# treangenlab/komb

Measured on AMD Instinct MI355X. Metric: peeled edges/sec (k-truss), higher is better.
Workload: dtype int32

## Files before the change

### komb_amd/csrc/api.cpp

```cpp
#include "common.h"

#include <cerrno>
#include <cmath>
#include <cstdlib>
#include <cstring>
#include <memory>
#include <new>
#include <vector>

using namespace komb;

namespace {

int require_device(komb_ctx *ctx)
{
    if (!ctx) return KOMB_ERR_ARG;
    if (!ctx->device_ok) {
        if (ctx->err.empty()) ctx->err = "no usable HIP device";
        return KOMB_ERR_DEVICE;
    }
    KOMB_HIP(ctx, hipSetDevice(ctx->device));
    ctx->err.clear();
    return KOMB_OK;
}

}

extern "C" {

int komb_abi_version(void) { return KOMB_ACCEL_ABI_VERSION; }

komb_ctx *komb_create(const komb_opts *opts)
{
    komb_ctx *ctx = new (std::nothrow) komb_ctx();
    if (!ctx) return nullptr;
    if (opts) ctx->opts = *opts;
    ctx->device = ctx->opts.device;
    int ndev = 0;
    hipError_t e = hipGetDeviceCount(&ndev);
    if (e != hipSuccess || ndev <= 0) {
        ctx->err = std::string("no usable HIP device: ") + (e != hipSuccess ? hipGetErrorString(e) : "device count is 0");
        (void)hipGetLastError();
        return ctx;
    }
    if (ctx->device < 0 || ctx->device >= ndev) {
        ctx->err = "device ordinal out of range";
        return ctx;
    }
    e = hipSetDevice(ctx->device);
    if (e == hipSuccess) e = hipHostMalloc((void **)&ctx->h_ctrl, 2 * sizeof(PeelCtrl), hipHostMallocDefault);
    if (e == hipSuccess) e = hipHostMalloc((void **)&ctx->h_local, 2 * sizeof(LocalCtrl), hipHostMallocDefault);
    if (e == hipSuccess) e = hipHostMalloc(&ctx->h_stage, kStageBytes, hipHostMallocDefault);
    ctx->stream = nullptr;
    if (e == hipSuccess && !(ctx->opts.reserved[0] & KOMB_CREATE_NULL_STREAM)) { e = hipStreamCreate(&ctx->stream); ctx->own_stream = e == hipSuccess; }
    if (e == hipSuccess && !ctx->timer.init()) e = hipErrorUnknown;
    if (e != hipSuccess) {
        ctx->err = std::string("device initialisation failed: ") + hipGetErrorString(e);
        return ctx;
    }
    ctx->device_ok = true;
    if (!(ctx->opts.reserved[0] & KOMB_CREATE_NO_WARMUP)) warm_up(ctx);
    return ctx;
}

void komb_destroy(komb_ctx *ctx)
{
    if (!ctx) return;
    if (ctx->device_ok) {
        (void)hipSetDevice(ctx->device);
        graph_free(ctx);
        stager_free(ctx);
        ctx->pool.clear();
        ctx->timer.destroy();
        if (ctx->own_stream && ctx->stream) (void)hipStreamDestroy(ctx->stream);
        if (ctx->h_ctrl) (void)hipHostFree(ctx->h_ctrl);
        if (ctx->h_local) (void)hipHostFree(ctx->h_local);
        if (ctx->h_stage) (void)hipHostFree(ctx->h_stage);
    }
    delete ctx;
}

const char *komb_last_error(const komb_ctx *ctx) { return ctx ? ctx->err.c_str() : "null context"; }

int komb_graph_from_edges(komb_ctx *ctx, int64_t nv, int64_t n_raw, const int64_t *uv_pairs)
{
    KOMB_TRY(require_device(ctx));
    return graph_from_edges(ctx, nv, n_raw, uv_pairs);
}
// ... 926 lines not shown
```

### komb_amd/csrc/clique_census.hip

```cpp
#include "clique_root_dev.h"

#include <algorithm>

namespace komb {

namespace {

constexpr int kCcGrid = 1024;
constexpr uint32_t kCcBatch = 256;
static_assert((long long)kCcGrid * kCcBatch == KOMB_MAXCLQ_OVERSHOOT, "the documented overshoot");
constexpr uint32_t kCcLdsCand = 512;
constexpr size_t kCcLdsBytes = 56u << 10;
constexpr size_t kCcScratchBytes = 512ull << 20;
constexpr long long kCcDefaultBudget = 1ll << 30;
constexpr long long kCcMaxBudget = 0x7FFFFFFFll - KOMB_MAXCLQ_OVERSHOOT;
constexpr unsigned long long kCcSat = ~0ull;
constexpr int32_t kCcPivotBit = (int32_t)0x80000000u;

struct CcCtl {
    unsigned long long nodes;
    unsigned long long n_roots;
    uint32_t cursor;
    uint32_t t_max;
    uint32_t max_p;
// ... 330 lines not shown
        uint32_t n_l = std::min(max_p, (uint32_t)cc_opt(ctx, "CENSUS_LDS", kCcLdsCand, 0, kCcLdsCand));
        while (n_l > 0 && (head_words + (size_t)n_l * ((n_l + 63u) >> 6)) * 8 > kCcLdsBytes) n_l -= 1;
        const uint32_t w_l = (n_l + 63u) >> 6;
        A.lds_cand = n_l;
        A.lds_off_tot = (uint32_t)(head_words - n_k);
        A.lds_off_mat = (uint32_t)head_words;
        A.lds_off_stk = A.lds_off_mat + n_l * w_l;
        A.lds_levels = std::min(n_l, depth) + 2;
        size_t lds_words = A.lds_off_stk;
        if (n_l > 0 && (lds_words + (size_t)A.lds_levels * w_l) * 8 <= kCcLdsBytes) lds_words += (size_t)A.lds_levels * w_l;
        else A.lds_levels = 0;
        if (lds_words * 8 > kCcLdsBytes)
            KOMB_FAIL(ctx, KOMB_ERR_LIMIT, "komb_clique_census_run: a window of %u sizes at t_max %d does not fit the LDS of a wavefront", n_k, (int)t_max);
        int grid = (int)std::min<uint32_t>(A.n_chunks, (uint32_t)kCcGrid);
        const size_t fit = kCcScratchBytes / A.slot_bytes;
        if ((size_t)grid > fit) grid = fit < 1 ? 1 : (int)fit;
        KOMB_HIP(ctx, bufs.alloc(&A.scratch, (size_t)grid * A.slot_bytes));
        A.count_only = false;
        KOMB_HIP(ctx, hipMemsetAsync(&A.ctl->cursor, 0, sizeof(uint32_t), s));
        k_cc_census<<<grid, kWave, lds_words * 8, s>>>(A);
        KOMB_HIP(ctx, hipGetLastError());
        const uint32_t n_scan = std::max<uint32_t>(n_k, k_local ? (uint32_t)nv : 0u);
        k_cc_saturated<<<(int)((n_scan + kBlock - 1) / kBlock), kBlock, 0, s>>>(A.total, n_k, A.local, (uint32_t)nv, A.ctl);
        KOMB_HIP(ctx, hipGetLastError());
        KOMB_HIP(ctx, d2h(ctx, &h, A.ctl, sizeof(CcCtl)));
        if (h.bad)
            KOMB_FAIL(ctx, KOMB_ERR_DEVICE, "komb_clique_census_run: the walk is inconsistent (k_lo %d, k_hi %d, largest candidate set %u)", (int)k_lo, (int)k_hi, max_p);
        KOMB_HIP(ctx, staged_copy(ctx, res.total.data(), A.total, (size_t)n_k * sizeof(unsigned long long), false));
        res.flags = (h.stopped ? 0 : KOMB_CENSUS_COMPLETE) | (h.saturated ? KOMB_CENSUS_SATURATED : 0);
        res.max_p = (int32_t)max_p;
        res.n_roots = (int64_t)h.n_roots;
        res.nodes = (int64_t)h.nodes;
    }
    res.ms = ctx->timer.stop(s);
    KOMB_HIP(ctx, hipGetLastError());
    for (uint32_t i = 0; i < n_k; ++i)
        if (res.total[i]) res.omega = k_lo + (int32_t)i;
    if (ctx_flag(ctx, "CENSUS_DEBUG"))
        fprintf(stderr, "komb clique census: %lld edges, t_max %d, window %d .. %d, k_local %d, omega %d, flags %d, largest candidate set %d, %lld roots, "
                "%lld nodes of %lld, run %.3f ms\n", (long long)m, res.t_max, res.k_lo, res.k_hi, res.k_local, res.omega, res.flags, res.max_p,
                (long long)res.n_roots, (long long)res.nodes, limit, res.ms);
    clique_census_drop(ctx);
    ctx->d_cc_local = fresh.local;
    fresh.local = nullptr;
    ctx->cc = std::move(res);
    ctx->cc_done = true;
    return KOMB_OK;
}

}
```

### komb_amd/csrc/clique_communities.hip

```cpp
#include "common.h"
#include "unionfind_dev.h"

#include <algorithm>

namespace komb {

namespace {

constexpr int kPcGrid = 1024;
constexpr long long kPcDefaultBudget = 1ll << 32;
constexpr long long kPcMaxWords = 1ll << 24;
constexpr uint32_t kPcMaxSize = 4098;
constexpr uint32_t kPcNone = 0xFFFFFFFFu;

struct PcCtl {
    unsigned long long pair_tests;
    unsigned long long links;
    uint32_t cursor;
    uint32_t bad;
    uint32_t pad[2];
};
static_assert(sizeof(PcCtl) == 32, "PcCtl layout");

struct PcArgs {
// ... 378 lines not shown
        k_pc_vfix<<<pc_grid(nv), kBlock, 0, s>>>(d_vc, d_vc + nv, unv);
        KOMB_HIP(ctx, hipGetLastError());
        KOMB_HIP(ctx, d2h(ctx, &h, A.ctl, sizeof(PcCtl)));
        if (h.bad)
            KOMB_FAIL(ctx, KOMB_ERR_DEVICE, "komb_clique_communities_run: the links are inconsistent (k %d, %lld member cliques, %lld communities)", (int)k,
                      (long long)res.n_member, (long long)n_comm);
        links_seen = (uint32_t)std::min<unsigned long long>(h.links, 0xFFFFFFFFull);
        res.n_comm = n_comm;
        res.rep.resize((size_t)n_comm);
        res.n_cliques.resize((size_t)n_comm);
        res.verts.resize((size_t)n_uniq);
        std::vector<uint32_t> coff((size_t)n_comm);
        KOMB_HIP(ctx, staged_copy(ctx, res.label.data(), d_label, (size_t)nc * sizeof(int32_t), false));
        KOMB_HIP(ctx, staged_copy(ctx, res.size.data(), d_size, (size_t)nc * sizeof(int32_t), false));
        KOMB_HIP(ctx, staged_copy(ctx, res.rep.data(), d_rep, (size_t)n_comm * sizeof(int32_t), false));
        KOMB_HIP(ctx, staged_copy(ctx, res.n_cliques.data(), d_ncl, (size_t)n_comm * sizeof(int32_t), false));
        KOMB_HIP(ctx, staged_copy(ctx, coff.data(), d_coff, (size_t)n_comm * sizeof(uint32_t), false));
        KOMB_HIP(ctx, staged_copy(ctx, res.verts.data(), d_cverts, (size_t)n_uniq * sizeof(int32_t), false));
        KOMB_HIP(ctx, staged_copy(ctx, res.v_comm.data(), d_vc, (size_t)nv * sizeof(int32_t), false));
        KOMB_HIP(ctx, staged_copy(ctx, res.v_first.data(), d_vc + nv, (size_t)nv * sizeof(int32_t), false));
        res.offset.assign((size_t)n_comm + 1, 0);
        for (int64_t c = 0; c < n_comm; ++c) res.offset[(size_t)c] = (int64_t)coff[(size_t)c];
        res.offset[(size_t)n_comm] = n_uniq;
        for (int64_t c = 0; c < n_comm; ++c) {
            const int64_t len = res.offset[(size_t)c + 1] - res.offset[(size_t)c];
            if (len < k) KOMB_FAIL(ctx, KOMB_ERR_DEVICE, "komb_clique_communities_run: community %lld has %lld vertices at k %d", (long long)c, (long long)len, (int)k);
            res.largest = std::max(res.largest, len);
        }
        for (int64_t v = 0; v < nv; ++v) {
            res.n_covered += res.v_comm[(size_t)v] >= 1;
            res.n_overlap += res.v_comm[(size_t)v] >= 2;
        }
    }
    res.ms = ctx->timer.stop(s);
    KOMB_HIP(ctx, hipGetLastError());
    if (ctx_flag(ctx, "PERC_DEBUG"))
        fprintf(stderr, "komb clique communities: k %d (list k_min %d), %lld cliques, %lld members of at most %u vertices, %lld entries, group %u, "
                "%lld pair tests of %llu, %u links, %lld communities, largest %lld, covered %lld, overlap %lld, run %.3f ms\n", (int)k, (int)res.k_min,
                (long long)nc, (long long)res.n_member, smax, (long long)entries, group, (long long)res.pair_tests, limit, links_seen, (long long)res.n_comm,
                (long long)res.largest, (long long)res.n_covered, (long long)res.n_overlap, res.ms);
    ctx->pc = std::move(res);
    ctx->pc_done = true;
    return KOMB_OK;
}

}
```

### komb_amd/csrc/common.h

```cpp
#pragma once

#include <hip/hip_runtime.h>

#include <chrono>
#include <cstddef>
#include <cstdint>
#include <cstdio>
#include <cstdlib>
#include <cstring>
#include <map>
#include <string>
#include <vector>

#include "komb_accel.h"

#include <roctracer/roctx.h>

namespace komb {

struct Range {
    explicit Range(const char *name) { (void)roctxRangePushA(name); }
    ~Range() { (void)roctxRangePop(); }
    void next(const char *name) { (void)roctxRangePop(); (void)roctxRangePushA(name); }
    Range(const Range &) = delete;
// ... 33 lines not shown
    int32_t  live_sel;
    int32_t  live_mode;
    int32_t  seq;
    uint32_t tail_l[2];
    uint32_t tail_h[2];
    int32_t  next_min;
    uint32_t live_tail;
    int32_t  last_retire;
    uint32_t tail_limit;
    uint32_t pad1[7];
    int32_t  max_retire_gap;
};
static_assert(offsetof(PeelCtrl, seq) == 60 && offsetof(PeelCtrl, tail_l) == 64, "PeelCtrl: the entry state is one 64-byte line");
static_assert(sizeof(PeelCtrl) == 128, "PeelCtrl layout");

struct LocalCtrl {
    int32_t  done;
    int32_t  iters;
    uint32_t spare[3];
    uint32_t bad;
    int32_t  max_val;
    uint32_t levels;
    uint32_t evals;
    uint32_t n_light, n_heavy;
    uint32_t n_giant;
    uint32_t n_chunk;
    uint32_t pad0;
    unsigned long long key_sum;
};
static_assert(sizeof(LocalCtrl) == 64, "LocalCtrl layout");

enum FinishMode : int { FIN_LOCAL = 0, FIN_LDS = 1, FIN_NONE = 2 };

struct Timer {
    hipEvent_t a = nullptr, b = nullptr;
    bool init() { return hipEventCreate(&a) == hipSuccess && hipEventCreate(&b) == hipSuccess; }
    void start(hipStream_t s) { (void)hipEventRecord(a, s); }
    double stop(hipStream_t s)
    {
        (void)hipEventRecord(b, s);
        (void)hipEventSynchronize(b);
        float ms = 0.f;
        (void)hipEventElapsedTime(&ms, a, b);
        return (double)ms;
    }
    void destroy() { if (a) (void)hipEventDestroy(a); if (b) (void)hipEventDestroy(b); a = b = nullptr; }
};

struct EventSet {
    std::vector<hipEvent_t> v;
    EventSet() = default;
    EventSet(const EventSet &) = delete;
    EventSet &operator=(const EventSet &) = delete;
    hipError_t make(hipEvent_t *out, unsigned flags = 0)
    {
        hipEvent_t e = nullptr;
        const hipError_t rc = flags ? hipEventCreateWithFlags(&e, flags) : hipEventCreate(&e);
        if (rc == hipSuccess) { v.push_back(e); *out = e; }
        return rc;
    }
    ~EventSet() { for (hipEvent_t e : v) if (e) (void)hipEventDestroy(e); }
};

}

struct Poison {
    bool on = false;
    uint32_t word = 0;
    hipStream_t stream = nullptr;
    hipError_t fill(void *p, size_t bytes) const
    {
        if (!on || !p || !bytes) return hipSuccess;
        const size_t words = bytes / 4, rest = bytes % 4;
        hipError_t e = hipSuccess;
        if (words) e = hipMemsetD32Async((hipDeviceptr_t)p, (int)word, words, stream);
        if (e == hipSuccess && rest) e = hipMemsetAsync((char *)p + 4 * words, (int)(word & 0xFFu), rest, stream);
        return e == hipSuccess ? hipStreamSynchronize(stream) : e;
    }
    hipError_t malloc(void **out, size_t bytes) const
// ... 58 lines not shown
        for (auto &b : blocks) { if (b.used) keep.push_back(b); else (void)hipFree(b.p); }
        blocks.swap(keep);
    }
    void clear()
    {
        for (auto &b : blocks) (void)hipFree(b.p);
        blocks.clear();
    }
};

struct TrussPrep {
    bool valid = false;
    int64_t nv = 0, ne = 0;
    int32_t  *o2i = nullptr, *i2o = nullptr;
    uint32_t *orow = nullptr;
    int32_t  *ocol = nullptr, *osrc = nullptr;
    uint32_t *e2k = nullptr;
    uint4    *vline = nullptr;
    void     *wtasks = nullptr;
    int64_t   n_wtasks = 0;
    int64_t   own_bound = 0;
    double    ms = 0.0;
    double    ms_part[4] = {0, 0, 0, 0};
};

struct komb_ctx {
    komb_opts opts{};
    DevPool pool;
    std::string err;
    bool device_ok = false;
    int device = 0;
    hipStream_t stream = nullptr;
    bool own_stream = false;
    komb::Timer timer;
    std::map<std::string, std::string> options;

    int64_t nv = -1, ne = 0;
    uint32_t *d_o_rowptr = nullptr;
    int32_t  *d_o_col = nullptr;
    TrussPrep prep;

    int32_t *d_deg = nullptr;
    int32_t *d_core = nullptr;
    bool core_done = false;

    int32_t *d_onion_layer = nullptr;
    int32_t *d_onion_core = nullptr;
    int64_t onion_layers = 0;
    int32_t onion_max_core = 0;
    double onion_ms = 0.0;
    bool onion_done = false;

    int32_t *d_comp_label = nullptr;
    int32_t *d_comp_size = nullptr;
    int32_t comp_kind = 0, comp_k = 0;
    int64_t comp_members = 0, comp_count = 0, comp_largest = 0;
    double comp_ms = 0.0;
    bool comp_done = false;

    int32_t *d_hier_nodes = nullptr;
    int32_t *d_hier_vnode = nullptr;
    int32_t hier_kind = 0, hier_kmax = 0, hier_depth = 0;
    int64_t hier_nodes = 0, hier_roots = 0;
    double hier_ms = 0.0;
    bool hier_done = false;

    int32_t *d_dens_member = nullptr;
// ... 178 lines not shown
    void release(void *q)
    {
        for (auto &p : owned) if (p == q && q) { ctx->pool.put(q); p = nullptr; }
    }
    ~DevBufs() { for (void *p : owned) if (p) ctx->pool.put(p); }
};

#define KOMB_FAIL(ctx, code, ...)                                   \
    do {                                                            \
        char _b[512];                                               \
        snprintf(_b, sizeof(_b), __VA_ARGS__);                      \
        (ctx)->err = _b;                                            \
        return (code);                                              \
    } while (0)

#define KOMB_HIP(ctx, call)                                                          \
    do {                                                                             \
        hipError_t _e = (call);                                                      \
        if (_e != hipSuccess) {                                                      \
            hipError_t _nomem = hipErrorOutOfMemory;                                 \
            KOMB_FAIL(ctx, _e == _nomem ? KOMB_ERR_NOMEM : KOMB_ERR_DEVICE,          \
                      "%s failed: %s (%s:%d)", #call, hipGetErrorString(_e),         \
                      __FILE__, __LINE__);                                           \
        }                                                                            \
    } while (0)

#define KOMB_TRY(expr)                         \
    do {                                       \
        int _s = (expr);                       \
        if (_s != KOMB_OK) return _s;          \
    } while (0)

constexpr size_t kStageBytes = 64 << 10;
inline hipError_t d2h(komb_ctx *ctx, void *dst, const void *src, size_t bytes)
{
    if (ctx->h_stage && bytes <= kStageBytes && dst != ctx->h_stage) {
        hipError_t e = hipMemcpyAsync(ctx->h_stage, src, bytes, hipMemcpyDeviceToHost, ctx->stream);
        if (e == hipSuccess) e = hipStreamSynchronize(ctx->stream);
        if (e == hipSuccess) memcpy(dst, ctx->h_stage, bytes);
        return e;
    }
    hipError_t e = hipMemcpyAsync(dst, src, bytes, hipMemcpyDeviceToHost, ctx->stream);
    return e == hipSuccess ? hipStreamSynchronize(ctx->stream) : e;
}

namespace komb {
int prim_sort_u64(komb_ctx *ctx, uint64_t *keys, uint64_t *tmp_keys, int64_t n, int end_bit, uint64_t **sorted);
int prim_unique_u64(komb_ctx *ctx, const uint64_t *in, uint64_t *out, int64_t n, int64_t *n_out);
int prim_exclusive_sum_u32(komb_ctx *ctx, const uint32_t *in, uint32_t *out, int64_t n);
int prim_exclusive_sum_u32_u64(komb_ctx *ctx, const uint32_t *in, unsigned long long *out, int64_t n);
int prim_sort_pairs_desc_i64(komb_ctx *ctx, int64_t *keys, int64_t *keys_tmp, uint32_t *vals, uint32_t *vals_tmp,
                             int64_t n, int end_bit, int64_t **sorted_keys, uint32_t **sorted_vals);

int prim_sort_pairs_u32_u64(komb_ctx *ctx, uint32_t *keys, uint32_t *keys_alt, unsigned long long *vals, unsigned long long *vals_alt,
                            int64_t n, int begin_bit, int end_bit, uint32_t **sorted_keys, unsigned long long **sorted_vals);
int prim_sort_pairs_u32_u32(komb_ctx *ctx, uint32_t *keys, uint32_t *keys_alt, uint32_t *vals, uint32_t *vals_alt,
                            int64_t n, int end_bit, uint32_t **sorted_keys, uint32_t **sorted_vals);
int prim_sort_pairs_u64_u32(komb_ctx *ctx, uint64_t *keys, uint64_t *keys_alt, uint32_t *vals, uint32_t *vals_alt,
                            int64_t n, int end_bit, uint64_t **sorted_keys, uint32_t **sorted_vals);

struct ForestNodes { int32_t *k, *rep, *par; uint32_t *size, *shell; };
struct ForestCtl {
    uint32_t log_n;
    uint32_t n_nodes;
    uint32_t n_roots;
    int32_t  depth;
// ... 41 lines not shown
void clique_census_drop(komb_ctx *ctx);
int maximal_cliques_run(komb_ctx *ctx, int32_t k_min, int64_t budget);
void maximal_cliques_drop(komb_ctx *ctx);
int clique_communities_run(komb_ctx *ctx, int32_t k, int64_t budget);
void clique_communities_drop(komb_ctx *ctx);
int densest_run(komb_ctx *ctx, int32_t iters);
int truss_run(komb_ctx *ctx, const uint8_t *vmask_host, int rank, int world, komb_allreduce_fn fn, void *user);
int merge_run(komb_ctx *ctx, const double *susp_host, int32_t *order, int32_t *side, int64_t *n_block, double *max_density);
int corea_ranks(komb_ctx *ctx, const int32_t *deg, const int32_t *core, int64_t n, double *rank_deg, double *rank_key);
int graph_from_edges(komb_ctx *ctx, int64_t nv, int64_t n_raw, const int64_t *uv);
int graph_from_csr(komb_ctx *ctx, int64_t nv, const int64_t *rowptr, const int32_t *col);
void graph_free(komb_ctx *ctx);
void stager_free(komb_ctx *ctx);
hipError_t staged_copy(komb_ctx *ctx, void *dst, const void *src, size_t bytes, bool to_device);
void warm_up(komb_ctx *ctx);
int prep_build(komb_ctx *ctx, const uint32_t *rowptr, const int32_t *col, int64_t nv, int64_t ns, TrussPrep *out);
void prep_free(komb_ctx *ctx, TrussPrep *p);
int prep_ensure(komb_ctx *ctx);
int prep_sources(komb_ctx *ctx, TrussPrep *p);
int graph_moments(komb_ctx *ctx, int64_t out[5]);
struct InducedCsr { int64_t nv = 0, ns = 0; uint32_t *rowptr = nullptr; int32_t *col = nullptr; int32_t *vold = nullptr; };
int induce_csr(komb_ctx *ctx, const uint8_t *vmask_host, InducedCsr *out);
void induced_free(komb_ctx *ctx, InducedCsr *g);
int edge_list(komb_ctx *ctx, const uint32_t *rowptr, const int32_t *col, int64_t nv, const int32_t *vold, int32_t *eu, int32_t *ev);
int truss_edges_canonical(komb_ctx *ctx);
void truss_free(komb_ctx *ctx);
int truss_support_canonical(komb_ctx *ctx);
void peel_ctrl_pre(hipStream_t s, uint32_t *d_grp_done);
void peel_collect_ctrl(hipStream_t s, PeelCtrl *d_collect, const PeelCtrl *d_from);
void peel_ctrl_init(hipStream_t s, PeelCtrl *d_ctrl, uint32_t *d_grp_done, uint32_t units, uint32_t tail_limit = 0);
int peel_grid(int64_t units);

template <typename F>
int drive_peel(komb_ctx *ctx, PeelCtrl *d_ctrl, int64_t units, F &&launch, int *launches_out)
{
#ifndef KOMB_PEEL_BATCH
#define KOMB_PEEL_BATCH 24
#endif
#ifndef KOMB_PEEL_BATCH_SHORT
#define KOMB_PEEL_BATCH_SHORT 6
#endif
    constexpr int kBatch = KOMB_PEEL_BATCH, kBatchShort = KOMB_PEEL_BATCH_SHORT, kShortBatches = 6;
    PeelCtrl first;
    KOMB_HIP(ctx, d2h(ctx, &first, d_ctrl, sizeof(PeelCtrl)));
    int32_t next = first.seq;
#ifdef KOMB_DEBUG_SWITCHES
    if (const char *tr = getenv("KOMB_PEEL_TRACE")) {
        FILE *f = fopen(tr, "a");
        hipEvent_t a = nullptr, b = nullptr;
        if (hipEventCreate(&a) != hipSuccess || hipEventCreate(&b) != hipSuccess) {
            if (f) fclose(f);
            if (a) (void)hipEventDestroy(a);
            KOMB_FAIL(ctx, KOMB_ERR_DEVICE, "peel trace: hipEventCreate failed");
        }
        int launches = 0;
        if (f) fprintf(f, "# peel units=%lld\n", (long long)units);
        for (int64_t i = 0; i < 4 * units + 4096; ++i) {
            PeelCtrl before;
            if (d2h(ctx, &before, d_ctrl, sizeof(PeelCtrl)) != hipSuccess) break;
            if (before.done) break;
            (void)hipEventRecord(a, ctx->stream);
            launch(before.seq); ++launches;
            (void)hipEventRecord(b, ctx->stream);
            (void)hipEventSynchronize(b);
            float ms = 0.f;
            (void)hipEventElapsedTime(&ms, a, b);
            if (f) fprintf(f, "%d %d %d %u %u %d %u %u %.1f\n", before.mode, before.level, before.round, before.cur_light,
                           before.cur_heavy, before.live_mode, before.live_count, before.remaining, ms * 1000.f);
        }
        if (f) fclose(f);
        (void)hipEventDestroy(a); (void)hipEventDestroy(b);
        if (launches_out) *launches_out = launches;
        KOMB_HIP(ctx, d2h(ctx, &ctx->h_ctrl[0], d_ctrl, sizeof(PeelCtrl)));
        return KOMB_OK;
    }
#endif
    EventSet evs;
    hipEvent_t ev[2] = {nullptr, nullptr};
    KOMB_HIP(ctx, evs.make(&ev[0], hipEventDisableTiming));
    KOMB_HIP(ctx, evs.make(&ev[1], hipEventDisableTiming));
    const int64_t max_batches = (4 * units + 4096) / kBatch + 16 + kShortBatches;
    int launches = 0, slot = 0, status = KOMB_OK;
    bool have_prev = false, finished = false, stuck = false;
    int32_t seen_seq = first.seq - 1;
    for (int64_t batch = 0; batch < max_batches && !finished; ++batch) {
        const int nb = (batch >= 1 && batch <= kShortBatches) ? kBatchShort : kBatch;
        for (int i = 0; i < nb; ++i) { launch(next); ++next; ++launches; }
        if (hipMemcpyAsync(&ctx->h_ctrl[slot], d_ctrl, sizeof(PeelCtrl), hipMemcpyDeviceToHost, ctx->stream) != hipSuccess ||
            hipEventRecord(ev[slot], ctx->stream) != hipSuccess) { status = KOMB_ERR_DEVICE; break; }
        if (have_prev) {
            if (hipEventSynchronize(ev[slot ^ 1]) != hipSuccess) { status = KOMB_ERR_DEVICE; break; }
            const PeelCtrl &h = ctx->h_ctrl[slot ^ 1];
            if (h.done) finished = true;
            else if (h.seq == seen_seq) { stuck = true; finished = true; }
            seen_seq = h.seq;
        }
        have_prev = true;
        slot ^= 1;
    }
    hipError_t e = hipStreamSynchronize(ctx->stream);
    if (launches_out) *launches_out = launches;
    if (status != KOMB_OK || e != hipSuccess)
        KOMB_FAIL(ctx, KOMB_ERR_DEVICE, "peel driver: HIP failure (%s)", hipGetErrorString(e));
    if (d2h(ctx, &ctx->h_ctrl[0], d_ctrl, sizeof(PeelCtrl)) != hipSuccess)
        KOMB_FAIL(ctx, KOMB_ERR_DEVICE, "peel driver: control block readback failed");
    if (!ctx->h_ctrl[0].done)
        KOMB_FAIL(ctx, KOMB_ERR_DEVICE, "peel driver: %s (level %d, remaining %u, launch %d of state %d)",
                  stuck ? "the launches make no progress" : "launch budget exhausted before completion",
                  ctx->h_ctrl[0].level, ctx->h_ctrl[0].remaining, (int)next, (int)ctx->h_ctrl[0].seq);
    return KOMB_OK;
}
}
```

### komb_amd/csrc/communities.hip

```cpp
#include "common.h"
#include "unionfind_dev.h"

namespace komb {

namespace {

constexpr uint32_t kCommShort = 16;
constexpr uint32_t kCommHeavy = 2048;
constexpr int kCommHeavyGrid = 256, kCommHeavyChunks = 8;
constexpr int kCommTailGrid = 2048;

struct CommCtl {
    uint32_t n_heavy;
    uint32_t n_members, n_communities, largest;
    uint32_t n_multi;
    uint32_t pad[11];
};
static_assert(sizeof(CommCtl) == 64, "CommCtl layout");

inline int comm_grid(int64_t n) { return (int)((n + kBlock - 1) / kBlock); }

__global__ void k_comm_flag(const int32_t *__restrict__ truss, uint32_t m, int32_t k, uint32_t *__restrict__ flag)
{
    const uint32_t i = blockIdx.x * kBlock + threadIdx.x;
// ... 247 lines not shown
    KOMB_HIP(ctx, bufs.alloc(&d_ctl, 1));
    KOMB_HIP(ctx, bufs.alloc(&d_flag, (size_t)m + 1));
    KOMB_HIP(ctx, bufs.alloc(&d_pos, (size_t)m + 1));
    KOMB_HIP(ctx, bufs.alloc(&d_kept, (size_t)m));
    KOMB_HIP(ctx, bufs.alloc(&d_mu, (size_t)m));
    KOMB_HIP(ctx, bufs.alloc(&d_mv, (size_t)m));
    KOMB_HIP(ctx, bufs.alloc(&d_parent, (size_t)m));
    KOMB_HIP(ctx, bufs.alloc(&d_heavy, (size_t)heavy_cap));
    KOMB_HIP(ctx, bufs.alloc(&d_rs, (size_t)nv));
    KOMB_HIP(ctx, bufs.alloc(&d_re, (size_t)nv));
    const uint32_t n_short = comm_opt_u32(ctx, "COMM_SHORT", kCommShort);
    uint32_t n_heavy = comm_opt_u32(ctx, "COMM_HEAVY", kCommHeavy);
    if (n_heavy <= n_short) n_heavy = n_short + 1;

    const int32_t *eu = ctx->d_t_eu, *ev = ctx->d_t_ev, *truss = ctx->d_t_truss;
    const uint32_t *d_nm = d_pos + m;
    uint32_t *d_cnt = d_flag;
    const int grid = comm_grid(m), grid1 = comm_grid(m + 1);
    ctx->timer.start(s);
    KOMB_HIP(ctx, hipMemsetAsync(d_ctl, 0, sizeof(CommCtl), s));
    KOMB_HIP(ctx, hipMemsetAsync(d_rs, 0, (size_t)nv * sizeof(uint32_t), s));
    KOMB_HIP(ctx, hipMemsetAsync(d_re, 0, (size_t)nv * sizeof(uint32_t), s));
    k_comm_flag<<<grid1, kBlock, 0, s>>>(truss, (uint32_t)m, k, d_flag);
    KOMB_TRY(prim_exclusive_sum_u32(ctx, d_flag, d_pos, m + 1));
    k_comm_compact<<<grid, kBlock, 0, s>>>(eu, ev, truss, (uint32_t)m, k, d_pos, d_kept, d_mu, d_mv, d_parent, d_cnt);
    k_comm_rows<<<grid, kBlock, 0, s>>>(d_mu, d_nm, d_rs, d_re);
    k_comm_tri<<<grid, kBlock, 0, s>>>(d_mu, d_mv, d_rs, d_re, d_nm, d_parent, d_ctl, d_heavy, heavy_cap, n_short, n_heavy);
    k_comm_heavy<<<dim3(kCommHeavyGrid, kCommHeavyChunks), kBlock, 0, s>>>(d_mu, d_mv, d_rs, d_re, d_parent, d_ctl, d_heavy, heavy_cap);
    k_comm_flatten<false><<<grid, kBlock, 0, s>>>(d_nm, d_parent);
    k_comm_flatten<true><<<grid, kBlock, 0, s>>>(d_nm, d_parent);
    const int tail_grid = grid < kCommTailGrid ? grid : kCommTailGrid;
    k_comm_count<<<tail_grid, kBlock, 0, s>>>(d_nm, d_parent, d_cnt);
    k_comm_finish<<<tail_grid, kBlock, 0, s>>>((uint32_t)m, truss, k, d_pos, d_parent, d_kept, d_cnt, ctx->d_comm_label, ctx->d_comm_size, d_ctl);
    const double ms = ctx->timer.stop(s);
    KOMB_HIP(ctx, hipGetLastError());
    CommCtl h;
    KOMB_HIP(ctx, d2h(ctx, &h, d_ctl, sizeof(CommCtl)));
    ctx->comm_members = (int64_t)h.n_members; ctx->comm_count = (int64_t)h.n_communities; ctx->comm_largest = (int64_t)h.largest;
    ctx->comm_ms = ms;
    ctx->comm_done = true;
    fail.armed = false;
    return KOMB_OK;
}

int communities_vertices(komb_ctx *ctx)
{
    if (ctx->comm_v_ready) return KOMB_OK;
    hipStream_t s = ctx->stream;
    const int64_t m = ctx->t_ne, nv = ctx->nv, nm = ctx->comm_members;
    if (!ctx->d_comm_ncomm) KOMB_HIP(ctx, ctx->pool.get((void **)&ctx->d_comm_ncomm, (size_t)(nv > 0 ? nv : 1) * sizeof(int32_t)));
    ctx->comm_multi = 0;
    ctx->timer.start(s);
    KOMB_HIP(ctx, hipMemsetAsync(ctx->d_comm_ncomm, 0, (size_t)(nv > 0 ? nv : 1) * sizeof(int32_t), s));
    if (nm > 0) {
        Range r_all("komb_truss_communities: vertices");
        DevBufs bufs(ctx);
        CommCtl *d_ctl = nullptr;
        uint32_t *d_flag = nullptr, *d_pos = nullptr;
        uint64_t *d_keys = nullptr, *d_tmp = nullptr, *sorted = nullptr;
        KOMB_HIP(ctx, bufs.alloc(&d_ctl, 1));
        KOMB_HIP(ctx, bufs.alloc(&d_flag, (size_t)m + 1));
        KOMB_HIP(ctx, bufs.alloc(&d_pos, (size_t)m + 1));
        KOMB_HIP(ctx, bufs.alloc(&d_keys, 2 * (size_t)nm));
        KOMB_HIP(ctx, bufs.alloc(&d_tmp, 2 * (size_t)nm));
        KOMB_HIP(ctx, hipMemsetAsync(d_ctl, 0, sizeof(CommCtl), s));
        k_comm_vflag<<<comm_grid(m + 1), kBlock, 0, s>>>(ctx->d_comm_label, (uint32_t)m, d_flag);
        KOMB_TRY(prim_exclusive_sum_u32(ctx, d_flag, d_pos, m + 1));
        k_comm_keys<<<comm_grid(m), kBlock, 0, s>>>(ctx->d_t_eu, ctx->d_t_ev, ctx->d_comm_label, (uint32_t)m, d_pos, d_keys);
        int vb = 1;
        while (vb < 31 && (1ll << vb) < nv) ++vb;
        KOMB_TRY(prim_sort_u64(ctx, d_keys, d_tmp, 2 * nm, 32 + vb, &sorted));
        uint64_t *uniq = sorted == d_keys ? d_tmp : d_keys;
        int64_t n_u = 0;
        KOMB_TRY(prim_unique_u64(ctx, sorted, uniq, 2 * nm, &n_u));
        k_comm_runs<<<comm_grid(n_u), kBlock, 0, s>>>(uniq, (uint32_t)n_u, ctx->d_comm_ncomm, d_ctl);
        KOMB_HIP(ctx, hipGetLastError());
        CommCtl h;
        KOMB_HIP(ctx, d2h(ctx, &h, d_ctl, sizeof(CommCtl)));
        ctx->comm_multi = (int64_t)h.n_multi;
    }
    ctx->comm_ms_vertices = ctx->timer.stop(s);
    ctx->comm_v_ready = true;
    return KOMB_OK;
}

}
```

### komb_amd/csrc/community_hierarchy.hip

```cpp
#include "forest_dev.h"

namespace komb {

namespace {

constexpr uint32_t kChShort = 16;
constexpr uint32_t kChHeavy = 2048;
constexpr int kChHeavyGrid = 256, kChHeavyChunks = 8;
constexpr uint64_t kChMaxRecords = 0x7FFFFFFFull;

struct ChCtl {
    ForestCtl f;
    uint32_t n_heavy;
    uint32_t n_members;
    uint32_t rec_n;
    uint32_t pad0;
    unsigned long long n_tri;
    uint32_t pad[6];
};
static_assert(sizeof(ChCtl) == 64 && offsetof(ChCtl, f) == 0, "ChCtl layout");


__global__ void k_ch_flag(const int32_t *__restrict__ truss, uint32_t m, uint32_t *__restrict__ flag)
{
// ... 325 lines not shown
            uint32_t n_levels = 0;
            for (int32_t k = (int32_t)levels - 1; k >= 3; --k) n_levels += moff[k + 1] - moff[k] ? 1u : 0u;
            KOMB_HIP(ctx, bufs.alloc(&seg, (size_t)n_levels + 1));
            KOMB_HIP(ctx, hipMemsetAsync(seg, 0, ((size_t)n_levels + 1) * sizeof(uint32_t), s));

            const ForestState f{parent, log, claimk, cur, cnt, seg, mnode, t, &d_ctl->f, nm};
            uint32_t li = 0;
            for (int32_t k = (int32_t)levels - 1; k >= 3; --k) {
                const uint32_t sh_b = moff[k], sh_n = moff[k + 1] - moff[k];
                const uint32_t r_b = roff[k], r_n = roff[k + 1] - roff[k];
                if (!sh_n) continue;
                if (li == 0) k_max = k;
                if (r_n) k_ch_link<<<forest_grid(r_n), kBlock, 0, s>>>(recs, r_b, r_n, nm, parent, d_ctl, log, nm);
                forest_level(ctx, f, k, li, false, mord, sh_b, sh_n, r_n < nm ? r_n : nm);
                ++li;
            }
            KOMB_HIP(ctx, hipGetLastError());
            KOMB_HIP(ctx, d2h(ctx, &h, d_ctl, sizeof(ChCtl)));
            if (h.f.n_nodes > nm || h.f.log_n > nm || h.rec_n != n_rec)
                KOMB_FAIL(ctx, KOMB_ERR_DEVICE, "komb_community_hierarchy_run: inconsistent state (%u nodes, %u hooks, %u members, %u of %u records)",
                          h.f.n_nodes, h.f.log_n, nm, h.rec_n, n_rec);
            n = h.f.n_nodes;
            if (n > 0) {
                cap_nodes = n;
                KOMB_HIP(ctx, ctx->pool.get((void **)&fresh.nodes, 5 * cap_nodes * sizeof(int32_t)));
                ForestNodes out{fresh.nodes, fresh.nodes + cap_nodes, fresh.nodes + 2 * cap_nodes,
                                (uint32_t *)fresh.nodes + 3 * cap_nodes, (uint32_t *)fresh.nodes + 4 * cap_nodes};
                KOMB_TRY(forest_tail(ctx, bufs, f, n, bits, out, rank, kept, mvals, mvals2));
            }
            k_ch_edges_out<<<grid, kBlock, 0, s>>>((uint32_t)m, truss, d_pos, mnode, rank, n, fresh.enode);
        } else {
            k_ch_edges_out<<<grid, kBlock, 0, s>>>((uint32_t)m, truss, d_pos, nullptr, nullptr, 0u, fresh.enode);
        }
        ms = ctx->timer.stop(s);
        KOMB_HIP(ctx, hipGetLastError());
        KOMB_HIP(ctx, d2h(ctx, &h, d_ctl, sizeof(ChCtl)));
        n_nodes = (int64_t)n; n_roots = (int64_t)h.f.n_roots; depth = h.f.depth; n_members = (int64_t)nm;
        if (n == 0) k_max = 2;
    }
    if (!fresh.nodes) KOMB_HIP(ctx, ctx->pool.get((void **)&fresh.nodes, 5 * cap_nodes * sizeof(int32_t)));

    community_hierarchy_drop(ctx);
    ctx->d_ch_nodes = fresh.nodes; ctx->d_ch_enode = fresh.enode;
    fresh.nodes = fresh.enode = nullptr;
    ctx->ch_cap = (int64_t)cap_nodes;
    ctx->ch_nodes = n_nodes; ctx->ch_roots = n_roots; ctx->ch_members = n_members;
    ctx->ch_kmax = k_max; ctx->ch_depth = depth; ctx->ch_ms = ms;
    ctx->ch_done = true;
    return KOMB_OK;
}

int community_hierarchy_labels(komb_ctx *ctx, int32_t k, int32_t *label, int32_t *size)
{
    const int64_t m = ctx->t_ne > 0 ? ctx->t_ne : 0;
    if (m == 0 || (!label && !size)) return KOMB_OK;
    hipStream_t s = ctx->stream;
    DevBufs bufs(ctx);
    int32_t *d_label = nullptr, *d_size = nullptr;
    KOMB_HIP(ctx, bufs.alloc(&d_label, (size_t)m));
    KOMB_HIP(ctx, bufs.alloc(&d_size, (size_t)m));
    const int32_t *nodes = ctx->d_ch_nodes;
    const size_t c = (size_t)ctx->ch_cap;
    k_ch_labels<<<forest_grid(m), kBlock, 0, s>>>((uint32_t)m, k, ctx->d_ch_enode, (uint32_t)ctx->ch_nodes, nodes, nodes + c, nodes + 2 * c,
                                              nodes + 3 * c, d_label, d_size);
    KOMB_HIP(ctx, hipGetLastError());
    KOMB_HIP(ctx, hipStreamSynchronize(s));
    if (label) KOMB_HIP(ctx, staged_copy(ctx, label, d_label, (size_t)m * sizeof(int32_t), false));
// ... 6 lines not shown
```

### komb_amd/csrc/components.hip

```cpp
#include "common.h"
#include "unionfind_dev.h"

namespace komb {

namespace {

constexpr uint32_t kCompShort = 16;
constexpr uint32_t kCompHeavy = 2048;
constexpr uint32_t kCompWindow = 16;
constexpr int kCompSamples = 1024;
constexpr int kCompHeavyGrid = 256, kCompHeavyChunks = 8;
constexpr int kCompTailGrid = 2048;

struct CompCtl {
    int32_t  giant;
    uint32_t n_heavy;
    uint32_t n_members, n_components, largest;
    uint32_t pad[11];
};
static_assert(sizeof(CompCtl) == 64, "CompCtl layout");

__global__ void k_comp_init(uint32_t nv, const int32_t *__restrict__ core, int32_t k, bool all, bool none,
                            int32_t *__restrict__ parent, int32_t *__restrict__ flag, uint32_t *__restrict__ cnt)
{
// ... 211 lines not shown

    const bool truss = kind == KOMB_COMP_TRUSS;
    const int64_t m = truss ? ctx->t_ne : 0;
    if (truss && m > 0) KOMB_TRY(truss_edges_canonical(ctx));

    Range r_all("komb_components_run");
    DevBufs bufs(ctx);
    const uint32_t heavy_cap = (uint32_t)((2 * ctx->ne) / kCompHeavy + 64);
    CompCtl *d_ctl = nullptr; uint32_t *d_cnt = nullptr; int32_t *d_heavy = nullptr;
    KOMB_HIP(ctx, bufs.alloc(&d_ctl, 1));
    KOMB_HIP(ctx, bufs.alloc(&d_cnt, (size_t)nv));
    if (!truss) KOMB_HIP(ctx, bufs.alloc(&d_heavy, (size_t)heavy_cap));
    const char *so = ctx_opt(ctx, "COMP_SAMPLE");
    const bool sample = so ? strcmp(so, "0") != 0 : true;

    int32_t *parent = ctx->d_comp_label, *flag = ctx->d_comp_size;
    const int grid = comp_grid(nv);
    const bool all = !truss && k == 0;
    const bool none = truss || (k > 0 && k > ctx->stats.max_coreness);
    ctx->timer.start(s);
    KOMB_HIP(ctx, hipMemsetAsync(d_ctl, 0, sizeof(CompCtl), s));
    k_comp_init<<<grid, kBlock, 0, s>>>((uint32_t)nv, ctx->d_core, k, all, none, parent, flag, d_cnt);
    if (truss) {
        if (m > 0) k_comp_truss<<<comp_grid(m), kBlock, 0, s>>>(ctx->d_t_eu, ctx->d_t_ev, ctx->d_t_truss, (uint32_t)m, k, parent, flag);
    } else if (!none && ctx->ne > 0) {
        if (all) comp_link_rows<true>(ctx, sample, k, parent, flag, d_ctl, d_heavy, heavy_cap);
        else comp_link_rows<false>(ctx, sample, k, parent, flag, d_ctl, d_heavy, heavy_cap);
    }
    k_comp_flatten<false><<<grid, kBlock, 0, s>>>((uint32_t)nv, parent, flag);
    k_comp_flatten<true><<<grid, kBlock, 0, s>>>((uint32_t)nv, parent, flag);
    const int tail_grid = grid < kCompTailGrid ? grid : kCompTailGrid;
    k_comp_count<<<tail_grid, kBlock, 0, s>>>((uint32_t)nv, parent, d_cnt);
    k_comp_finish<<<tail_grid, kBlock, 0, s>>>((uint32_t)nv, parent, d_cnt, ctx->d_comp_size, d_ctl);
    const double ms = ctx->timer.stop(s);
    KOMB_HIP(ctx, hipGetLastError());
    CompCtl h;
    KOMB_HIP(ctx, d2h(ctx, &h, d_ctl, sizeof(CompCtl)));
    ctx->comp_members = (int64_t)h.n_members; ctx->comp_count = (int64_t)h.n_components; ctx->comp_largest = (int64_t)h.largest;
    ctx->comp_ms = ms;
    ctx->comp_done = true;
    return KOMB_OK;
}

}
```

### komb_amd/csrc/corea.hip

```cpp
#include "common.h"

namespace komb {

namespace {

__global__ __launch_bounds__(kBlock) void k_corea_keys(const int32_t *__restrict__ deg, const int32_t *__restrict__ core,
                                                       int64_t n, int64_t *__restrict__ kdeg, int64_t *__restrict__ kcore,
                                                       uint32_t *__restrict__ idx0, uint32_t *__restrict__ idx1)
{
    for (int64_t i = (int64_t)blockIdx.x * kBlock + threadIdx.x; i < n; i += (int64_t)gridDim.x * kBlock) {
        const int64_t d = deg[i];
        kdeg[i] = d;
        kcore[i] = (int64_t)core[i] * n + d;
        idx0[i] = (uint32_t)i; idx1[i] = (uint32_t)i;
    }
}

__global__ __launch_bounds__(kBlock) void k_run_ranks(const int64_t *__restrict__ sk, const uint32_t *__restrict__ sidx,
                                                      int64_t n, double *__restrict__ rank)
{
    for (int64_t p = (int64_t)blockIdx.x * kBlock + threadIdx.x; p < n; p += (int64_t)gridDim.x * kBlock) {
        const int64_t key = sk[p];
        int64_t lo = 0, hi = p;
        while (lo < hi) {
// ... 25 lines not shown
    if (n < 0 || (n > 0 && (!deg || !core || !rank_deg || !rank_key)))
        KOMB_FAIL(ctx, KOMB_ERR_ARG, "komb_corea: bad arguments");
    ctx->stats.ms_corea = 0.0;
    if (n == 0) return KOMB_OK;
    if (n > INT32_MAX - 1) KOMB_FAIL(ctx, KOMB_ERR_LIMIT, "komb_corea: n exceeds 2^31-2");
    int32_t maxd = 0, maxc = 0;
    for (int64_t i = 0; i < n; ++i) {
        if (deg[i] < 0 || core[i] < 0) KOMB_FAIL(ctx, KOMB_ERR_ARG, "komb_corea: negative degree/coreness at %lld", (long long)i);
        if (deg[i] > maxd) maxd = deg[i];
        if (core[i] > maxc) maxc = core[i];
    }
    hipStream_t s = ctx->stream;
    DevBufs bufs(ctx);
    int32_t *d_deg = nullptr, *d_core = nullptr; int64_t *d_k[4] = {nullptr, nullptr, nullptr, nullptr};
    uint32_t *d_i[4] = {nullptr, nullptr, nullptr, nullptr}; double *d_r[2] = {nullptr, nullptr};
    KOMB_HIP(ctx, bufs.alloc(&d_deg, (size_t)n));
    KOMB_HIP(ctx, bufs.alloc(&d_core, (size_t)n));
    for (int t = 0; t < 4; ++t) KOMB_HIP(ctx, bufs.alloc(&d_k[t], (size_t)n));
    for (int t = 0; t < 4; ++t) KOMB_HIP(ctx, bufs.alloc(&d_i[t], (size_t)n));
    for (int t = 0; t < 2; ++t) KOMB_HIP(ctx, bufs.alloc(&d_r[t], (size_t)n));
    KOMB_HIP(ctx, staged_copy(ctx, d_deg, deg, (size_t)n * 4, true));
    KOMB_HIP(ctx, staged_copy(ctx, d_core, core, (size_t)n * 4, true));
    int64_t g64 = (n + kBlock - 1) / kBlock;
    const int grid = (int)(g64 > 4096 ? 4096 : g64);
    ctx->timer.start(s);
    k_corea_keys<<<grid, kBlock, 0, s>>>(d_deg, d_core, n, d_k[0], d_k[2], d_i[0], d_i[2]);
    int64_t *sk = nullptr; uint32_t *si = nullptr;
    int st = prim_sort_pairs_desc_i64(ctx, d_k[0], d_k[1], d_i[0], d_i[1], n, bits_for(maxd), &sk, &si);
    if (st == KOMB_OK) {
        k_run_ranks<<<grid, kBlock, 0, s>>>(sk, si, n, d_r[0]);
        st = prim_sort_pairs_desc_i64(ctx, d_k[2], d_k[3], d_i[2], d_i[3], n, bits_for((int64_t)maxc * n + maxd), &sk, &si);
    }
    if (st == KOMB_OK) k_run_ranks<<<grid, kBlock, 0, s>>>(sk, si, n, d_r[1]);
    ctx->stats.ms_corea = ctx->timer.stop(s);
    KOMB_TRY(st);
    KOMB_HIP(ctx, staged_copy(ctx, rank_deg, d_r[0], (size_t)n * 8, false));
    KOMB_HIP(ctx, staged_copy(ctx, rank_key, d_r[1], (size_t)n * 8, false));
    return KOMB_OK;
}

}
```

### komb_amd/csrc/densest.hip

```cpp
#include "common.h"

namespace komb {

namespace {

constexpr uint32_t kDenShort = 16;
constexpr uint32_t kDenHeavy = 2048;
constexpr int kDenHeavyGrid = 64, kDenHeavyChunks = 8;
constexpr int kDenGrid = 2048;
constexpr uint32_t kDenLdsBins = 4096;
constexpr int kDenLocalBlock = 1024;
constexpr int kDenPairs = 4;
constexpr uint64_t kDenLocalAutoPairs = 20000;

struct DenCtl {
    uint32_t n_heavy;
    int32_t  k_best, k_prune;
    uint32_t n_p;
    uint32_t max_deg_p;
    uint32_t load_max;
    int32_t  source;
    uint32_t best_i;
    unsigned long long m_best, n_best;
    unsigned long long m_p;
// ... 437 lines not shown
    DevBufs bufs(ctx);
    const int32_t k_max = ctx->stats.max_coreness > 0 ? ctx->stats.max_coreness : 0;
    const uint32_t K = (uint32_t)k_max + 1u;
    const uint32_t heavy_cap = (uint32_t)((2 * ctx->ne) / kDenHeavy + 64);
    const int grid = den_grid((uint64_t)nv);

    DenCtl *d_ctl = nullptr; int32_t *d_heavy = nullptr;
    uint32_t *d_hist = nullptr, *d_flag = nullptr, *d_pid = nullptr, *d_cnt = nullptr, *d_off = nullptr, *d_hdeg = nullptr, *d_hcur = nullptr;
    long long *d_prof = nullptr;
    KOMB_HIP(ctx, bufs.alloc(&d_ctl, 1));
    KOMB_HIP(ctx, bufs.alloc(&d_heavy, (size_t)heavy_cap));
    KOMB_HIP(ctx, bufs.alloc(&d_hdeg, (size_t)heavy_cap));
    KOMB_HIP(ctx, bufs.alloc(&d_hcur, (size_t)heavy_cap));
    KOMB_HIP(ctx, bufs.alloc(&d_hist, (size_t)2 * K));
    KOMB_HIP(ctx, bufs.alloc(&d_prof, (size_t)2 * K));
    KOMB_HIP(ctx, bufs.alloc(&d_flag, (size_t)nv));
    KOMB_HIP(ctx, bufs.alloc(&d_pid, (size_t)nv));
    KOMB_HIP(ctx, bufs.alloc(&d_cnt, (size_t)nv));
    KOMB_HIP(ctx, bufs.alloc(&d_off, (size_t)nv));

    ctx->timer.start(s);
    KOMB_HIP(ctx, hipMemsetAsync(d_ctl, 0, sizeof(DenCtl), s));
    KOMB_HIP(ctx, hipMemsetAsync(d_hist, 0, (size_t)2 * K * sizeof(uint32_t), s));
    KOMB_HIP(ctx, hipMemsetAsync(d_hdeg, 0, (size_t)heavy_cap * sizeof(uint32_t), s));
    KOMB_HIP(ctx, hipMemsetAsync(d_hcur, 0, (size_t)heavy_cap * sizeof(uint32_t), s));
    if (K <= kDenLdsBins) den_row_pass(ctx, DenHist<true>{ctx->d_core, K, d_hist}, (size_t)2 * K * sizeof(uint32_t), d_ctl, d_heavy, heavy_cap);
    else den_row_pass(ctx, DenHist<false>{ctx->d_core, K, d_hist}, 0, d_ctl, d_heavy, heavy_cap);
    k_den_profile<<<1, kBlock, 0, s>>>(K, d_hist, d_prof, d_prof + K, d_ctl);
    k_den_mark<<<grid, kBlock, 0, s>>>((uint32_t)nv, ctx->d_core, d_ctl, d_flag);
    KOMB_TRY(prim_exclusive_sum_u32(ctx, d_flag, d_pid, nv));
    den_row_pass(ctx, DenCount{ctx->d_core, d_cnt, d_hdeg, 0u, 0u, 0u}, 0, d_ctl, d_heavy, heavy_cap);
    KOMB_TRY(prim_exclusive_sum_u32(ctx, d_cnt, d_off, nv));
    k_den_total<<<1, kBlock, 0, s>>>((uint32_t)nv, d_flag, d_pid, d_cnt, d_off, d_hdeg, heavy_cap, d_ctl);
    double ms = ctx->timer.stop(s);
    KOMB_HIP(ctx, hipGetLastError());
    DenCtl h;
    KOMB_HIP(ctx, d2h(ctx, &h, d_ctl, sizeof(DenCtl)));
    std::vector<int64_t> profile((size_t)2 * K);
    KOMB_HIP(ctx, d2h(ctx, profile.data(), d_prof, profile.size() * sizeof(int64_t)));
    const uint64_t n_p = h.n_p, m_p = h.m_p;
    if (n_p > (uint64_t)nv || m_p > (uint64_t)ctx->ne)
        KOMB_FAIL(ctx, KOMB_ERR_DEVICE, "komb_densest_subgraph_run: inconsistent state (%llu of %lld vertices, %llu of %lld edges)",
                  (unsigned long long)n_p, (long long)nv, (unsigned long long)m_p, (long long)ctx->ne);
    if ((uint64_t)iters * h.max_deg_p > (uint64_t)INT32_MAX)
        KOMB_FAIL(ctx, KOMB_ERR_LIMIT, "komb_densest_subgraph_run: %d rounds on a vertex of degree %u inside the pruned set overflow the 32-bit load word",
                  iters, h.max_deg_p);

    const bool rounds = iters >= 1 && m_p > 0;
    uint2 *d_pairs = nullptr; uint32_t *d_load = nullptr, *d_delta = nullptr, *d_rank = nullptr, *d_rhist = nullptr;
    uint64_t *d_keys = nullptr, *d_keys2 = nullptr;
    unsigned long long *d_excl = nullptr, *d_part = nullptr;
    const int part_grid = den_grid_capped(n_p);
    bool local = false;
    if (rounds) {
        KOMB_HIP(ctx, bufs.alloc(&d_pairs, (size_t)m_p + kDenPairs));
        KOMB_HIP(ctx, bufs.alloc(&d_load, (size_t)n_p));
        KOMB_HIP(ctx, bufs.alloc(&d_delta, (size_t)n_p));
        KOMB_HIP(ctx, bufs.alloc(&d_rank, (size_t)n_p));
        KOMB_HIP(ctx, bufs.alloc(&d_rhist, (size_t)n_p));
        KOMB_HIP(ctx, bufs.alloc(&d_keys, (size_t)n_p));
        KOMB_HIP(ctx, bufs.alloc(&d_keys2, (size_t)n_p));
        KOMB_HIP(ctx, bufs.alloc(&d_excl, (size_t)n_p));
        KOMB_HIP(ctx, bufs.alloc(&d_part, (size_t)2 * part_grid));
        int lds_cap = 0;
        KOMB_HIP(ctx, hipDeviceGetAttribute(&lds_cap, hipDeviceAttributeMaxSharedMemoryPerBlock, ctx->device));
        const bool fits = n_p * 2 * sizeof(uint32_t) <= (uint64_t)(lds_cap > 0 ? lds_cap : 0) && m_p <= 0xFFFFFFFFull;
        const char *lo = ctx_opt(ctx, "DENSEST_LOCAL");
        local = fits && (lo ? strcmp(lo, "0") != 0 : m_p <= kDenLocalAutoPairs);
        if (local)
            KOMB_HIP(ctx, hipFuncSetAttribute((const void *)k_den_local, hipFuncAttributeMaxDynamicSharedMemorySize, (int)(n_p * 2 * sizeof(uint32_t))));
    }
    ctx->timer.start(s);
    if (rounds) {
        den_row_pass(ctx, DenFill{ctx->d_core, d_pid, d_off, d_pairs, d_hcur, m_p, 0u}, 0, d_ctl, d_heavy, heavy_cap);
        if (local) {
            k_den_local<<<1, kDenLocalBlock, (size_t)n_p * 2 * sizeof(uint32_t), s>>>(d_pairs, (uint32_t)m_p, (uint32_t)n_p, iters, d_load);
        } else {
            const int rgrid = den_grid((m_p + kDenPairs - 1) / kDenPairs), ngrid = den_grid(n_p);
            k_den_zero2<<<ngrid, kBlock, 0, s>>>((uint32_t)n_p, d_load, d_delta);
            for (int32_t t = 0; t < iters; ++t) {
                k_den_round<<<rgrid, kBlock, 0, s>>>(d_pairs, m_p, (uint32_t)n_p, d_load, d_delta, t & 1);
                k_den_fold<<<ngrid, kBlock, 0, s>>>((uint32_t)n_p, d_load, d_delta);
            }
        }
        KOMB_HIP(ctx, hipGetLastError());
        k_den_keys<<<part_grid, kBlock, 0, s>>>((uint32_t)n_p, d_load, d_keys, d_ctl);
        uint64_t *sorted = nullptr;
        KOMB_TRY(prim_sort_u64(ctx, d_keys, d_keys2, (int64_t)n_p, 64, &sorted));
        k_den_ranks<<<den_grid(n_p), kBlock, 0, s>>>((uint32_t)n_p, sorted, d_rank, d_rhist);
        k_den_rank_hist<<<den_grid(m_p), kBlock, 0, s>>>(d_pairs, m_p, (uint32_t)n_p, d_rank, d_rhist);
        KOMB_TRY(prim_exclusive_sum_u32_u64(ctx, d_rhist, d_excl, (int64_t)n_p));
        k_den_prefix_part<<<part_grid, kBlock, 0, s>>>((uint32_t)n_p, d_rhist, d_excl, d_part);
    }
    k_den_decide<<<1, kWave, 0, s>>>(rounds ? (uint32_t)part_grid : 0u, d_part, d_ctl);
    KOMB_HIP(ctx, hipGetLastError());
    k_den_out<<<grid, kBlock, 0, s>>>((uint32_t)nv, ctx->d_core, d_pid, d_load, d_rank, d_ctl, ctx->d_dens_member, ctx->d_dens_load);
    ms += ctx->timer.stop(s);
    hipError_t e = hipGetLastError();
    if (e == hipSuccess) e = d2h(ctx, &h, d_ctl, sizeof(DenCtl));
    if (e != hipSuccess) { ctx->dens_done = false; KOMB_HIP(ctx, e); }
    komb_ctx::Densest &r = ctx->dens;
    r.source = h.source; r.k_best = h.k_best; r.k_prune = h.k_prune; r.iters = iters; r.k_max = k_max;
    r.n_pruned = (int64_t)n_p; r.m_pruned = (int64_t)m_p; r.n_sub = (int64_t)h.n_sub; r.m_sub = (int64_t)h.m_sub;
    r.load_max = (int64_t)h.load_max; r.ms = ms; r.local = local;
    ctx->dens_profile.swap(profile);
    ctx->dens_done = true;
    return KOMB_OK;
}

}
```

### komb_amd/csrc/hierarchy.hip

```cpp
#include "forest_dev.h"

namespace komb {

namespace {

constexpr uint32_t kHierShort = 16;
constexpr uint32_t kHierHeavy = 2048;
constexpr int kHierHeavyGrid = 64, kHierHeavyChunks = 8;

struct HierCtl {
    ForestCtl f;
    uint32_t n_heavy;
    uint32_t pad[11];
};
static_assert(sizeof(HierCtl) == 64 && offsetof(HierCtl, f) == 0, "HierCtl layout");

__global__ void k_hier_init(uint32_t nv, int32_t *__restrict__ parent, int32_t *__restrict__ cur, int32_t *__restrict__ claimk,
                            uint32_t *__restrict__ cnt, int32_t *__restrict__ vnode, int32_t *__restrict__ lvl)
{
    const uint32_t v = blockIdx.x * kBlock + threadIdx.x;
    if (v >= nv) return;
    parent[v] = (int32_t)v;
    cur[v] = -1;
    claimk[v] = 0x7FFFFFFF;
// ... 213 lines not shown
        if (li == 0) k_top = k;
        uint64_t hooks;
        if (truss) {
            k_hier_edges<<<forest_grid(e_n), kBlock, 0, s>>>(ctx->d_t_eu, ctx->d_t_ev, eord, second[k], e_n, parent, d_ctl, log, (uint32_t)nv);
            hooks = e_n < (uint64_t)nv ? e_n : (uint64_t)nv;
        } else {
            if (k > 0) {
                k_hier_rows<<<forest_grid(sh_n), kBlock, 0, s>>>(ctx->d_o_rowptr, ctx->d_o_col, ctx->d_core, k, vord, sh_b, sh_n, parent, d_ctl,
                                                               d_heavy, heavy_cap, log, (uint32_t)nv);
                if (second[k])
                    k_hier_heavy<<<dim3(second[k] < (uint32_t)kHierHeavyGrid ? second[k] : kHierHeavyGrid, kHierHeavyChunks), kBlock, 0, s>>>(
                        ctx->d_o_rowptr, ctx->d_o_col, ctx->d_core, k, parent, d_ctl, d_heavy, heavy_done, second[k], heavy_cap, log, (uint32_t)nv);
                heavy_done += second[k];
            }
            hooks = (uint64_t)nv - voff[k];
        }
        forest_level(ctx, f, k, li, !truss && k == 0, vord, sh_b, sh_n, hooks);
        ++li;
    }
    KOMB_HIP(ctx, hipGetLastError());
    HierCtl h;
    KOMB_HIP(ctx, d2h(ctx, &h, d_ctl, sizeof(HierCtl)));
    if (h.f.n_nodes > (uint64_t)nv || h.f.log_n > (uint64_t)nv)
        KOMB_FAIL(ctx, KOMB_ERR_DEVICE, "komb_hierarchy_run: inconsistent state (%u nodes, %u hooks, %lld vertices)", h.f.n_nodes, h.f.log_n, (long long)nv);
    if (h.n_heavy != heavy_done)
        KOMB_FAIL(ctx, KOMB_ERR_DEVICE, "komb_hierarchy_run: inconsistent state (%u long rows queued, %u counted)", h.n_heavy, heavy_done);
    const uint32_t n = h.f.n_nodes;

    ForestNodes out{ctx->d_hier_nodes, ctx->d_hier_nodes + cap, ctx->d_hier_nodes + 2 * cap,
                    (uint32_t *)ctx->d_hier_nodes + 3 * cap, (uint32_t *)ctx->d_hier_nodes + 4 * cap};
    int32_t *rank = cur;
    if (n > 0) KOMB_TRY(forest_tail(ctx, bufs, f, n, bits, out, rank, nullptr, vvals, vvals2));
    k_hier_vertices_out<<<grid, kBlock, 0, s>>>((uint32_t)nv, vnode, rank, ctx->d_hier_vnode);
    const double ms = ctx->timer.stop(s);
    KOMB_HIP(ctx, hipGetLastError());
    KOMB_HIP(ctx, d2h(ctx, &h, d_ctl, sizeof(HierCtl)));
    ctx->hier_nodes = (int64_t)n; ctx->hier_roots = (int64_t)h.f.n_roots; ctx->hier_depth = h.f.depth;
    ctx->hier_kmax = n > 0 ? k_top : k_min;
    ctx->hier_ms = ms;
    ctx->hier_done = true;
    return KOMB_OK;
}

}
```

### komb_amd/csrc/kcore.hip

```cpp
#include "peel_dev.h"
#include "core_tail.h"
#include "local_dev.h"
#include "shard_dev.h"

#include <cstdlib>

namespace komb {

namespace {

__global__ __launch_bounds__(kBlock) void k_core_init(const uint32_t *__restrict__ rowptr, int64_t nv,
                                                      int32_t *__restrict__ deg, int32_t *__restrict__ degw,
                                                      int32_t *__restrict__ core, uint32_t *__restrict__ init)
{
    uint32_t zeros = 0;
    int32_t lmin = 0x7FFFFFFF;
    for (int64_t v = (int64_t)blockIdx.x * kBlock + threadIdx.x; v < nv; v += (int64_t)gridDim.x * kBlock) {
        const int32_t d = (int32_t)(rowptr[v + 1] - rowptr[v]);
        deg[v] = d; degw[v] = d;
        if (d == 0) { core[v] = 0; ++zeros; }
        else { core[v] = alive_marker((uint32_t)d); lmin = min(lmin, d); }
    }
    block_add_min(zeros, lmin, &init[0], (int32_t *)&init[1]);
}
// ... 171 lines not shown
{
    k_ctrl_init<<<1, 64, 0, s>>>(d_ctrl, d_grp_done, units, tail_limit);
}

int peel_grid(int64_t units)
{
    int64_t g = (units + kPeelBlock - 1) / kPeelBlock;
    if (g < 1) g = 1;
    if (g > 256 * kPeelPerCu) g = 256 * kPeelPerCu;
    return (int)g;
}

int core_run(komb_ctx *ctx, int rank, int world, komb_allreduce_fn fn, void *user, bool sharded)
{
    if (ctx->nv < 0) KOMB_FAIL(ctx, KOMB_ERR_STATE, "komb_core_run: no graph loaded");
    const int64_t nv = ctx->nv;
    hipStream_t s = ctx->stream;
    ctx->core_done = false;
    if (!ctx->d_deg) {
        KOMB_HIP(ctx, dev_malloc(ctx, (void **)&ctx->d_deg, (size_t)(nv > 0 ? nv : 1) * sizeof(int32_t)));
        KOMB_HIP(ctx, dev_malloc(ctx, (void **)&ctx->d_core, (size_t)(nv > 0 ? nv : 1) * sizeof(int32_t)));
    }
    komb_stats &stt = ctx->stats;
    stt.core_levels = stt.core_subrounds = stt.core_launches = 0;
    stt.max_coreness = 0; stt.ms_core = 0.0;
    stt.core_local_units = 0; stt.core_local_sweeps = 0; stt.core_local_items = 0; stt.ms_core_local = 0.0;
    if (ctx_flag(ctx, "SHARD_ENGINE")) sharded = true;
    stt.shard_exchanges = 0; stt.ms_exchange = 0.0; stt.exchange_words = 0;
    stt.engine_flags = sharded ? KOMB_ENGINE_SHARD_PEEL : 0;
    if (nv == 0) { ctx->core_done = true; return KOMB_OK; }

    Range r_all("komb_core_run");
    DevBufs bufs(ctx);
    const size_t heavy_cap = (size_t)(2 * ctx->ne) / 32 + 64;
    int32_t *d_degw = nullptr; PeelCtrl *d_ctrl = nullptr; uint32_t *d_grp = nullptr;
    CoreTailBufs T{};
    PeelQueues Q{nullptr, {nullptr, nullptr}, {nullptr, nullptr}, {nullptr, nullptr}, 0};
    KOMB_HIP(ctx, bufs.alloc(&d_degw, (size_t)nv));
    for (int i = 0; i < 2; ++i) {
        KOMB_HIP(ctx, bufs.alloc(&Q.light[i], (size_t)nv));
        KOMB_HIP(ctx, bufs.alloc(&Q.heavy[i], heavy_cap));
        KOMB_HIP(ctx, bufs.alloc(&Q.live[i], (size_t)nv / 2 + 64));
    }
    KOMB_HIP(ctx, bufs.alloc(&Q.code, (size_t)nv));
    KOMB_HIP(ctx, bufs.alloc(&d_ctrl, 1));
    KOMB_HIP(ctx, bufs.alloc(&d_grp, (size_t)kInitOff + 4));
    const FinishMode fin = finish_mode(ctx, FIN_LOCAL);
    uint32_t tail_limit = 0;
    const size_t live_words = ((size_t)nv + 63) / 64;
    unsigned long long *d_livebits = nullptr;
    if (fin == FIN_LDS) {
        tail_limit = kCoreTailV;
        if (const char *tl = ctx_opt(ctx, "CORE_TAIL")) tail_limit = (uint32_t)strtoul(tl, nullptr, 10);
        if (tail_limit > kCoreTailV) tail_limit = kCoreTailV;
        if (tail_limit) {
            KOMB_HIP(ctx, bufs.alloc(&T.livebits, live_words));
            KOMB_HIP(ctx, bufs.alloc(&T.vnum, (size_t)nv));
            KOMB_HIP(ctx, bufs.alloc(&T.cnt, 4));
            KOMB_HIP(ctx, bufs.alloc(&T.vlist, (size_t)kCoreTailV));
            KOMB_HIP(ctx, bufs.alloc(&T.rows, (size_t)kCoreTailV * kCoreTailWords));
        }
    } else if (fin == FIN_LOCAL) {
        tail_limit = local_limit(ctx, (uint64_t)nv, 16);
        if (tail_limit) KOMB_HIP(ctx, bufs.alloc(&d_livebits, live_words));
    }

    int64_t g = (nv + kBlock - 1) / kBlock;
    const int grid_init = (int)(g > 1024 ? 1024 : g);
    const int grid = peel_grid(nv);
    CoreProblem P{(uint32_t)nv, ctx->d_o_rowptr, ctx->d_o_col, d_degw, ctx->d_core};
    ctx->timer.start(s);
    peel_ctrl_pre(s, d_grp);
    k_core_init<<<grid_init, kBlock, 0, s>>>(ctx->d_o_rowptr, nv, ctx->d_deg, d_degw, ctx->d_core, d_grp + kInitOff);
    peel_ctrl_init(s, d_ctrl, d_grp, (uint32_t)nv, tail_limit);
    auto run_tail = [&](const int32_t *list, uint32_t n_in) -> int {
        KOMB_HIP(ctx, hipMemsetAsync(T.livebits, 0, live_words * sizeof(unsigned long long), s));
        KOMB_HIP(ctx, hipMemsetAsync(T.cnt, 0, 4 * sizeof(uint32_t), s));
        KOMB_HIP(ctx, hipMemsetAsync(T.rows, 0, (size_t)kCoreTailV * kCoreTailWords * sizeof(unsigned long long), s));
        int64_t gm = ((int64_t)n_in + kBlock - 1) / kBlock;
        k_ctail_mark<<<(int)(gm < 1 ? 1 : (gm > 1024 ? 1024 : gm)), kBlock, 0, s>>>(list, n_in, ctx->d_core, T);
        k_ctail_rows<<<dim3(kCoreTailV, 8), kBlock, 0, s>>>(ctx->d_o_rowptr, ctx->d_o_col, T);
        k_core_tail<false><<<1, 1024, 0, s>>>(d_ctrl, T, d_degw, ctx->d_core, nullptr);
        KOMB_HIP(ctx, d2h(ctx, &ctx->h_ctrl[0], d_ctrl, sizeof(PeelCtrl)));
        return KOMB_OK;
    };
    auto run_local = [&]() -> int {
        const PeelCtrl hc = ctx->h_ctrl[0];
        Range r_local("core: local finish");
        EventSet evs;
        hipEvent_t ev[2] = {nullptr, nullptr};
        for (auto &e : ev) KOMB_HIP(ctx, evs.make(&e));
        (void)hipEventRecord(ev[0], s);
        KOMB_HIP(ctx, hipMemsetAsync(d_livebits, 0, live_words * sizeof(unsigned long long), s));
        LocalStats ls;
        const int rc = local_finish(ctx, bufs, hc, d_ctrl, (uint32_t)nv, ctx->d_core, d_degw, Q.live[hc.live_sel],
            (uint32_t)kWave * CoreLocal::kU, sizeof(uint32_t), local_item_limit(ctx, std::max<uint64_t>(kCoreLocalItems, (uint64_t)ctx->ne / 3)), 0u, false, 0, ctx->d_core,
            [&](const LocalGraph &lg, const int32_t *num, void *items, PeelCtrl *d_cctrl, int32_t launch) {
                CoreCollect C{(uint32_t)nv, ctx->d_o_rowptr, ctx->d_o_col, ctx->d_core, d_livebits, num, lg.off, lg.cur, (uint32_t *)items};
                k_peel_step<CoreCollect><<<grid, kPeelBlock, 0, s>>>(d_cctrl, d_grp, Q, C, launch);
            },
            [&](const LocalGraph &lg, void *items, uint64_t total, LocalCtrl *d_lctrl, uint32_t *d_cnt, int *launches) -> int {
                return local_fixpoint(ctx, d_lctrl, d_cnt, lg, CoreLocal{(const uint32_t *)items}, total, launches);
            },
            &ls,
            [&](const LocalGraph &lg) { k_live_bits<<<(int)((lg.n + 255) / 256 > 1024 ? 1024 : (lg.n + 255) / 256), 256, 0, s>>>(lg.gid, lg.n, d_livebits); });
        (void)hipEventRecord(ev[1], s);
        (void)hipEventSynchronize(ev[1]);
        float ms = 0.f;
        (void)hipEventElapsedTime(&ms, ev[0], ev[1]);
        KOMB_TRY(rc);
        if (ls.refused) { ctx->h_ctrl[0].done = 0; ctx->h_ctrl[0].tail_limit = ls.new_limit; return KOMB_OK; }
        stt.core_local_units = (int32_t)ls.units; stt.core_local_sweeps = ls.sweeps; stt.core_local_items = (int64_t)ls.items;
        stt.ms_core_local = (double)ms;
        PeelCtrl done = hc;
        done.done = 1; done.remaining = 0;
        done.n_levels += (int32_t)ls.levels;
        done.max_level = ls.max_val > done.max_level ? ls.max_val : done.max_level;
        ctx->h_ctrl[0] = done;
        return KOMB_OK;
    };
    int launches = 0, st = KOMB_OK;
    if (sharded) {
        uint32_t iw[2] = {0u, 0u};
        KOMB_HIP(ctx, d2h(ctx, iw, d_grp + kInitOff, sizeof(iw)));
        ShardCore SP{(uint32_t)nv, ctx->d_o_rowptr, ctx->d_o_col, d_degw, ctx->d_core, 0u, 0u};
        shard_bounds((uint64_t)nv, rank, world, &SP.lo, &SP.hi);
        ShardStats ss;
        st = shard_peel(ctx, bufs, SP, d_degw, (uint32_t)nv, iw[0], (int32_t)iw[1], rank, world, fn, user, Q, d_ctrl,
                        [&](int32_t launch) { k_peel_step<ShardCore><<<grid, kPeelBlock, 0, s>>>(d_ctrl, d_grp, Q, SP, launch); },
                        fin == FIN_LOCAL ? tail_limit : 0u, [&]() -> int { return run_local(); }, &ss);
        stt.shard_exchanges = (int32_t)ss.exchanges; stt.ms_exchange = ss.ms_exchange; stt.exchange_words = ss.words;
        launches = ss.launches;
        PeelCtrl fc{};
        fc.done = st == KOMB_OK ? 1 : 2; fc.n_levels = ss.levels; fc.n_rounds = ss.rounds; fc.n_scans = ss.scans; fc.max_level = ss.max_level;
        ctx->h_ctrl[0] = fc;
    } else if (tail_limit && (uint64_t)nv <= tail_limit) {
        st = d2h(ctx, &ctx->h_ctrl[0], d_ctrl, sizeof(PeelCtrl)) == hipSuccess ? KOMB_OK : KOMB_ERR_DEVICE;
        if (st == KOMB_OK && !ctx->h_ctrl[0].done) st = (fin == FIN_LOCAL) ? run_local() : run_tail(nullptr, (uint32_t)nv);
    } else {
        ctx->h_ctrl[0].done = 0;
    }
    for (int guard = 0; st == KOMB_OK && ctx->h_ctrl[0].done != 1 && ctx->h_ctrl[0].done != 2 && guard < 64; ++guard) {
        if (ctx->h_ctrl[0].done == 3) {
            const PeelCtrl &c = ctx->h_ctrl[0];
            if (fin == FIN_LOCAL) st = run_local();
            else st = c.live_mode ? run_tail(Q.live[c.live_sel], c.live_count) : run_tail(nullptr, (uint32_t)nv);
            continue;
        }
        int batch = 0;
        st = drive_peel(ctx, d_ctrl, nv, [&](int32_t launch) {
            k_peel_step<CoreProblem><<<grid, kPeelBlock, 0, s>>>(d_ctrl, d_grp, Q, P, launch);
        }, &batch);
        launches += batch;
    }
    stt.ms_core = ctx->timer.stop(s);
#ifdef KOMB_STEP_TIMERS
    {
        const PeelCtrl &c = ctx->h_ctrl[0];
        const double n = c.pad1[6] ? (double)c.pad1[6] : 1.0;
        fprintf(stderr, "komb core step timers (block 0, %u small multi-workgroup PROCESS steps), us per step: ctrl %.2f queue+slice %.2f items %.2f flush %.2f barrier %.2f ticket %.2f\n",
                c.pad1[6], c.pad1[0] / n / 100.0, c.pad1[1] / n / 100.0, c.pad1[2] / n / 100.0, c.pad1[3] / n / 100.0, c.pad1[4] / n / 100.0, c.pad1[5] / n / 100.0);
    }
#endif
    KOMB_TRY(st);
    if (ctx->h_ctrl[0].done != 1) KOMB_FAIL(ctx, KOMB_ERR_DEVICE, "k-core peel ended in an inconsistent state");
    if (stt.core_local_units) stt.engine_flags |= KOMB_ENGINE_LOCAL_FINISH;
    else if (fin == FIN_LDS && tail_limit) stt.engine_flags |= KOMB_ENGINE_LDS_TAIL;
    stt.core_levels = ctx->h_ctrl[0].n_levels;
    stt.core_subrounds = ctx->h_ctrl[0].n_rounds;
    stt.core_launches = launches;
    stt.max_coreness = ctx->h_ctrl[0].max_level;
    ctx->core_done = true;
    return KOMB_OK;
}

}
```

### komb_amd/csrc/ktruss.hip

```cpp
#include "peel_dev.h"
#include "truss_tail.h"
#include "local_dev.h"
#include "shard_dev.h"

#include <algorithm>
#include <cstdlib>
#include <cstring>

#include "truss_line.h"
#include "truss_tri.h"
#include "truss_wedge.h"
#include "truss_index.h"
#include "truss_gather.h"

namespace komb {

namespace {

struct TrussProblem {
    static constexpr bool kChain = false;
    static constexpr bool kSingleStep = false;
    uint32_t units;
    const uint2 *off2;
    const int2 *inc;
// ... 226 lines not shown
    hipStream_t s = ctx->stream;
    const int64_t m = ctx->t_ne;
    KOMB_HIP(ctx, ctx->pool.get((void **)&ctx->d_t_sup, (size_t)m * sizeof(int32_t)));
#ifndef KOMB_TEST_SKIP_SLICE_ZERO
    if (ctx->t_k_lo) KOMB_HIP(ctx, hipMemsetAsync(ctx->d_t_sup, 0, (size_t)ctx->t_k_lo * sizeof(int32_t), s));
    if (ctx->t_k_hi < (uint32_t)m) KOMB_HIP(ctx, hipMemsetAsync(ctx->d_t_sup + ctx->t_k_hi, 0, ((size_t)m - ctx->t_k_hi) * sizeof(int32_t), s));
#endif
    k_scatter_len<<<grid_for(m), kBlock, 0, s>>>(ctx->d_t_slice, ctx->prep.e2k, m, ctx->t_k_lo, ctx->t_k_hi, ctx->d_t_sup);
    KOMB_HIP(ctx, hipStreamSynchronize(s));
    ctx->t_sup_ready = true;
    return KOMB_OK;
}

int truss_run(komb_ctx *ctx, const uint8_t *vmask_host, int rank, int world, komb_allreduce_fn fn, void *user)
{
    if (world < 1 || rank < 0 || rank >= world || (world > 1 && !fn))
        KOMB_FAIL(ctx, KOMB_ERR_ARG, "komb_truss_run_sharded: bad rank %d / world %d / callback", rank, world);
    if (ctx->nv < 0) KOMB_FAIL(ctx, KOMB_ERR_STATE, "komb_truss_run: no graph loaded");
    truss_free(ctx);
    hipStream_t s = ctx->stream;
    komb_stats &st = ctx->stats;
    st.triangles = 0; st.truss_levels = st.truss_subrounds = st.truss_launches = 0;
    st.max_trussness = 0; st.ms_support = st.ms_peel = st.ms_orient = st.ms_tri_count = st.ms_tri_fill = st.ms_gather = st.ms_allreduce = st.ms_compact = 0.0;
    st.truss_scans = 0; st.ms_prepare = 0.0; st.truss_prepared = 0; st.ms_prep_vertex = st.ms_prep_edges = st.ms_prep_rows = 0.0;
    auto empty_result = [&]() -> int {
        KOMB_HIP(ctx, ctx->pool.get((void **)&ctx->d_t_eu, 4)); KOMB_HIP(ctx, ctx->pool.get((void **)&ctx->d_t_ev, 4));
        KOMB_HIP(ctx, ctx->pool.get((void **)&ctx->d_t_truss, 4)); KOMB_HIP(ctx, ctx->pool.get((void **)&ctx->d_t_sup, 4));
        ctx->t_own_edges = true; ctx->t_ne = 0; ctx->truss_done = true; ctx->t_sup_ready = true;
        return KOMB_OK;
    };
    if (ctx->nv == 0 || ctx->ne == 0) return empty_result();
    Range r_all("komb_truss_run");
    DevBufs bufs(ctx);

    Range phase("truss: preparation");
    InducedCsr sub;
    TrussPrep sub_prep;
    struct SubGuard { komb_ctx *c; InducedCsr *g; TrussPrep *p; ~SubGuard() { prep_free(c, p); induced_free(c, g); } } sub_guard{ctx, &sub, &sub_prep};
    TrussPrep *tp = &ctx->prep;
    if (vmask_host) {
        ctx->timer.start(s);
        KOMB_TRY(induce_csr(ctx, vmask_host, &sub));
        st.ms_orient = ctx->timer.stop(s);
        if (sub.ns == 0) return empty_result();
        KOMB_TRY(prep_build(ctx, sub.rowptr, sub.col, sub.nv, sub.ns, &sub_prep));
        st.ms_prepare = sub_prep.ms; st.truss_prepared = 1;
        st.ms_prep_vertex = sub_prep.ms_part[0]; st.ms_prep_edges = sub_prep.ms_part[1]; st.ms_prep_rows = sub_prep.ms_part[2];
        tp = &sub_prep;
    } else if (!ctx->prep.valid) {
        KOMB_TRY(prep_ensure(ctx));
        st.ms_prepare = ctx->prep.ms; st.truss_prepared = 1;
        st.ms_prep_vertex = ctx->prep.ms_part[0]; st.ms_prep_edges = ctx->prep.ms_part[1]; st.ms_prep_rows = ctx->prep.ms_part[2];
    }
    const int64_t nv = tp->nv;
    const int64_t m = tp->ne;
    const uint32_t *d_orow = tp->orow;
    const int32_t *d_ocol = tp->ocol;
    const uint4 *d_line = tp->vline;
    const uint2 *d_wtasks = (const uint2 *)tp->wtasks;
    const int64_t n_wtasks = tp->n_wtasks;
    const int gw = grid_for(n_wtasks, kTriWaves);
    phase.next("truss: triangles + incidence index");

    const int ge = grid_for(m);
    const int tri_tv = (int)std::max<int64_t>(1, std::min<int64_t>(kTriV, nv / (256 * KOMB_TRI_EU * kTriWaves * 4)));
    const int64_t ntasks = (nv + tri_tv - 1) / tri_tv;
    const int gt = grid_for(ntasks, kTriWaves);
    uint32_t *d_own = nullptr, *d_other = nullptr, *d_cnt = nullptr, *d_off = nullptr;
    uint2 *d_off2 = nullptr;
    KOMB_HIP(ctx, bufs.alloc(&d_own, 2 * ((size_t)m + 1)));
    d_other = d_own + ((size_t)m + 1);
    KOMB_HIP(ctx, bufs.alloc(&d_cnt, (size_t)m + 1));
    KOMB_HIP(ctx, bufs.alloc(&d_off2, (size_t)m + 4));
    unsigned long long *d_mom = nullptr;
    KOMB_HIP(ctx, bufs.alloc(&d_mom, 12));
    KOMB_HIP(ctx, hipMemsetAsync(d_mom, 0, 12 * sizeof(unsigned long long), s));
// ... 8 lines not shown
        if (const char *tl = ctx_opt(ctx, "TAIL")) tail_limit = (uint32_t)strtoul(tl, nullptr, 10);
        if (tail_limit > kTailMaxEdges) tail_limit = kTailMaxEdges;
    } else if (fin == FIN_LOCAL) tail_limit = local_limit(ctx, (uint64_t)m, 32);
    const bool whole_peel_finish = tail_limit && (uint64_t)m <= tail_limit;
    const bool shard_peel_on = (ctx->shard_peel && world > 1) || ctx_flag(ctx, "SHARD_ENGINE");
    enum { IDX_STREAM = 0, IDX_TWO_PASS = 2 };
    int layout = IDX_STREAM;
    if (const char *ix = ctx_opt(ctx, "INDEX")) {
        if (!strcmp(ix, "two_pass")) layout = IDX_TWO_PASS;
        else if (strcmp(ix, "stream")) KOMB_FAIL(ctx, KOMB_ERR_ARG, "option INDEX=%s: expected stream or two_pass", ix);
    }
    int2 *d_owndense = nullptr;
    unsigned long long *d_ownoff = nullptr, *d_dcur = nullptr;
    uint32_t *d_cnt_ref = nullptr;
    uint32_t *d_toff = nullptr;
    uint32_t *d_grp = nullptr;
    int32_t *d_light0 = nullptr;
    uint32_t *d_bintot = nullptr;
    uint32_t *d_reckey = nullptr;
    int2 *d_recval = nullptr;
    const BinGeom geom = bin_geom(m);
    const int64_t n_bins = (int64_t)geom.nb;
    const TriStream no_stream{nullptr, nullptr, nullptr, 0ull, 0u, 0u, 0};
#ifdef KOMB_DEBUG_SWITCHES
    const int ablate = getenv("KOMB_TRI_ABLATE") ? atoi(getenv("KOMB_TRI_ABLATE")) : 0;
#else
    const int ablate = 0;
#endif
    st.ms_sort = 0.0; st.tri_records = 0; st.ms_compact = 0.0; st.ms_tri_count = 0.0; st.ms_tri_fill = 0.0; st.stream_retries = 0;
    st.index_layout = layout;
    auto zero_counts = [&]() -> hipError_t { return hipMemsetAsync(d_own, 0, 2 * ((size_t)m + 1) * sizeof(uint32_t), s); };
    if (!(world == 1 && layout == IDX_STREAM)) KOMB_HIP(ctx, zero_counts());
    bool have_counts = false;
    if (world > 1) {
        const int64_t task_lo = n_wtasks * rank / world, task_hi = n_wtasks * (rank + 1) / world;
        ctx->timer.start(s);
        k_wedges<TRI_COUNT><<<gw, kBlock, 0, s>>>(d_orow, d_ocol, d_line, d_wtasks, task_lo, task_hi, d_own, d_other, nullptr, nullptr, 0ull, nullptr, no_stream, nullptr, ablate);
        st.ms_tri_count = ctx->timer.stop(s);
        k_sum_counts<<<ge, kBlock, 0, s>>>(d_own, d_other, nullptr, m + 1, d_cnt, d_mom + 5);
        ctx->timer.start(s);
        KOMB_HIP(ctx, hipStreamSynchronize(s));
        if (fn(user, d_cnt, (int64_t)m + 1) != 0)
            KOMB_FAIL(ctx, KOMB_ERR_DEVICE, "komb_truss_run_sharded: all-reduce callback failed");
        st.ms_allreduce = ctx->timer.stop(s);
        KOMB_HIP(ctx, hipMemsetAsync(d_mom + 5, 0, sizeof(unsigned long long), s));
        k_total_u32<<<ge, kBlock, 0, s>>>(d_cnt, m + 1, d_mom + 5);
        have_counts = true;
        if (layout != IDX_TWO_PASS) {
            KOMB_HIP(ctx, bufs.alloc(&d_cnt_ref, (size_t)m + 1));
            KOMB_HIP(ctx, hipMemcpyAsync(d_cnt_ref, d_cnt, ((size_t)m + 1) * sizeof(uint32_t), hipMemcpyDeviceToDevice, s));
            KOMB_HIP(ctx, zero_counts());
        }
    }

    if (layout == IDX_STREAM) {
        const unsigned long long bound = (unsigned long long)tp->own_bound;
        const int gws = std::min(gw, 256 * KOMB_WEDGE_EU);
        const unsigned long long slack = (unsigned long long)gws * kTriWaves * kRecChunk + kRecChunk;
        const unsigned long long own_slack = (unsigned long long)gws * kTriWaves * kOwnChunk + kOwnChunk;
        const unsigned long long t_bound = bound / 2;
        const unsigned long long own_full = bound + bound / 8 + own_slack, rec_full = 3 * t_bound + (3 * t_bound) / 14 + slack;
        unsigned long long own_cap = std::min(own_full, 4ull * (unsigned long long)m + own_slack);
        unsigned long long rec_cap = std::min(rec_full, 2ull * (unsigned long long)m + slack);
        bool fixed_caps = false;
        if (const char *oc = ctx_opt(ctx, "OWN_DENSE_CAP")) { own_cap = strtoull(oc, nullptr, 10) + 1; rec_cap = rec_full; fixed_caps = true; }
        if (ctx_flag(ctx, "NO_OWN_DENSE")) { own_cap = 1; rec_cap = rec_full; fixed_caps = true; }
        if (const char *rc = ctx_opt(ctx, "REC_CAP")) { rec_cap = strtoull(rc, nullptr, 10) + 1; fixed_caps = true; }
        if (ctx_flag(ctx, "FULL_CAPS")) { own_cap = own_full; rec_cap = rec_full; }
        if (!fixed_caps && ctx->cap_hint.nv == nv && ctx->cap_hint.m == m) {
            own_cap = std::min(own_full, std::max(own_cap, ctx->cap_hint.own_cap));
            rec_cap = std::min(rec_full, std::max(rec_cap, ctx->cap_hint.rec_cap));
        }
        const uint32_t sentinel = geom.sentinel_base();
        uint32_t *d_key = nullptr; int2 *d_val = nullptr;
        unsigned long long n_claimed = 0;
        bool ok = false;
        st.ms_tri_fill = 0.0;
        for (int attempt = 0; attempt < 2; ++attempt) {
            size_t free_b = 0, total_b = 0;
            (void)hipMemGetInfo(&free_b, &total_b);
            const unsigned long long budget = (unsigned long long)((free_b + ctx->pool.unused_bytes()) * 0.7);
            if (own_cap * sizeof(int2) > budget / 2) own_cap = budget / 2 / sizeof(int2);
            if (rec_cap * 12ull > budget / 2) rec_cap = budget / 2 / 12ull;
            if (rec_cap > 0xFFFFFFF0ull) rec_cap = 0xFFFFFFF0ull;
            ok = bufs.alloc(&d_key, (size_t)rec_cap) == hipSuccess && bufs.alloc(&d_val, (size_t)rec_cap) == hipSuccess &&
                 bufs.alloc(&d_owndense, (size_t)own_cap) == hipSuccess &&
                 (d_ownoff || bufs.alloc(&d_ownoff, (size_t)m + 1) == hipSuccess) && (d_dcur || bufs.alloc(&d_dcur, 4) == hipSuccess);
            uint2 *d_scratch = nullptr;
            if (ok && !ctx_flag(ctx, "NO_REC_SCRATCH") && bufs.alloc(&d_scratch, (size_t)gws * kTriWaves * kScratchRec) != hipSuccess) { (void)hipGetLastError(); d_scratch = nullptr; }
            if (!ok) { (void)hipGetLastError(); break; }
            KOMB_HIP(ctx, hipMemsetAsync(d_dcur, 0, 4 * sizeof(unsigned long long), s));
            const TriStream ts{d_key, d_val, d_dcur + 2, rec_cap, sentinel, geom.nb - 1u, kChunkBits};
            ctx->timer.start(s);
            k_wedges<TRI_SINGLE><<<gws, kBlock, 0, s>>>(d_orow, d_ocol, d_line, d_wtasks, 0, n_wtasks, d_own, d_other, d_owndense, d_dcur, own_cap, d_ownoff, ts, d_scratch, ablate);
            st.ms_tri_fill += ctx->timer.stop(s);
            unsigned long long dc[4] = {0, 0, 0, 0};
            KOMB_HIP(ctx, d2h(ctx, dc, d_dcur, sizeof(dc)));
            n_claimed = dc[2];
            bufs.release(d_scratch);
            if (ctx_flag(ctx, "TRI_DEBUG"))
                fprintf(stderr, "komb triangles: stream build (attempt %d): %llu record positions claimed of %llu, dense own-role region %llu entries claimed of %llu, %llu task ranges overflowed their record buffer\n",
                        attempt, dc[2], rec_cap, dc[0], own_cap, dc[1]);
            if (n_claimed <= rec_cap) {
                if (!fixed_caps) { ctx->cap_hint.nv = nv; ctx->cap_hint.m = m; ctx->cap_hint.own_cap = own_cap; ctx->cap_hint.rec_cap = rec_cap; }
                break;
            }
            ok = false;
            if (attempt == 1 || fixed_caps) break;
            bufs.release(d_key); bufs.release(d_val); bufs.release(d_owndense);
            d_key = nullptr; d_val = nullptr; d_owndense = nullptr;
            own_cap = std::min(own_full, std::max(own_cap, dc[0] + own_slack));
            rec_cap = std::min(rec_full, n_claimed + slack);
            st.stream_retries += 1;
        }
        uint32_t *d_skey = nullptr;
        if (ok) {
            uint32_t *d_key2 = nullptr; unsigned long long *d_val2 = nullptr;
            ok = bufs.alloc(&d_key2, (size_t)n_claimed + 1) == hipSuccess && bufs.alloc(&d_val2, (size_t)n_claimed + 1) == hipSuccess;
            if (ok) {
                ctx->timer.start(s);
                unsigned long long *sv = nullptr;
                if (geom.nb_bits > 0) KOMB_TRY(prim_sort_pairs_u32_u64(ctx, d_key, d_key2, (unsigned long long *)d_val, d_val2, (int64_t)n_claimed, kChunkBits, kChunkBits + geom.nb_bits, &d_skey, &sv));
                else { d_skey = d_key; sv = (unsigned long long *)d_val; }
                st.ms_sort = ctx->timer.stop(s);
                d_recval = (int2 *)sv;
                if (d_skey == d_key) { bufs.release(d_key2); bufs.release(d_val2); } else { bufs.release(d_key); bufs.release(d_val); }
                d_reckey = d_skey;
                KOMB_HIP(ctx, bufs.alloc(&d_toff, (size_t)n_bins + 2));
                KOMB_HIP(ctx, bufs.alloc(&d_bintot, (size_t)n_bins + 2));
                KOMB_HIP(ctx, bufs.alloc(&d_grp, (size_t)kInitOff + 4));
                if (!whole_peel_finish && !shard_peel_on && !ctx_flag(ctx, "NO_FIRST_QUEUE")) KOMB_HIP(ctx, bufs.alloc(&d_light0, (size_t)m));
                ctx->timer.start(s);
                peel_ctrl_pre(s, d_grp);
                KOMB_HIP(ctx, hipMemsetAsync(d_mom + 5, 0, sizeof(unsigned long long), s));
                k_bin_offsets<<<grid_for(n_bins + 1), kBlock, 0, s>>>(d_skey, (int64_t)n_claimed, geom, d_toff);
                k_bin_count<<<grid_for(n_bins, 1, 256 * 8), kBlock, 0, s>>>(d_skey, d_toff, geom, d_own, m, d_cnt, d_bintot, d_mom + 5, (int32_t *)(d_grp + kInitOff + 1));
                st.ms_compact = ctx->timer.stop(s);
                st.tri_records = (int64_t)n_claimed;
            } else (void)hipGetLastError();
        }
        if (!ok) {
            bufs.release(d_key); bufs.release(d_val); bufs.release(d_owndense); bufs.release(d_ownoff); bufs.release(d_dcur);
            bufs.release(d_grp); bufs.release(d_light0); d_grp = nullptr; d_light0 = nullptr;
            d_owndense = nullptr; d_ownoff = nullptr; d_dcur = nullptr;
            KOMB_HIP(ctx, zero_counts());
            KOMB_HIP(ctx, hipMemsetAsync(d_mom + 5, 0, sizeof(unsigned long long), s));
            st.ms_tri_fill = 0.0;
            layout = IDX_TWO_PASS;
        }
    }
    if (layout != IDX_TWO_PASS && d_cnt_ref) {
        k_count_mismatch<<<ge, kBlock, 0, s>>>(d_cnt, d_cnt_ref, m + 1, d_mom + 8);
    }
    if (layout == IDX_TWO_PASS) {
        if (d_cnt_ref) {
            KOMB_HIP(ctx, hipMemcpyAsync(d_cnt, d_cnt_ref, ((size_t)m + 1) * sizeof(uint32_t), hipMemcpyDeviceToDevice, s));
            KOMB_HIP(ctx, hipMemsetAsync(d_mom + 5, 0, sizeof(unsigned long long), s));
            k_total_u32<<<ge, kBlock, 0, s>>>(d_cnt, m + 1, d_mom + 5);
        } else if (!have_counts) {
            ctx->timer.start(s);
            k_triangles<TRI_COUNT><<<gt, kBlock, 0, s>>>(d_orow, d_ocol, nv, 0, ntasks, d_own, d_other, nullptr, nullptr, ablate, tri_tv);
            st.ms_tri_count = ctx->timer.stop(s);
            k_sum_counts<<<ge, kBlock, 0, s>>>(d_own, d_other, nullptr, m + 1, d_cnt, d_mom + 5);
        }
    }
    st.index_layout = layout;
    {
        unsigned long long mom[9];
        KOMB_HIP(ctx, d2h(ctx, mom, d_mom, sizeof(mom)));
        st.triangles = (int64_t)(mom[5] / 3);
        bufs.release(d_mom);
        if (mom[8] != 0)
            KOMB_FAIL(ctx, KOMB_ERR_DEVICE, "komb_truss_run_sharded: %llu edges whose all-reduced support differs from the support of the index build", mom[8]);
        if (mom[5] > 0xFFFFFFF0ull)
            KOMB_FAIL(ctx, KOMB_ERR_LIMIT, "graph has %llu triangles; the incidence index is limited to 2^32-16 entries (3 per triangle)",
                      mom[5] / 3);
    }
    bufs.release(d_cnt_ref);
    uint32_t total = 0;
    const uint32_t sum_supports = (uint32_t)st.triangles * 3u;
    int2 *d_inc = nullptr;
    int32_t *d_sup = nullptr, *d_stamp = nullptr, *d_truss = nullptr;
    uint8_t *d_st8 = nullptr;
    bool peel_inited = false;
    if (layout == IDX_STREAM) {
        KOMB_TRY(prim_exclusive_sum_u32(ctx, d_bintot, d_bintot, n_bins + 1));
        total = sum_supports;
        KOMB_HIP(ctx, bufs.alloc(&d_inc, (size_t)total));
        KOMB_HIP(ctx, bufs.alloc(&d_sup, (size_t)m));
        KOMB_HIP(ctx, bufs.alloc(&d_stamp, (size_t)m));
        KOMB_HIP(ctx, bufs.alloc(&d_st8, (size_t)m + 16));
        KOMB_HIP(ctx, bufs.alloc(&d_truss, (size_t)m));
        ctx->timer.start(s);
        k_bin_finish<<<grid_for(n_bins, 1, 256 * kFinPerCu), kFinBlock, 0, s>>>(d_reckey, d_recval, d_toff, geom, d_own, d_cnt, d_bintot, d_owndense, d_ownoff, d_inc, m,
                                                                      d_off2, d_sup, d_stamp, d_st8, d_grp + kInitOff, d_light0);
        st.ms_compact += ctx->timer.stop(s);
        peel_inited = true;
        bufs.release(d_toff); bufs.release(d_bintot); bufs.release((void *)d_recval); bufs.release(d_reckey);
        bufs.release(d_owndense); bufs.release(d_ownoff); bufs.release(d_dcur);
    } else {
        KOMB_HIP(ctx, bufs.alloc(&d_off, (size_t)m + 1));
        KOMB_TRY(prim_exclusive_sum_u32(ctx, d_cnt, d_off, m + 1));
        KOMB_HIP(ctx, d2h(ctx, &total, d_off + m, sizeof(uint32_t)));
        KOMB_HIP(ctx, bufs.alloc(&d_inc, (size_t)total));
        ctx->timer.start(s);
        KOMB_HIP(ctx, zero_counts());
        k_back_cursors<<<ge, kBlock, 0, s>>>(d_off, m, d_other);
        k_triangles<TRI_SINGLE><<<gt, kBlock, 0, s>>>(d_orow, d_ocol, nv, 0, ntasks, d_own, d_other, d_off, d_inc, ablate, tri_tv);
        st.ms_tri_fill = ctx->timer.stop(s);
    }
    st.ms_support = st.ms_tri_count + st.ms_tri_fill + st.ms_sort + st.ms_compact;
    bufs.release(d_cnt); bufs.release(d_own);

    phase.next("truss: peel");
    PeelCtrl *d_ctrl = nullptr;
    PeelQueues Q{nullptr, {nullptr, nullptr}, {nullptr, nullptr}, {nullptr, nullptr}, 0};
    const size_t heavy_cap = (size_t)total / 32 + 64;
    if (!peel_inited) {
        KOMB_HIP(ctx, bufs.alloc(&d_sup, (size_t)m));
        KOMB_HIP(ctx, bufs.alloc(&d_stamp, (size_t)m));
        KOMB_HIP(ctx, bufs.alloc(&d_st8, (size_t)m + 16));
        KOMB_HIP(ctx, bufs.alloc(&d_truss, (size_t)m));
        KOMB_HIP(ctx, bufs.alloc(&d_grp, (size_t)kInitOff + 4));
    }
    for (int i = 0; i < 2; ++i) {
        if (i == 0 && d_light0) Q.light[0] = d_light0;
        else KOMB_HIP(ctx, bufs.alloc(&Q.light[i], (size_t)m));
        KOMB_HIP(ctx, bufs.alloc(&Q.heavy[i], heavy_cap));
        KOMB_HIP(ctx, bufs.alloc(&Q.live[i], (size_t)m / 2 + 64));
    }
    KOMB_HIP(ctx, bufs.alloc(&d_ctrl, 1));
    KOMB_HIP(ctx, bufs.alloc(&Q.code, (size_t)m));
    KOMB_HIP(ctx, bufs.alloc(&Q.rlevel, (size_t)m + 2));
    KOMB_HIP(ctx, hipMemsetAsync(Q.rlevel, 0, 2 * sizeof(int32_t), s));
    int32_t retire_every = kRetireEvery;
    if (const char *e = ctx_opt(ctx, "RETIRE_EVERY")) retire_every = std::max(1, std::min((int)kRetireEvery, atoi(e)));
#ifdef KOMB_DEBUG_SWITCHES
    TrussProblem P{(uint32_t)m, d_off2, d_inc, d_sup, d_stamp, d_st8, retire_every, getenv("KOMB_PEEL_ABLATE") ? atoi(getenv("KOMB_PEEL_ABLATE")) : 0};
#else
    TrussProblem P{(uint32_t)m, d_off2, d_inc, d_sup, d_stamp, d_st8, retire_every};
#endif
    TailBufs T{};
    if (fin == FIN_LDS && tail_limit) {
        KOMB_HIP(ctx, bufs.alloc(&T.vmap, (size_t)nv));
        KOMB_HIP(ctx, bufs.alloc(&T.cnt, 64));
        KOMB_HIP(ctx, bufs.alloc(&T.vlist, (size_t)kTailMaxV));
        KOMB_HIP(ctx, bufs.alloc(&T.rows, (size_t)kTailMaxV * kTailRowWords));
        KOMB_HIP(ctx, bufs.alloc(&T.pair, (size_t)tail_limit));
        KOMB_HIP(ctx, bufs.alloc(&T.sup, (size_t)tail_limit));
        KOMB_HIP(ctx, bufs.alloc(&T.gid, (size_t)tail_limit));
        KOMB_HIP(ctx, bufs.alloc(&T.gid_by_rank, (size_t)tail_limit));
        KOMB_HIP(ctx, bufs.alloc(&T.pair_by_rank, (size_t)tail_limit));
        KOMB_HIP(ctx, bufs.alloc(&T.truss_by_rank, (size_t)tail_limit));
        KOMB_HIP(ctx, bufs.alloc(&T.spill[0], (size_t)tail_limit));
        KOMB_HIP(ctx, bufs.alloc(&T.spill[1], (size_t)tail_limit));
        T.max_edges = tail_limit;
    }
    auto run_tail = [&](const int32_t *list, uint32_t n_in) -> int {
        KOMB_HIP(ctx, hipMemsetAsync(T.vmap, 0, (size_t)nv * sizeof(int32_t), s));
        KOMB_HIP(ctx, hipMemsetAsync(T.cnt, 0, 64 * sizeof(uint32_t), s));
        KOMB_HIP(ctx, hipMemsetAsync(T.rows, 0, (size_t)kTailMaxV * kTailRowWords * sizeof(unsigned long long), s));
        const int g = grid_for(n_in, kBlock, 256);
        const bool dbg = ctx_flag(ctx, "TAIL_DEBUG");
        hipEvent_t ev[3] = {nullptr, nullptr, nullptr};
        for (auto &e : ev) (void)hipEventCreate(&e);
        (void)hipEventRecord(ev[0], s);
        k_tail_mark<<<g, kBlock, 0, s>>>(list, n_in, d_sup, d_stamp, d_osrc, d_ocol, T);
        k_tail_number<<<1, kTailMaxV, 0, s>>>(T);
        k_tail_rows<<<g, kBlock, 0, s>>>(list, n_in, d_sup, d_stamp, d_osrc, d_ocol, T);
        (void)hipEventRecord(ev[1], s);
        k_truss_tail<<<1, 1024, 0, s>>>(d_ctrl, T, d_truss);
        (void)hipEventRecord(ev[2], s);
        KOMB_HIP(ctx, d2h(ctx, &ctx->h_ctrl[0], d_ctrl, sizeof(PeelCtrl)));
        ++st.truss_tail_runs;
        float m0 = 0, m1 = 0, m2 = 0;
        (void)hipEventElapsedTime(&m0, ctx->timer.a, ev[0]); (void)hipEventElapsedTime(&m1, ev[0], ev[1]); (void)hipEventElapsedTime(&m2, ev[1], ev[2]);
        for (auto &e : ev) (void)hipEventDestroy(e);
        st.ms_tail += (double)m1 + (double)m2;
        if (dbg) {
            uint32_t h[16];
            KOMB_HIP(ctx, d2h(ctx, h, T.cnt, sizeof(h)));
            fprintf(stderr, "komb tail: %u vertices, %u edges, %s; general engine before it %.1f us, setup %.1f us, tail kernel %.1f us\n",
                    h[0], h[1], ctx->h_ctrl[0].done == 1 ? "done" : "refused", m0 * 1000.f, m1 * 1000.f, m2 * 1000.f);
#ifdef KOMB_TAIL_TIMERS
            fprintf(stderr, "komb tail: us in kernel: load %.1f ranks %.1f supports %.1f scan %.1f mark %.1f triangles %.1f retire %.1f results %.1f\n",
                    h[14] / 100.0, h[15] / 100.0, h[8] / 100.0, h[9] / 100.0, h[10] / 100.0, h[11] / 100.0, h[12] / 100.0, h[13] / 100.0);
#endif
        }
        return KOMB_OK;
    };
    const int gp = peel_grid(m);
    auto run_local = [&]() -> int {
        const PeelCtrl hc = ctx->h_ctrl[0];
        EventSet evs;
        hipEvent_t ev[2] = {nullptr, nullptr};
        for (auto &e : ev) KOMB_HIP(ctx, evs.make(&e));
        (void)hipEventRecord(ev[0], s);
        LocalStats ls;
        const int lrc = local_finish(ctx, bufs, hc, d_ctrl, (uint32_t)m, d_stamp, d_sup, Q.live[hc.live_sel],
            (uint32_t)kWave * TrussLocal::kU, sizeof(uint2), local_item_limit(ctx, kTrussLocalItems), local_density_limit(ctx, kTrussLocalDensity), true, 2, d_truss,
            [&](const LocalGraph &lg, const int32_t *num, void *items, PeelCtrl *d_cctrl, int32_t launch) {
                TrussCollect C{(uint32_t)m, d_off2, d_inc, d_stamp, num, lg.off, lg.cur, (uint2 *)items};
                PeelQueues Qc = Q;
                Qc.rlevel = nullptr;
                k_peel_step<TrussCollect><<<gp, kPeelBlock, 0, s>>>(d_cctrl, d_grp, Qc, C, launch);
            },
            [&](const LocalGraph &lg, void *items, uint64_t total_items, LocalCtrl *d_lctrl, uint32_t *d_cnt, int *nl) -> int {
                return local_fixpoint(ctx, d_lctrl, d_cnt, lg, TrussLocal{(const uint2 *)items}, total_items, nl);
            },
            &ls, [](const LocalGraph &) {});
        (void)hipEventRecord(ev[1], s);
        (void)hipEventSynchronize(ev[1]);
        float ms = 0.f;
        (void)hipEventElapsedTime(&ms, ev[0], ev[1]);
        KOMB_TRY(lrc);
        if (ls.refused) { ctx->h_ctrl[0].done = 0; ctx->h_ctrl[0].tail_limit = ls.new_limit; return KOMB_OK; }
        st.truss_local_units = (int32_t)ls.units; st.truss_local_sweeps = ls.sweeps; st.truss_local_items = (int64_t)ls.items;
        st.ms_truss_local = (double)ms;
        PeelCtrl fin_c = hc;
        fin_c.done = 1; fin_c.remaining = 0;
        fin_c.n_levels += (int32_t)ls.levels;
        fin_c.max_level = ls.max_val > fin_c.max_level ? ls.max_val : fin_c.max_level;
        ctx->h_ctrl[0] = fin_c;
        return KOMB_OK;
    };
    ctx->timer.start(s);
    if (!peel_inited) {
        peel_ctrl_pre(s, d_grp);
        k_peel_init<<<grid_for(m, kBlock, 1024), kBlock, 0, s>>>(m, d_off, d_off2, d_sup, d_stamp, d_st8, d_grp + kInitOff);
    }
    peel_ctrl_init(s, d_ctrl, d_grp, (uint32_t)m, tail_limit);
    int launches = 0, rc = KOMB_OK;
    st.truss_tail_runs = 0; st.ms_tail = 0.0;
    st.truss_local_units = 0; st.truss_local_sweeps = 0; st.truss_local_items = 0; st.ms_truss_local = 0.0;
    st.shard_exchanges = 0; st.ms_exchange = 0.0; st.exchange_words = 0;
    if (shard_peel_on) {
        uint32_t iw[2] = {0u, 0u};
        KOMB_HIP(ctx, d2h(ctx, iw, d_grp + kInitOff, sizeof(iw)));
        ShardTruss SP{(uint32_t)m, d_off2, d_inc, d_sup, d_stamp, 0u, 0u};
        shard_bounds((uint64_t)m, rank, world, &SP.lo, &SP.hi);
        ShardStats ss;
        rc = shard_peel(ctx, bufs, SP, d_sup, (uint32_t)m, iw[0], (int32_t)iw[1], rank, world, fn, user, Q, d_ctrl,
                        [&](int32_t launch) { k_peel_step<ShardTruss><<<gp, kPeelBlock, 0, s>>>(d_ctrl, d_grp, Q, SP, launch); },
                        fin == FIN_LOCAL ? tail_limit : 0u, [&]() -> int { return run_local(); }, &ss);
        st.shard_exchanges = (int32_t)ss.exchanges; st.ms_exchange = ss.ms_exchange; st.exchange_words = ss.words;
        launches = ss.launches;
        PeelCtrl fc{};
        fc.done = rc == KOMB_OK ? 1 : 2; fc.n_levels = ss.levels; fc.n_rounds = ss.rounds; fc.n_scans = ss.scans; fc.max_level = ss.max_level;
        ctx->h_ctrl[0] = fc;
    } else if (whole_peel_finish) {
        rc = d2h(ctx, &ctx->h_ctrl[0], d_ctrl, sizeof(PeelCtrl)) == hipSuccess ? KOMB_OK : KOMB_ERR_DEVICE;
        if (rc == KOMB_OK && !ctx->h_ctrl[0].done) rc = (fin == FIN_LOCAL) ? run_local() : run_tail(nullptr, (uint32_t)m);
    } else {
        ctx->h_ctrl[0].done = 0;
    }
    for (int guard = 0; rc == KOMB_OK && ctx->h_ctrl[0].done != 1 && ctx->h_ctrl[0].done != 2 && guard < 64; ++guard) {
        if (ctx->h_ctrl[0].done == 3) {
            const PeelCtrl &c = ctx->h_ctrl[0];
            if (fin == FIN_LOCAL) rc = run_local();
            else rc = c.live_mode ? run_tail(Q.live[c.live_sel], c.live_count) : run_tail(nullptr, (uint32_t)m);
            continue;
        }
        int batch = 0;
        rc = drive_peel(ctx, d_ctrl, m, [&](int32_t launch) {
            k_peel_step<TrussProblem><<<gp, kPeelBlock, 0, s>>>(d_ctrl, d_grp, Q, P, launch);
        }, &batch);
        launches += batch;
    }
    st.ms_peel = ctx->timer.stop(s);
    KOMB_TRY(rc);
#ifdef KOMB_STEP_TIMERS
    {
        const PeelCtrl &c = ctx->h_ctrl[0];
        const double n = c.pad1[6] ? (double)c.pad1[6] : 1.0;
        fprintf(stderr, "komb step timers (block 0, %u small multi-workgroup PROCESS steps), us per step: ctrl %.2f queue+slice %.2f items %.2f flush %.2f barrier %.2f ticket %.2f\n",
                c.pad1[6], c.pad1[0] / n / 100.0, c.pad1[1] / n / 100.0, c.pad1[2] / n / 100.0, c.pad1[3] / n / 100.0, c.pad1[4] / n / 100.0, c.pad1[5] / n / 100.0);
    }
#endif
    if (ctx->h_ctrl[0].done != 1) KOMB_FAIL(ctx, KOMB_ERR_DEVICE, "k-truss peel ended in an inconsistent state");
    if (ctx->h_ctrl[0].max_retire_gap > retire_every)
        KOMB_FAIL(ctx, KOMB_ERR_DEVICE, "k-truss peel: %d sub-rounds passed without a RETIRE step (period %d): edge state codes may have wrapped",
                  ctx->h_ctrl[0].max_retire_gap, retire_every);
    st.engine_flags = (layout == IDX_TWO_PASS ? KOMB_ENGINE_TWO_PASS : 0) | (shard_peel_on ? KOMB_ENGINE_SHARD_PEEL : 0) |
                      (st.truss_local_units ? KOMB_ENGINE_LOCAL_FINISH : 0) | (st.truss_tail_runs ? KOMB_ENGINE_LDS_TAIL : 0);
    st.truss_levels = ctx->h_ctrl[0].n_levels;
    st.truss_subrounds = ctx->h_ctrl[0].n_rounds;
    st.truss_launches = launches;
    st.truss_scans = ctx->h_ctrl[0].n_scans;
    st.max_trussness = ctx->h_ctrl[0].max_level + 2;
    for (int i = 0; i < 2; ++i) { bufs.release(Q.light[i]); bufs.release(Q.heavy[i]); bufs.release(Q.live[i]); }
    bufs.release(Q.code);
    bufs.release(d_sup); bufs.release(d_inc);

    phase.next("truss: canonical gather");
    ctx->timer.start(s);
    KOMB_HIP(ctx, ctx->pool.get((void **)&ctx->d_t_truss, (size_t)m * sizeof(int32_t)));
    uint32_t k_lo = 0, k_hi = (uint32_t)m;
    if (!vmask_host) {
        ctx->d_t_eu = ctx->d_ceu; ctx->d_t_ev = ctx->d_cev;
        ctx->t_own_edges = false;
        if (ctx->slice_world > 1) {
            shard_bounds((uint64_t)m, ctx->slice_rank, ctx->slice_world, &k_lo, &k_hi);
#ifndef KOMB_TEST_SKIP_SLICE_ZERO
            if (k_lo) KOMB_HIP(ctx, hipMemsetAsync(ctx->d_t_truss, 0, (size_t)k_lo * sizeof(int32_t), s));
            if (k_hi < (uint32_t)m) KOMB_HIP(ctx, hipMemsetAsync(ctx->d_t_truss + k_hi, 0, ((size_t)m - k_hi) * sizeof(int32_t), s));
#endif
        }
    } else {
        ctx->t_own_edges = true;
        KOMB_HIP(ctx, ctx->pool.get((void **)&ctx->d_t_eu, (size_t)m * sizeof(int32_t)));
        KOMB_HIP(ctx, ctx->pool.get((void **)&ctx->d_t_ev, (size_t)m * sizeof(int32_t)));
        KOMB_TRY(edge_list(ctx, sub.rowptr, sub.col, sub.nv, sub.vold, ctx->d_t_eu, ctx->d_t_ev));
    }
    ctx->t_k_lo = k_lo; ctx->t_k_hi = k_hi;
    k_truss_results<<<grid_for(m), kBlock, 0, s>>>(d_stamp, Q.rlevel, d_truss, tp->e2k, m, k_lo, k_hi, ctx->d_t_truss);
    ctx->d_t_slice = d_off2;
    bufs.detach(d_off2);
    ctx->t_sup_ready = false;
    if (vmask_host) {
        ctx->t_ne = m;
        KOMB_HIP(ctx, ctx->pool.get((void **)&ctx->d_t_sup, (size_t)m * sizeof(int32_t)));
        k_scatter_len<<<grid_for(m), kBlock, 0, s>>>(ctx->d_t_slice, tp->e2k, m, 0u, (uint32_t)m, ctx->d_t_sup);
        ctx->t_sup_ready = true;
    }
    st.ms_gather = ctx->timer.stop(s);
    if (ctx_flag(ctx, "POOL_DEBUG")) {
        size_t held = 0;
        for (const auto &b : ctx->pool.blocks) held += b.bytes;
        fprintf(stderr, "komb pool: %zu blocks, %.2f GB held, %zu hipMalloc calls so far (%.1f ms inside them), %zu trims\n", ctx->pool.blocks.size(), held / 1e9, ctx->pool.n_malloc, ctx->pool.ms_malloc, ctx->pool.n_trim);
    }
    if (vmask_host) KOMB_HIP(ctx, hipStreamSynchronize(s));
    ctx->t_ne = m;
    ctx->truss_done = true;
    return KOMB_OK;
}

}
```

### komb_amd/csrc/local_dev.h

```cpp
#pragma once

#include "peel_dev.h"

namespace komb {

constexpr int kLocBlock = 512;
constexpr int kLocWaves = kLocBlock / kWave;
constexpr int kLocHB = 4096;
constexpr int kLocBins = kLocHB / kLocBlock;
constexpr int kCntWays = 8;
constexpr int kCntWords = (5 * kCntWays + 5) * 32;
constexpr int kCntTimerWords = 6 * 12 * 2;
constexpr int kHvU = 8;
constexpr uint32_t kKeyBins = 4096;
constexpr uint32_t kMedMax = 2048;
constexpr int kGiantWin = 8;
constexpr uint32_t kGiantChunk = 8192;
constexpr int kLocBatch = 6;


struct LocalGraph {
    uint32_t n, nh;
    uint32_t *off;
    int32_t *val;
// ... 637 lines not shown
    }
    __shared__ int32_t sh_mx;
    if (threadIdx.x == 0) sh_mx = 0;
    __syncthreads();
    for (uint32_t i = threadIdx.x; i < kFinWords; i += kBlock) if (sh_bits[i]) atomicOr(&present[i], sh_bits[i]);
    for (int o = 32; o > 0; o >>= 1) mx = max(mx, __shfl_xor(mx, o));
    if (lane_id() == 0 && mx) atomicMax(&sh_mx, mx);
    __syncthreads();
    if (threadIdx.x == 0 && sh_mx) atomicMax(&ctrl->max_val, sh_mx);
}
static __global__ __launch_bounds__(kBlock) void k_local_levels(const uint32_t *__restrict__ present, uint32_t words, const uint32_t *__restrict__ cnt, LocalCtrl *ctrl)
{
    if (blockIdx.x == 0 && threadIdx.x == 0) { uint32_t e = 0; for (int i = 0; i < kCntWays; ++i) e += cnt[(4 * kCntWays + i) * 32]; ctrl->evals = e; }
    uint32_t c = 0;
    for (uint32_t i = blockIdx.x * kBlock + threadIdx.x; i < words; i += gridDim.x * kBlock) c += (uint32_t)__popc(present[i]);
    c = wave_sum(c);
    if (lane_id() == 0 && c) atomicAdd(&ctrl->levels, c);
}

template <class P>
int local_fixpoint(komb_ctx *ctx, LocalCtrl *d_ctrl, uint32_t *d_cnt, const LocalGraph &g, const P &p, uint64_t total_items, int *launches_out)
{
    hipStream_t s = ctx->stream;
    const int grid = 512;
    const uint32_t nlight_all = g.n - g.nh;
    const int list_grid = (int)std::min<uint32_t>(256u, (nlight_all + kListBlock - 1) / kListBlock ? (nlight_all + kListBlock - 1) / kListBlock : 1u);
    EventSet evs;
    hipEvent_t ev[2] = {nullptr, nullptr};
    KOMB_HIP(ctx, evs.make(&ev[0], hipEventDisableTiming));
    KOMB_HIP(ctx, evs.make(&ev[1], hipEventDisableTiming));
    LocalCtrl *h = ctx->h_local;
    const uint64_t max_launches = total_items + (uint64_t)g.n + 64u;
    int launches = 0, slot = 0, status = KOMB_OK;
    bool have_prev = false, finished = false, stuck = false;
    int32_t k = 0, seen_iters = -1;
    uint32_t full_thr = g.n / 8u + 1u;
#ifdef KOMB_DEBUG_SWITCHES
    if (const char *e = getenv("KOMB_LOCAL_FULL")) { const long d = atol(e); full_thr = d > 0 ? g.n / (uint32_t)d + 1u : 0xFFFFFFFFu; }
#endif
    const char *dbg_env = ctx_opt(ctx, "LOCAL_DEBUG");
    const bool per_sweep = dbg_env && atoi(dbg_env) >= 2;
    std::vector<hipEvent_t> sw;
    if (per_sweep) { sw.resize(1); if (evs.make(&sw[0]) == hipSuccess) (void)hipEventRecord(sw[0], s); }
    while (!finished && (uint64_t)launches < max_launches && k < 0x3FFFFFF0) {
        for (int i = 0; i < kLocBatch; ++i) {
            ++k;
            if (g.flags & kLocUseList) k_local_list<<<list_grid, kListBlock, 0, s>>>(d_ctrl, d_cnt, g, k);
            k_local_step<P><<<grid, kLocBlock, 0, s>>>(d_ctrl, d_cnt, g, p, k, full_thr); ++launches;
            if (g.nchunk && (g.flags & kLocDeferNotify)) k_local_giant_notify<P><<<(int)std::min<uint32_t>(g.nchunk, 1024u), kLocBlock, 0, s>>>(d_ctrl, g, p, k);
            if (per_sweep && sw.size() < 600) { hipEvent_t e2 = nullptr; if (evs.make(&e2) == hipSuccess) { (void)hipEventRecord(e2, s); sw.push_back(e2); } }
        }
        if (hipMemcpyAsync(&h[slot], d_ctrl, sizeof(LocalCtrl), hipMemcpyDeviceToHost, s) != hipSuccess ||
            hipEventRecord(ev[slot], s) != hipSuccess) { status = KOMB_ERR_DEVICE; break; }
        if (have_prev) {
            if (hipEventSynchronize(ev[slot ^ 1]) != hipSuccess) { status = KOMB_ERR_DEVICE; break; }
            if (h[slot ^ 1].done) finished = true;
            else if ((int32_t)h[slot ^ 1].spare[0] == seen_iters) { stuck = true; finished = true; }
            seen_iters = (int32_t)h[slot ^ 1].spare[0];
        }
        have_prev = true;
        slot ^= 1;
    }
    hipError_t e = hipStreamSynchronize(s);
    if (per_sweep) {
        fprintf(stderr, "komb local sweeps (us):");
        for (size_t i = 1; i < sw.size(); ++i) { float ms = 0.f; (void)hipEventElapsedTime(&ms, sw[i - 1], sw[i]); fprintf(stderr, " %.0f", ms * 1e3f); }
        fprintf(stderr, "\n");
    }
    if (launches_out) *launches_out = launches;
    if (status != KOMB_OK || e != hipSuccess)
        KOMB_FAIL(ctx, KOMB_ERR_DEVICE, "local fixed point: HIP failure (%s)", hipGetErrorString(e));
    if (stuck) KOMB_FAIL(ctx, KOMB_ERR_DEVICE, "local fixed point: the sweeps make no progress (sweep %d)", (int)seen_iters);
    return KOMB_OK;
}

static __global__ __launch_bounds__(kBlock) void k_local_zero(uint32_t *a, uint32_t na, uint32_t *b, uint32_t nb, uint32_t *c, uint32_t nc,
                                                       uint32_t *d, uint32_t nd, uint32_t *e, uint32_t ne)
{
    const uint32_t t = blockIdx.x * kBlock + threadIdx.x, step = gridDim.x * kBlock;
    for (uint32_t i = t; i < na; i += step) a[i] = 0u;
    for (uint32_t i = t; i < nb; i += step) b[i] = 0u;
    for (uint32_t i = t; i < nc; i += step) c[i] = 0u;
    for (uint32_t i = t; i < nd; i += step) d[i] = 0u;
    for (uint32_t i = t; i < ne; i += step) e[i] = 0u;
}

struct LocalStats {
    uint32_t units = 0, heavy = 0, levels = 0;
    int32_t max_val = 0;
    int sweeps = 0, launches = 0;
    uint64_t items = 0, evals = 0;
    bool refused = false;
    uint32_t new_limit = 0;
};

template <class LaunchCollect, class RunFix, class AfterNumber>
int local_finish(komb_ctx *ctx, DevBufs &bufs, const PeelCtrl &hc, PeelCtrl *d_ctrl, uint32_t units, const int32_t *marker,
                 const int32_t *key, const int32_t *live_list, uint32_t light_max, size_t item_bytes, uint64_t item_limit, uint32_t max_density, bool use_list, int32_t add, int32_t *out,
                 LaunchCollect &&launch_collect, RunFix &&run_fix, LocalStats *ls, AfterNumber &&after_number)
{
    hipStream_t s = ctx->stream;
    const uint32_t n = hc.remaining;
    if (n == 0) KOMB_FAIL(ctx, KOMB_ERR_STATE, "local finish: nothing left to hand over");
    const bool dbg = ctx_opt(ctx, "LOCAL_DEBUG") != nullptr;
    EventSet evs;
    hipEvent_t ev[5] = {nullptr, nullptr, nullptr, nullptr, nullptr};
    if (dbg) for (auto &e : ev) (void)evs.make(&e);
    auto stamp = [&](int i) { if (dbg) (void)hipEventRecord(ev[i], s); };
    stamp(0);
    const int32_t *list = hc.live_mode ? live_list : nullptr;
    const uint32_t n_in = hc.live_mode ? hc.live_count : units;
    LocalGraph g{};
    int32_t *d_num = nullptr;
    LocalCtrl *d_lctrl = nullptr;
    PeelCtrl *d_cctrl = nullptr;
    uint32_t *d_present = nullptr;
    const size_t present_words = ((size_t)units >> 5) + 2 > kFinWords ? ((size_t)units >> 5) + 2 : (size_t)kFinWords;
    KOMB_HIP(ctx, bufs.alloc(&d_num, (size_t)units));
    KOMB_HIP(ctx, bufs.alloc(&g.off, (size_t)n + 1));
    KOMB_HIP(ctx, bufs.alloc(&g.len, (size_t)n + 1));
    KOMB_HIP(ctx, bufs.alloc(&g.val, (size_t)n));
    KOMB_HIP(ctx, bufs.alloc(&g.mark[0], (size_t)n));
    KOMB_HIP(ctx, bufs.alloc(&g.mark[1], (size_t)n));
    KOMB_HIP(ctx, bufs.alloc(&g.gid, (size_t)n));
    KOMB_HIP(ctx, bufs.alloc(&g.cur, (size_t)n));
    KOMB_HIP(ctx, bufs.alloc(&g.list, (size_t)n));
    KOMB_HIP(ctx, bufs.alloc(&g.giant, (size_t)n));
    KOMB_HIP(ctx, bufs.alloc(&g.khist, (size_t)kKeyBins));
    KOMB_HIP(ctx, bufs.alloc(&d_lctrl, 1));
    uint32_t *d_cnt = nullptr;
    KOMB_HIP(ctx, bufs.alloc(&d_cnt, (size_t)kCntWords + kCntTimerWords));
    KOMB_HIP(ctx, bufs.alloc(&d_cctrl, 1));
// ... 61 lines not shown
    int32_t K = 0x7FFFFFFF;
    {
        uint64_t ge = 0;
        for (int32_t k = (int32_t)kKeyBins - 1; k >= 0; --k) {
            ge += kh[(size_t)k];
            if (ge >= (uint64_t)k) { if (k < (int32_t)kKeyBins - 1) K = k; break; }
        }
    }
    stamp(1);
    after_number(g);
    KOMB_HIP(ctx, bufs.alloc((unsigned char **)&d_items, (size_t)total * item_bytes));

    peel_collect_ctrl(s, d_cctrl, d_ctrl);
    PeelCtrl hcc{};
    int32_t cl = 1;
    for (int guard = 0; guard < 16 && hcc.done == 0; ++guard) {
        for (int i = 0; i < 3; ++i) launch_collect(g, d_num, d_items, d_cctrl, cl++);
        KOMB_HIP(ctx, d2h(ctx, &hcc, d_cctrl, sizeof(PeelCtrl)));
        cl = hcc.seq;
    }
    if (hcc.done != 1) KOMB_FAIL(ctx, KOMB_ERR_DEVICE, "local finish: collect pass did not complete (state %d)", hcc.done);
    int64_t gn = ((int64_t)n + kBlock - 1) / kBlock;
    const int grid_n = (int)(gn > 1024 ? 1024 : gn);
    k_local_check<<<grid_n, kBlock, 0, s>>>(g, d_lctrl);
    if (K != 0x7FFFFFFF) k_local_clamp<<<grid_n, kBlock, 0, s>>>(g, K);
    stamp(2);

    int launches = 0;
    KOMB_TRY(run_fix(g, d_items, (uint64_t)total, d_lctrl, d_cnt, &launches));
    stamp(3);
    k_local_finish<<<grid_n, kBlock, 0, s>>>(g, add, out, d_present, d_lctrl);
    k_local_levels<<<(int)(present_words / kBlock + 1 > 256 ? 256 : present_words / kBlock + 1), kBlock, 0, s>>>(d_present, (uint32_t)present_words, d_cnt, d_lctrl);
    stamp(4);
    KOMB_HIP(ctx, d2h(ctx, &hl, d_lctrl, sizeof(LocalCtrl)));
    if (dbg) {
        float t[4] = {0, 0, 0, 0};
        for (int i = 0; i < 4; ++i) (void)hipEventElapsedTime(&t[i], ev[i], ev[i + 1]);
        fprintf(stderr, "komb local finish: %u units (%u heavy, %u of them long; bound %d), %u items; number+scan %.1f us, collect %.1f us, %d sweeps (%d launches, %u evaluations) %.1f us, scatter %.1f us\n",
                n, g.nh, g.ng, K == 0x7FFFFFFF ? -1 : K, total, t[0] * 1e3f, t[1] * 1e3f, hl.iters, launches, hl.evals, t[2] * 1e3f, t[3] * 1e3f);
    }
#ifdef KOMB_LOCAL_TIMERS
    {
        unsigned long long tm[72];
        KOMB_HIP(ctx, d2h(ctx, tm, d_cnt + kCntWords, sizeof(tm)));
        for (int sw = 0; sw < 6; ++sw) {
            const unsigned long long *t = tm + sw * 12;
            const double nwv = t[10] ? (double)t[10] : 1.0;
            fprintf(stderr, "komb local timers, sweep %d (%llu waves), us per wave: hscan %.1f medium %.1f workgroup %.1f setup %.1f load+count %.1f search %.1f notify %.1f; "
                            "batches/wave %.2f groups/wave %.2f; slowest wave %.1f us\n",
                    sw == 0 ? 1 : sw * 4, t[10], t[0] / nwv / 100.0, t[1] / nwv / 100.0, t[2] / nwv / 100.0, t[3] / nwv / 100.0, t[4] / nwv / 100.0, t[5] / nwv / 100.0,
                    t[6] / nwv / 100.0, t[7] / nwv, t[8] / nwv, t[9] / 100.0);
        }
    }
#endif
    if (hl.bad) KOMB_FAIL(ctx, KOMB_ERR_DEVICE, "local finish: %u consistency failures in the compact index", hl.bad);
    if (!hl.done) KOMB_FAIL(ctx, KOMB_ERR_DEVICE, "local finish: launch budget exhausted before the fixed point");
    if (ls) {
        ls->units = n; ls->heavy = g.nh; ls->levels = hl.levels; ls->max_val = hl.max_val;
        ls->sweeps = hl.iters; ls->launches = launches; ls->items = total; ls->evals = hl.evals;
    }
    release_all();
    return KOMB_OK;
}

}
```

### komb_amd/csrc/max_clique.hip

```cpp
#include "clique_root_dev.h"

#include <algorithm>

namespace komb {

namespace {

constexpr int kMcGrid = 1024;
constexpr uint32_t kMcBatch = 256;
static_assert((long long)kMcGrid * kMcBatch == KOMB_MAXCLQ_OVERSHOOT, "the documented overshoot");
constexpr uint32_t kMcLdsCand = 512;
constexpr size_t kMcLdsBytes = 56u << 10;
constexpr size_t kMcScratchBytes = 512ull << 20;
constexpr int kMcSeedWaves = 64;
constexpr long long kMcDefaultBudget = 1ll << 30;
constexpr long long kMcMaxBudget = 0x7FFFFFFFll - KOMB_MAXCLQ_OVERSHOOT;
constexpr long long kMcListDefault = 65536;

enum McMode : int { MC_COUNT = 0, MC_SEED = 1, MC_SEARCH = 2, MC_ENUM = 3 };

struct McCtl {
    unsigned long long nodes;
    unsigned long long n_cliques;
    unsigned long long n_roots;
// ... 373 lines not shown
            KOMB_TRY(run.launch(MC_ENUM, omega, kMcGrid));
            enumerated = !run.h.stopped;
            if (enumerated && run.h.n_cliques < 1)
                KOMB_FAIL(ctx, KOMB_ERR_DEVICE, "komb_max_clique_run: the enumeration found no clique of %u vertices", omega);
        }
        if (enumerated) {
            res.flags |= KOMB_MAXCLQ_ENUMERATED;
            res.n_max = (int64_t)run.h.n_cliques;
            if (run.h.n_cliques <= (unsigned long long)list_cap) {
                res.flags |= KOMB_MAXCLQ_LISTED;
                const size_t n = (size_t)run.h.n_cliques;
                std::vector<int32_t> raw(n * omega);
                KOMB_HIP(ctx, staged_copy(ctx, raw.data(), A.list, raw.size() * sizeof(int32_t), false));
                std::vector<size_t> order(n);
                for (size_t i = 0; i < n; ++i) { order[i] = i; std::sort(raw.begin() + i * omega, raw.begin() + (i + 1) * omega); }
                std::sort(order.begin(), order.end(), [&](size_t x, size_t y) {
                    return std::lexicographical_compare(raw.begin() + x * omega, raw.begin() + (x + 1) * omega, raw.begin() + y * omega, raw.begin() + (y + 1) * omega);
                });
                res.list.resize(n * omega);
                for (size_t i = 0; i < n; ++i) std::copy(raw.begin() + order[i] * omega, raw.begin() + (order[i] + 1) * omega, res.list.begin() + i * omega);
                wit.assign(res.list.begin(), res.list.begin() + omega);
            }
        } else {
            res.n_max = -1;
            KOMB_HIP(ctx, hipMemsetAsync(fresh.count, 0, (size_t)nv * sizeof(int32_t), s));
            k_mc_mark<<<(int)((omega + kBlock - 1) / kBlock), kBlock, 0, s>>>(d_wit, omega, fresh.count);
            KOMB_HIP(ctx, hipGetLastError());
        }
        (void)hipEventRecord(e3, s);
        timed = true;
        res.n_roots = (int64_t)run.h.n_roots;
        res.nodes = (int64_t)run.h.nodes;
    }
    res.ms = ctx->timer.stop(s);
    KOMB_HIP(ctx, hipGetLastError());
    if (ctx_flag(ctx, "MAXCLQ_DEBUG")) {
        float f[3] = {0.f, 0.f, 0.f};
        if (timed) { (void)hipEventElapsedTime(&f[0], e0, e1); (void)hipEventElapsedTime(&f[1], e1, e2); (void)hipEventElapsedTime(&f[2], e2, e3); }
        fprintf(stderr, "komb max clique: %lld edges, t_max %d, omega %d, upper %d, flags %d, %lld maximum cliques, %lld roots, nodes %llu seed + %llu search + "
                "%llu enumeration of %lld, run %.3f ms, seed %.3f ms, search %.3f ms, verify + enumeration %.3f ms\n", (long long)m, res.t_max, res.omega,
                res.upper, res.flags, (long long)res.n_max, (long long)res.n_roots, (unsigned long long)nodes_seed, (unsigned long long)nodes_search,
                (unsigned long long)((uint64_t)res.nodes - nodes_seed - nodes_search), limit, res.ms, f[0], f[1], f[2]);
    }
    max_clique_drop(ctx);
    ctx->d_mc_count = fresh.count;
    fresh.count = nullptr;
    ctx->mc = std::move(res);
    ctx->mc_done = true;
    return KOMB_OK;
}

}
```

### komb_amd/csrc/maximal_cliques.hip

```cpp
#include "clique_root_dev.h"

#include <algorithm>
#include <numeric>

namespace komb {

namespace {

constexpr int kMxGrid = 1024;
constexpr uint32_t kMxBatch = 256;
static_assert((long long)kMxGrid * kMxBatch == KOMB_MAXCLQ_OVERSHOOT, "the documented overshoot");
constexpr uint32_t kMxLdsCand = 512;
constexpr size_t kMxLdsBytes = 56u << 10;
constexpr size_t kMxScratchBytes = 512ull << 20;
constexpr long long kMxDefaultBudget = 1ll << 30;
constexpr long long kMxMaxBudget = 0x7FFFFFFFll - KOMB_MAXCLQ_OVERSHOOT;
constexpr long long kMxListDefault = 65536;
constexpr long long kMxListMax = 1ll << 24;

struct MxCtl {
    unsigned long long nodes;
    unsigned long long n_roots;
    unsigned long long list_words;
    uint32_t cursor;
// ... 396 lines not shown
        else A.lds_levels = 0;
        if (lds_words * 8 > kMxLdsBytes)
            KOMB_FAIL(ctx, KOMB_ERR_LIMIT, "komb_maximal_cliques_run: %u sizes at t_max %d do not fit the LDS of a wavefront", n_k, (int)t_max);
        int grid = (int)std::min<uint32_t>(A.n_chunks, (uint32_t)kMxGrid);
        const size_t fit = kMxScratchBytes / A.slot_bytes;
        if ((size_t)grid > fit) grid = fit < 1 ? 1 : (int)fit;
        KOMB_HIP(ctx, bufs.alloc(&A.scratch, (size_t)grid * A.slot_bytes));
        A.list_cap = (unsigned long long)std::min<long long>(list_cap * ((long long)t_max + 1), kMxListMax);
        KOMB_HIP(ctx, bufs.alloc(&A.list, (size_t)A.list_cap));
        A.count_only = false;
        KOMB_HIP(ctx, hipMemsetAsync(&A.ctl->cursor, 0, sizeof(uint32_t), s));
        k_mx_walk<<<grid, kWave, lds_words * 8, s>>>(A);
        KOMB_HIP(ctx, hipGetLastError());
        KOMB_HIP(ctx, d2h(ctx, &h, A.ctl, sizeof(MxCtl)));
        if (h.bad)
            KOMB_FAIL(ctx, KOMB_ERR_DEVICE, "komb_maximal_cliques_run: the walk is inconsistent (k_min %d, t_max %d, largest candidate list %u)", (int)k_min,
                      (int)t_max, max_q);
        std::vector<unsigned long long> hist(n_k);
        KOMB_HIP(ctx, staged_copy(ctx, hist.data(), A.hist, (size_t)n_k * sizeof(unsigned long long), false));
        for (uint32_t i = 0; i < n_k; ++i) res.hist[i] = (int64_t)hist[i];
        res.n_cliques = std::accumulate(res.hist.begin(), res.hist.end(), (int64_t)0);
        res.flags = h.stopped ? 0 : KOMB_MAXIMAL_COMPLETE;
        if (!h.stopped && !h.overflow && h.list_words <= A.list_cap && res.n_cliques <= list_cap) {
            std::vector<int32_t> raw((size_t)h.list_words);
            if (!raw.empty()) KOMB_HIP(ctx, staged_copy(ctx, raw.data(), A.list, raw.size() * sizeof(int32_t), false));
            if (!mx_sort_list(raw, (size_t)res.n_cliques, res.offset, res.verts))
                KOMB_FAIL(ctx, KOMB_ERR_DEVICE, "komb_maximal_cliques_run: the stream of %llu words does not hold %lld cliques", h.list_words, (long long)res.n_cliques);
            res.flags |= KOMB_MAXIMAL_LISTED;
        }
        res.max_q = (int32_t)max_q;
        res.n_roots = (int64_t)h.n_roots;
        res.nodes = (int64_t)h.nodes;
    }
    res.ms = ctx->timer.stop(s);
    KOMB_HIP(ctx, hipGetLastError());
    for (uint32_t i = 0; i < n_k; ++i)
        if (res.hist[i]) res.omega = k_min + (int32_t)i;
    if (ctx_flag(ctx, "MAXIMAL_DEBUG"))
        fprintf(stderr, "komb maximal cliques: %lld edges, t_max %d, k_min %d, omega %d, flags %d, %lld cliques, largest candidate list %d, %lld roots, "
                "%lld nodes of %lld, run %.3f ms\n", (long long)m, res.t_max, res.k_min, res.omega, res.flags, (long long)res.n_cliques, res.max_q,
                (long long)res.n_roots, (long long)res.nodes, limit, res.ms);
    maximal_cliques_drop(ctx);
    ctx->d_mx_count = fresh.count;
    fresh.count = nullptr;
    ctx->mx = std::move(res);
    ctx->mx_done = true;
    return KOMB_OK;
}

}
```

### komb_amd/csrc/nucleus.hip

```cpp
#include "common.h"
#include "nucleus_search_dev.h"

namespace komb {

namespace {

constexpr uint32_t kNucShort = 16;
constexpr uint32_t kNucHeavy = 2048;
constexpr int kNucHeavyGrid = 256, kNucHeavyChunks = 8;
constexpr int kNucSweepGrid = 2048;
constexpr int64_t kNucMaxTri = 0x7FFFFFFFll, kNucMaxClq = 0x3FFFFFFFll;

struct NucCtl {
    unsigned long long n_tri, n_clq;
    uint32_t n_heavy;
    uint32_t n_queued;
    uint32_t bad;
    int32_t kmin;
    uint32_t n_q[2];
    uint32_t pad[6];
};
static_assert(sizeof(NucCtl) == 64, "NucCtl layout");

inline int nuc_grid(int64_t n) { return (int)((n + kBlock - 1) / kBlock); }
// ... 465 lines not shown
            KOMB_HIP(ctx, hipMemcpyAsync(d_key, key0, (size_t)T * sizeof(int32_t), hipMemcpyDeviceToDevice, s));
            KOMB_HIP(ctx, hipMemsetAsync(fresh.b.theta, 0xFF, (size_t)T * sizeof(int32_t), s));
            uint32_t *queue[2] = {d_queue, d_queue + T};
            const int sweep = nuc_sweep(T);
            int64_t remaining = T;
            while (remaining > 0) {
                k_nuc_level_begin<<<1, 1, 0, s>>>(d_ctl);
                k_nuc_min<<<sweep, kBlock, 0, s>>>(uT, fresh.b.theta, d_key, d_ctl);
                k_nuc_collect<<<sweep, kBlock, 0, s>>>(uT, fresh.b.theta, d_key, d_ctl, queue[0]);
                int sel = 0, grid = sweep;
                bool first = true;
                for (;;) {
                    k_nuc_stamp<<<grid, kBlock, 0, s>>>(d_ctl, sel, queue[sel], uT, fresh.b.theta);
                    k_nuc_walk<<<grid, kBlock, 0, s>>>(d_ctl, sel, queue[sel], queue[sel ^ 1], uT, d_inc_ptr, d_inc, d_clq, d_dead, fresh.b.theta, d_key, n_short);
                    KOMB_HIP(ctx, hipGetLastError());
                    KOMB_HIP(ctx, d2h(ctx, &h, d_ctl, sizeof(NucCtl)));
                    const int64_t done = h.n_q[sel], next = h.n_q[sel ^ 1];
                    if (h.bad || done < 1 || done + next > remaining)
                        KOMB_FAIL(ctx, KOMB_ERR_DEVICE, "komb_nucleus_run: the peel is inconsistent at level %d (frontier %lld, next %lld, left %lld, bad %u)",
                                  h.kmin, (long long)done, (long long)next, (long long)remaining, h.bad);
                    remaining -= done;
                    ++res.n_subrounds;
                    if (first) { ++res.n_levels; res.theta_max = h.kmin; first = false; }
                    if (next == 0) break;
                    sel ^= 1;
                    grid = nuc_sweep(next);
                }
            }
            (void)hipEventRecord(e_p1, s);
            k_nuc_out<<<nuc_grid(T), kBlock, 0, s>>>(uT, o, fresh.b.theta, fresh.b.edge, fresh.b.vertex);
            KOMB_HIP(ctx, hipGetLastError());
        }
    }
    res.ms = ctx->timer.stop(s);
    KOMB_HIP(ctx, hipGetLastError());
    res.n_tri = T; res.n_clq = Q;
    if (T == 0) res.theta_max = -1;
    if (timed_clq) {
        float f = 0.f;
        if (hipEventElapsedTime(&f, e_t0, e_t1) == hipSuccess) res.ms_tri = (double)f;
        if (hipEventElapsedTime(&f, e_q0, e_q1) == hipSuccess) res.ms_clq = (double)f;
        if (hipEventElapsedTime(&f, e_q1, e_p1) == hipSuccess) res.ms_peel = (double)f;
    }
    if (ctx_flag(ctx, "NUC_DEBUG"))
        fprintf(stderr, "komb nucleus: %lld edges, %lld triangles, %lld cliques, theta_max %d, %d levels, %lld sub-rounds, run %.3f ms, "
                "triangle pass %.3f ms, clique pass %.3f ms, peel %.3f ms\n", (long long)m, (long long)T, (long long)Q, res.theta_max,
                res.n_levels, (long long)res.n_subrounds, res.ms, res.ms_tri, res.ms_clq, res.ms_peel);
    nucleus_drop(ctx);
    ctx->d_nuc_a = fresh.b.a; ctx->d_nuc_b = fresh.b.b; ctx->d_nuc_c = fresh.b.c; ctx->d_nuc_key0 = fresh.b.key0;
    ctx->d_nuc_theta = fresh.b.theta; ctx->d_nuc_edge = fresh.b.edge; ctx->d_nuc_vertex = fresh.b.vertex;
    fresh.b = NucBlocks{};
    ctx->nuc = res;
    ctx->nuc_done = true;
    return KOMB_OK;
}

}
```

### komb_amd/csrc/nucleus_hierarchy.hip

```cpp
#include "forest_dev.h"
#include "nucleus_search_dev.h"

namespace komb {

namespace {

constexpr uint32_t kNhShort = 16;

struct NhCtl {
    ForestCtl f;
    uint32_t rec_n;
    uint32_t n_members;
    uint32_t bad;
    uint32_t pad[9];
};
static_assert(sizeof(NhCtl) == 64 && offsetof(NhCtl, f) == 0, "NhCtl layout");

struct NhStream { uint32_t *keys, *idx; uint4 *recs; uint32_t cap; };


__global__ void k_nh_rows(const int32_t *__restrict__ eu, uint32_t m, uint32_t *__restrict__ rs, uint32_t *__restrict__ re)
{
    const uint32_t j = blockIdx.x * kBlock + threadIdx.x;
    if (j >= m) return;
// ... 365 lines not shown
        if (!ascending || moff[levels] != nm || roff[levels] != uQ || moff[1] != 0u || roff[1] != 0u)
            KOMB_FAIL(ctx, KOMB_ERR_DEVICE, "komb_nucleus_hierarchy_run: inconsistent level table (%u of %u members, %u of %u records, %u / %u below level 1)",
                      moff[levels], nm, roff[levels], uQ, moff[1], roff[1]);

        uint32_t n_levels = 0;
        for (int32_t k = (int32_t)levels - 1; k >= 1; --k) n_levels += moff[k + 1] - moff[k] ? 1u : 0u;
        KOMB_HIP(ctx, bufs.alloc(&seg, (size_t)n_levels + 1));
        KOMB_HIP(ctx, hipMemsetAsync(seg, 0, ((size_t)n_levels + 1) * sizeof(uint32_t), s));

        const ForestState f{parent, log, claimk, cur, cnt, seg, mnode, t, &d_ctl->f, nm};
        uint32_t li = 0;
        for (int32_t k = (int32_t)levels - 1; k >= 1; --k) {
            const uint32_t sh_b = moff[k], sh_n = moff[k + 1] - moff[k];
            const uint32_t r_b = roff[k], r_n = roff[k + 1] - roff[k];
            if (!sh_n) continue;
            if (r_n) k_nh_link<<<forest_grid(r_n), kBlock, 0, s>>>(st.recs, order, r_b, r_n, uQ, uT, parent, d_ctl, log, nm);
            forest_level(ctx, f, k, li, false, mord, sh_b, sh_n, 3ull * r_n < nm ? 3ull * r_n : nm);
            ++li;
        }
        KOMB_HIP(ctx, hipGetLastError());
        KOMB_HIP(ctx, d2h(ctx, &h, d_ctl, sizeof(NhCtl)));
        if (h.f.n_nodes < 1 || h.f.n_nodes > nm || h.f.log_n > nm || h.bad)
            KOMB_FAIL(ctx, KOMB_ERR_DEVICE, "komb_nucleus_hierarchy_run: inconsistent state (%u nodes, %u hooks, %u members, bad %u)",
                      h.f.n_nodes, h.f.log_n, nm, h.bad);

        const uint32_t n = h.f.n_nodes;
        int32_t *rank = cur;
        cap_nodes = n;
        KOMB_HIP(ctx, ctx->pool.get((void **)&fresh.nodes, 5 * cap_nodes * sizeof(int32_t)));
        ForestNodes out{fresh.nodes, fresh.nodes + cap_nodes, fresh.nodes + 2 * cap_nodes,
                        (uint32_t *)fresh.nodes + 3 * cap_nodes, (uint32_t *)fresh.nodes + 4 * cap_nodes};
        KOMB_TRY(forest_tail(ctx, bufs, f, n, bits, out, rank, nullptr, mvals, mvals2));
        k_nh_tri_out<<<forest_grid(T), kBlock, 0, s>>>(uT, theta, mnode, rank, n, fresh.tnode);
        res.ms = ctx->timer.stop(s);
        KOMB_HIP(ctx, hipGetLastError());
        KOMB_HIP(ctx, d2h(ctx, &h, d_ctl, sizeof(NhCtl)));
        res.n_nodes = (int64_t)n; res.n_roots = (int64_t)h.f.n_roots; res.depth = h.f.depth; res.n_members = (int64_t)nm;
    } else {
        if (T > 0) KOMB_HIP(ctx, hipMemsetAsync(fresh.tnode, 0xFF, (size_t)T * sizeof(int32_t), s));
        res.ms = ctx->timer.stop(s);
        KOMB_HIP(ctx, hipGetLastError());
    }
    if (!fresh.nodes) KOMB_HIP(ctx, ctx->pool.get((void **)&fresh.nodes, 5 * cap_nodes * sizeof(int32_t)));
    res.cap = (int64_t)cap_nodes;

    nucleus_hierarchy_drop(ctx);
    ctx->d_nh_nodes = fresh.nodes; ctx->d_nh_tnode = fresh.tnode;
    fresh.nodes = fresh.tnode = nullptr;
    ctx->nh = res;
    ctx->nh_done = true;
    return KOMB_OK;
}

int nucleus_hierarchy_labels(komb_ctx *ctx, int32_t k, int32_t *label, int32_t *size)
{
    const int64_t T = ctx->nuc.n_tri;
    if (T == 0 || (!label && !size)) return KOMB_OK;
    DevBufs bufs(ctx);
    int32_t *d_label = nullptr, *d_size = nullptr;
    KOMB_HIP(ctx, bufs.alloc(&d_label, (size_t)T));
    KOMB_HIP(ctx, bufs.alloc(&d_size, (size_t)T));
    KOMB_TRY(nh_labels_dev(ctx, k, d_label, d_size));
    KOMB_HIP(ctx, hipStreamSynchronize(ctx->stream));
    if (label) KOMB_HIP(ctx, staged_copy(ctx, label, d_label, (size_t)T * sizeof(int32_t), false));
    if (size) KOMB_HIP(ctx, staged_copy(ctx, size, d_size, (size_t)T * sizeof(int32_t), false));
    return KOMB_OK;
}

int nucleus_hierarchy_nuclei(komb_ctx *ctx, int32_t k, int64_t cap, int64_t *n_nuclei, int32_t *rep, int32_t *n_triangles,
                             int32_t *n_edges, int32_t *n_vertices)
{
    hipStream_t s = ctx->stream;
    const int64_t T = ctx->nuc.n_tri, m = ctx->t_ne > 0 ? ctx->t_ne : 0;
// ... 60 lines not shown
```

### komb_amd/csrc/onion.hip

```cpp
#include "peel_dev.h"
#include "core_tail.h"

namespace komb {

namespace {

__global__ __launch_bounds__(kBlock) void k_onion_init(const uint32_t *__restrict__ rowptr, int64_t nv, int32_t *__restrict__ degw,
                                                       int32_t *__restrict__ core, int32_t *__restrict__ layer, uint32_t *__restrict__ init)
{
    uint32_t zeros = 0;
    int32_t lmin = 0x7FFFFFFF;
    for (int64_t v = (int64_t)blockIdx.x * kBlock + threadIdx.x; v < nv; v += (int64_t)gridDim.x * kBlock) {
        const int32_t d = (int32_t)(rowptr[v + 1] - rowptr[v]);
        degw[v] = d;
        if (d == 0) { core[v] = 0; layer[v] = 1; ++zeros; }
        else { core[v] = alive_marker((uint32_t)d); lmin = min(lmin, d); }
    }
    block_add_min(zeros, lmin, &init[0], (int32_t *)&init[1]);
}

__global__ void k_onion_round_base(PeelCtrl *ctrl, const uint32_t *grp_done)
{
    if (threadIdx.x == 0 && grp_done[kInitOff] != 0u) ctrl->round = 2;
}
// ... 90 lines not shown
    peel_ctrl_pre(s, d_grp);
    k_onion_init<<<grid_init, kBlock, 0, s>>>(ctx->d_o_rowptr, nv, d_degw, ctx->d_onion_core, ctx->d_onion_layer, d_grp + kInitOff);
    peel_ctrl_init(s, d_ctrl, d_grp, (uint32_t)nv, tail_limit);
    k_onion_round_base<<<1, 64, 0, s>>>(d_ctrl, d_grp);
    auto run_tail = [&](const int32_t *list, uint32_t n_in) -> int {
        KOMB_HIP(ctx, hipMemsetAsync(T.livebits, 0, live_words * sizeof(unsigned long long), s));
        KOMB_HIP(ctx, hipMemsetAsync(T.cnt, 0, 4 * sizeof(uint32_t), s));
        KOMB_HIP(ctx, hipMemsetAsync(T.rows, 0, (size_t)kCoreTailV * kCoreTailWords * sizeof(unsigned long long), s));
        const int64_t gm = ((int64_t)n_in + kBlock - 1) / kBlock;
        k_ctail_mark<<<(int)(gm < 1 ? 1 : (gm > 1024 ? 1024 : gm)), kBlock, 0, s>>>(list, n_in, ctx->d_onion_core, T);
        k_ctail_rows<<<dim3(kCoreTailV, 8), kBlock, 0, s>>>(ctx->d_o_rowptr, ctx->d_o_col, T);
        k_core_tail<true><<<1, 1024, 0, s>>>(d_ctrl, T, d_degw, ctx->d_onion_core, ctx->d_onion_layer);
        KOMB_HIP(ctx, d2h(ctx, &ctx->h_ctrl[0], d_ctrl, sizeof(PeelCtrl)));
        return KOMB_OK;
    };
    int st = KOMB_OK;
    if (tail_limit && (uint64_t)nv <= tail_limit) {
        st = d2h(ctx, &ctx->h_ctrl[0], d_ctrl, sizeof(PeelCtrl)) == hipSuccess ? KOMB_OK : KOMB_ERR_DEVICE;
        if (st == KOMB_OK && !ctx->h_ctrl[0].done) st = run_tail(nullptr, (uint32_t)nv);
    } else {
        ctx->h_ctrl[0].done = 0;
    }
    for (int guard = 0; st == KOMB_OK && ctx->h_ctrl[0].done != 1 && ctx->h_ctrl[0].done != 2 && guard < 64; ++guard) {
        if (ctx->h_ctrl[0].done == 3) {
            const PeelCtrl &c = ctx->h_ctrl[0];
            st = c.live_mode ? run_tail(Q.live[c.live_sel], c.live_count) : run_tail(nullptr, (uint32_t)nv);
            continue;
        }
        int batch = 0;
        st = drive_peel(ctx, d_ctrl, nv, [&](int32_t launch) {
            k_peel_step<OnionProblem><<<grid, kPeelBlock, 0, s>>>(d_ctrl, d_grp, Q, P, launch);
        }, &batch);
    }
    const double ms = ctx->timer.stop(s);
    KOMB_TRY(st);
    if (ctx->h_ctrl[0].done != 1) KOMB_FAIL(ctx, KOMB_ERR_DEVICE, "onion peel ended in an inconsistent state");
    ctx->onion_layers = (int64_t)ctx->h_ctrl[0].round - 1;
    ctx->onion_max_core = ctx->h_ctrl[0].max_level;
    ctx->onion_ms = ms;
    ctx->onion_done = true;
    return KOMB_OK;
}

}
```

### komb_amd/csrc/structural.hip

```cpp
#include "common.h"
#include "unionfind_dev.h"

namespace komb {

namespace {

typedef unsigned __int128 u128;

constexpr int32_t kScNone = 0x7FFFFFFF;
constexpr int kScTailGrid = 2048;

struct ScCtl {
    uint32_t n_similar, n_cores, n_borders, n_hubs, n_outliers, n_clusters, largest;
    uint32_t pad[9];
};
static_assert(sizeof(ScCtl) == 64, "ScCtl layout");

inline int sc_grid(int64_t n) { return (int)((n + kBlock - 1) / kBlock); }

__global__ void k_sc_init(uint32_t nv, const uint32_t *__restrict__ rowptr, uint32_t *__restrict__ deg, uint32_t *__restrict__ simdeg,
                          int32_t *__restrict__ parent, int32_t *__restrict__ lo, int32_t *__restrict__ hi, uint32_t *__restrict__ cnt)
{
    const uint32_t v = blockIdx.x * kBlock + threadIdx.x;
    if (v >= nv) return;
// ... 242 lines not shown
        KOMB_HIP(ctx, bufs.alloc(&d_parent, (size_t)nv));
        KOMB_HIP(ctx, bufs.alloc(&d_lo, (size_t)nv));
        KOMB_HIP(ctx, bufs.alloc(&d_hi, (size_t)nv));
        EventSet evs;
        hipEvent_t e0 = nullptr, e1 = nullptr;
        KOMB_HIP(ctx, evs.make(&e0));
        KOMB_HIP(ctx, evs.make(&e1));

        const int32_t *eu = ctx->d_t_eu, *ev = ctx->d_t_ev, *sup = ctx->d_t_sup;
        const bool whole = !ctx->t_own_edges;
        uint32_t *simdeg = (uint32_t *)fresh.b.simdeg;
        const uint32_t un = (uint32_t)nv, um = (uint32_t)m, umu = (uint32_t)mu;
        const uint64_t num2 = (uint64_t)eps_num * (uint64_t)eps_num, den2 = (uint64_t)eps_den * (uint64_t)eps_den;
        const int gv = sc_grid(nv), ge = sc_grid(m);
        ctx->timer.start(s);
        KOMB_HIP(ctx, hipMemsetAsync(d_ctl, 0, sizeof(ScCtl), s));
        k_sc_init<<<gv, kBlock, 0, s>>>(un, whole ? ctx->d_o_rowptr : nullptr, d_deg, simdeg, d_parent, d_lo, d_hi, d_cnt);
        if (m > 0) {
            if (!whole) k_sc_degree<<<ge, kBlock, 0, s>>>(eu, ev, um, d_deg);
            (void)hipEventRecord(e0, s);
            k_sc_similar<<<ge, kBlock, 0, s>>>(eu, ev, sup, um, d_deg, num2, den2, fresh.b.similar, simdeg, d_ctl);
            (void)hipEventRecord(e1, s);
            k_sc_link<<<ge, kBlock, 0, s>>>(eu, ev, fresh.b.similar, um, simdeg, umu, d_parent);
            k_sc_flatten<false><<<gv, kBlock, 0, s>>>(un, simdeg, umu, d_parent, fresh.b.label);
        }
        k_sc_flatten<true><<<gv, kBlock, 0, s>>>(un, simdeg, umu, d_parent, fresh.b.label);
        if (m > 0) {
            k_sc_border<<<ge, kBlock, 0, s>>>(eu, ev, fresh.b.similar, um, simdeg, umu, fresh.b.label);
            k_sc_hub<<<ge, kBlock, 0, s>>>(eu, ev, um, fresh.b.label, d_lo, d_hi);
        }
        const int tail_grid = gv < kScTailGrid ? gv : kScTailGrid;
        k_sc_count<<<tail_grid, kBlock, 0, s>>>(un, fresh.b.label, d_cnt);
        k_sc_finish<<<tail_grid, kBlock, 0, s>>>(un, simdeg, umu, d_lo, d_hi, d_cnt, fresh.b.label, fresh.b.size, fresh.b.role, d_ctl);
        res.ms = ctx->timer.stop(s);
        KOMB_HIP(ctx, hipGetLastError());
        ScCtl h;
        KOMB_HIP(ctx, d2h(ctx, &h, d_ctl, sizeof(ScCtl)));
        if (m > 0) {
            float f = 0.f;
            if (hipEventElapsedTime(&f, e0, e1) == hipSuccess) res.ms_similar = (double)f;
        }
        res.n_similar = (int64_t)h.n_similar; res.n_cores = (int64_t)h.n_cores; res.n_borders = (int64_t)h.n_borders;
        res.n_hubs = (int64_t)h.n_hubs; res.n_outliers = (int64_t)h.n_outliers; res.n_clusters = (int64_t)h.n_clusters;
        res.largest = (int64_t)h.largest;
        if (ctx_flag(ctx, "STRUCT_DEBUG"))
            fprintf(stderr, "komb structural: %lld vertices, %lld edges, run %.3f ms, similarity pass %.3f ms\n",
                    (long long)nv, (long long)m, res.ms, res.ms_similar);
    }
    structural_drop(ctx);
    ctx->d_sc_label = fresh.b.label; ctx->d_sc_size = fresh.b.size; ctx->d_sc_role = fresh.b.role; ctx->d_sc_simdeg = fresh.b.simdeg;
    ctx->d_sc_similar = fresh.b.similar;
    fresh.b = ScBlocks{};
    ctx->sc = res;
    ctx->sc_done = true;
    return KOMB_OK;
}

int structural_fetch_edges(komb_ctx *ctx, int32_t *similar)
{
    const int64_t m = ctx->t_ne > 0 ? ctx->t_ne : 0;
    if (m == 0 || ctx->nv <= 0 || !similar) return KOMB_OK;
    DevBufs bufs(ctx);
    int32_t *d_out = nullptr;
    KOMB_HIP(ctx, bufs.alloc(&d_out, (size_t)m));
    k_sc_widen<<<sc_grid(m), kBlock, 0, ctx->stream>>>(ctx->d_sc_similar, (uint32_t)m, d_out);
    KOMB_HIP(ctx, hipGetLastError());
    KOMB_HIP(ctx, hipStreamSynchronize(ctx->stream));
// ... 6 lines not shown
```

Before: 4.098 billion.

## Defer timer event synchronization and trim host round-trips in peel drivers

Replaces the blocking Timer with a Stopwatch that records event marks and resolves all spans at one final synchronization, so intermediate phase timings no longer stall the host. The peel driver can take a known starting sequence instead of reading it back from the device, returns as soon as a done control block is observed, and polls into separate pinned slots. Local finish can skip its final stream synchronize and defer the control readback. The k-truss path also gains a staging keep area and an index capacity check. The cost is more bookkeeping and a larger risk that deferred checks or timings are resolved at the wrong point.

Result: no change. 4.128 billion (median of 6 runs) (+0.7%).

```diff
diff --git a/komb_amd/csrc/api.cpp b/komb_amd/csrc/api.cpp
--- a/komb_amd/csrc/api.cpp
+++ b/komb_amd/csrc/api.cpp
@@ -48,12 +48,11 @@
         return ctx;
     }
     e = hipSetDevice(ctx->device);
-    if (e == hipSuccess) e = hipHostMalloc((void **)&ctx->h_ctrl, 2 * sizeof(PeelCtrl), hipHostMallocDefault);
+    if (e == hipSuccess) e = hipHostMalloc((void **)&ctx->h_ctrl, 3 * sizeof(PeelCtrl), hipHostMallocDefault);
     if (e == hipSuccess) e = hipHostMalloc((void **)&ctx->h_local, 2 * sizeof(LocalCtrl), hipHostMallocDefault);
-    if (e == hipSuccess) e = hipHostMalloc(&ctx->h_stage, kStageBytes, hipHostMallocDefault);
+    if (e == hipSuccess) e = hipHostMalloc(&ctx->h_stage, kStageBytes + kStageKeep, hipHostMallocDefault);
     ctx->stream = nullptr;
     if (e == hipSuccess && !(ctx->opts.reserved[0] & KOMB_CREATE_NULL_STREAM)) { e = hipStreamCreate(&ctx->stream); ctx->own_stream = e == hipSuccess; }
-    if (e == hipSuccess && !ctx->timer.init()) e = hipErrorUnknown;
     if (e != hipSuccess) {
         ctx->err = std::string("device initialisation failed: ") + hipGetErrorString(e);
         return ctx;
diff --git a/komb_amd/csrc/clique_census.hip b/komb_amd/csrc/clique_census.hip
--- a/komb_amd/csrc/clique_census.hip
+++ b/komb_amd/csrc/clique_census.hip
@@ -386,7 +386,8 @@
         res.n_roots = (int64_t)h.n_roots;
         res.nodes = (int64_t)h.nodes;
     }
-    res.ms = ctx->timer.stop(s);
+    ctx->timer.stop(s, &res.ms);
+    KOMB_HIP(ctx, ctx->timer.resolve());
     KOMB_HIP(ctx, hipGetLastError());
     for (uint32_t i = 0; i < n_k; ++i)
         if (res.total[i]) res.omega = k_lo + (int32_t)i;
diff --git a/komb_amd/csrc/clique_communities.hip b/komb_amd/csrc/clique_communities.hip
--- a/komb_amd/csrc/clique_communities.hip
+++ b/komb_amd/csrc/clique_communities.hip
@@ -434,7 +434,8 @@
             res.n_overlap += res.v_comm[(size_t)v] >= 2;
         }
     }
-    res.ms = ctx->timer.stop(s);
+    ctx->timer.stop(s, &res.ms);
+    KOMB_HIP(ctx, ctx->timer.resolve());
     KOMB_HIP(ctx, hipGetLastError());
     if (ctx_flag(ctx, "PERC_DEBUG"))
         fprintf(stderr, "komb clique communities: k %d (list k_min %d), %lld cliques, %lld members of at most %u vertices, %lld entries, group %u, "
diff --git a/komb_amd/csrc/common.h b/komb_amd/csrc/common.h
--- a/komb_amd/csrc/common.h
+++ b/komb_amd/csrc/common.h
@@ -89,19 +89,43 @@
 
 enum FinishMode : int { FIN_LOCAL = 0, FIN_LDS = 1, FIN_NONE = 2 };
 
-struct Timer {
-    hipEvent_t a = nullptr, b = nullptr;
-    bool init() { return hipEventCreate(&a) == hipSuccess && hipEventCreate(&b) == hipSuccess; }
-    void start(hipStream_t s) { (void)hipEventRecord(a, s); }
-    double stop(hipStream_t s)
-    {
-        (void)hipEventRecord(b, s);
-        (void)hipEventSynchronize(b);
-        float ms = 0.f;
-        (void)hipEventElapsedTime(&ms, a, b);
-        return (double)ms;
-    }
-    void destroy() { if (a) (void)hipEventDestroy(a); if (b) (void)hipEventDestroy(b); a = b = nullptr; }
+struct Stopwatch {
+    struct Span { int a, b; double *dst; bool add; };
+    std::vector<hipEvent_t> ev;
+    std::vector<Span> spans;
+    int used = 0, open = -1;
+    int mark(hipStream_t s)
+    {
+        if (used == (int)ev.size()) {
+            hipEvent_t e = nullptr;
+            if (hipEventCreate(&e) != hipSuccess) { (void)hipGetLastError(); return -1; }
+            ev.push_back(e);
+        }
+        if (hipEventRecord(ev[(size_t)used], s) != hipSuccess) { (void)hipGetLastError(); return -1; }
+        return used++;
+    }
+    void span(int a, int b, double *dst, bool add = false) { spans.push_back({a, b, dst, add}); }
+    void start(hipStream_t s) { open = mark(s); }
+    void stop(hipStream_t s, double *dst, bool add = false) { span(open, mark(s), dst, add); }
+    void forget(const double *dst)
+    {
+        size_t k = 0;
+        for (const Span &p : spans) if (p.dst != dst) spans[k++] = p;
+        spans.resize(k);
+    }
+    hipError_t resolve()
+    {
+        const hipError_t rc = used ? hipEventSynchronize(ev[(size_t)used - 1]) : hipSuccess;
+        for (const Span &p : spans) {
+            float ms = 0.f;
+            if (rc != hipSuccess || p.a < 0 || p.b < 0 || hipEventElapsedTime(&ms, ev[(size_t)p.a], ev[(size_t)p.b]) != hipSuccess) ms = 0.f;
+            if (p.add) *p.dst += (double)ms; else *p.dst = (double)ms;
+        }
+        discard();
+        return rc;
+    }
+    void discard() { spans.clear(); used = 0; open = -1; }
+    void destroy() { for (hipEvent_t e : ev) if (e) (void)hipEventDestroy(e); ev.clear(); discard(); }
 };
 
 struct EventSet {
@@ -226,7 +250,7 @@
     int device = 0;
     hipStream_t stream = nullptr;
     bool own_stream = false;
-    komb::Timer timer;
+    komb::Stopwatch timer;
     std::map<std::string, std::string> options;
 
     int64_t nv = -1, ne = 0;
@@ -471,6 +495,8 @@
     } while (0)
 
 constexpr size_t kStageBytes = 64 << 10;
+constexpr size_t kStageKeep = 256;
+inline void *stage_keep(komb_ctx *ctx) { return ctx->h_stage ? (char *)ctx->h_stage + kStageBytes : nullptr; }
 inline hipError_t d2h(komb_ctx *ctx, void *dst, const void *src, size_t bytes)
 {
     if (ctx->h_stage && bytes <= kStageBytes && dst != ctx->h_stage) {
@@ -578,7 +604,7 @@
 int peel_grid(int64_t units);
 
 template <typename F>
-int drive_peel(komb_ctx *ctx, PeelCtrl *d_ctrl, int64_t units, F &&launch, int *launches_out)
+int drive_peel(komb_ctx *ctx, PeelCtrl *d_ctrl, int64_t units, F &&launch, int *launches_out, int32_t first_seq = -1)
 {
 #ifndef KOMB_PEEL_BATCH
 #define KOMB_PEEL_BATCH 24
@@ -587,8 +613,9 @@
 #define KOMB_PEEL_BATCH_SHORT 6
 #endif
     constexpr int kBatch = KOMB_PEEL_BATCH, kBatchShort = KOMB_PEEL_BATCH_SHORT, kShortBatches = 6;
-    PeelCtrl first;
-    KOMB_HIP(ctx, d2h(ctx, &first, d_ctrl, sizeof(PeelCtrl)));
+    PeelCtrl first{};
+    first.seq = first_seq;
+    if (first_seq < 0) KOMB_HIP(ctx, d2h(ctx, &first, d_ctrl, sizeof(PeelCtrl)));
     int32_t next = first.seq;
 #ifdef KOMB_DEBUG_SWITCHES
     if (const char *tr = getenv("KOMB_PEEL_TRACE")) {
@@ -629,16 +656,21 @@
     int launches = 0, slot = 0, status = KOMB_OK;
     bool have_prev = false, finished = false, stuck = false;
     int32_t seen_seq = first.seq - 1;
+    PeelCtrl *poll = ctx->h_ctrl + 1;
     for (int64_t batch = 0; batch < max_batches && !finished; ++batch) {
         const int nb = (batch >= 1 && batch <= kShortBatches) ? kBatchShort : kBatch;
         for (int i = 0; i < nb; ++i) { launch(next); ++next; ++launches; }
-        if (hipMemcpyAsync(&ctx->h_ctrl[slot], d_ctrl, sizeof(PeelCtrl), hipMemcpyDeviceToHost, ctx->stream) != hipSuccess ||
+        if (hipMemcpyAsync(&poll[slot], d_ctrl, sizeof(PeelCtrl), hipMemcpyDeviceToHost, ctx->stream) != hipSuccess ||
             hipEventRecord(ev[slot], ctx->stream) != hipSuccess) { status = KOMB_ERR_DEVICE; break; }
         if (have_prev) {
             if (hipEventSynchronize(ev[slot ^ 1]) != hipSuccess) { status = KOMB_ERR_DEVICE; break; }
-            const PeelCtrl &h = ctx->h_ctrl[slot ^ 1];
-            if (h.done) finished = true;
-            else if (h.seq == seen_seq) { stuck = true; finished = true; }
+            const PeelCtrl &h = poll[slot ^ 1];
+            if (h.done) {
+                ctx->h_ctrl[0] = h;
+                if (launches_out) *launches_out = launches;
+                return KOMB_OK;
+            }
+            if (h.seq == seen_seq) { stuck = true; finished = true; }
             seen_seq = h.seq;
         }
         have_prev = true;
diff --git a/komb_amd/csrc/communities.hip b/komb_amd/csrc/communities.hip
--- a/komb_amd/csrc/communities.hip
+++ b/komb_amd/csrc/communities.hip
@@ -303,7 +303,9 @@
     const int tail_grid = grid < kCommTailGrid ? grid : kCommTailGrid;
     k_comm_count<<<tail_grid, kBlock, 0, s>>>(d_nm, d_parent, d_cnt);
     k_comm_finish<<<tail_grid, kBlock, 0, s>>>((uint32_t)m, truss, k, d_pos, d_parent, d_kept, d_cnt, ctx->d_comm_label, ctx->d_comm_size, d_ctl);
-    const double ms = ctx->timer.stop(s);
+    double ms = 0.0;
+    ctx->timer.stop(s, &ms);
+    KOMB_HIP(ctx, ctx->timer.resolve());
     KOMB_HIP(ctx, hipGetLastError());
     CommCtl h;
     KOMB_HIP(ctx, d2h(ctx, &h, d_ctl, sizeof(CommCtl)));
@@ -350,7 +352,8 @@
         KOMB_HIP(ctx, d2h(ctx, &h, d_ctl, sizeof(CommCtl)));
         ctx->comm_multi = (int64_t)h.n_multi;
     }
-    ctx->comm_ms_vertices = ctx->timer.stop(s);
+    ctx->timer.stop(s, &ctx->comm_ms_vertices);
+    KOMB_HIP(ctx, ctx->timer.resolve());
     ctx->comm_v_ready = true;
     return KOMB_OK;
 }
diff --git a/komb_amd/csrc/community_hierarchy.hip b/komb_amd/csrc/community_hierarchy.hip
--- a/komb_amd/csrc/community_hierarchy.hip
+++ b/komb_amd/csrc/community_hierarchy.hip
@@ -381,7 +381,8 @@
         } else {
             k_ch_edges_out<<<grid, kBlock, 0, s>>>((uint32_t)m, truss, d_pos, nullptr, nullptr, 0u, fresh.enode);
         }
-        ms = ctx->timer.stop(s);
+        ctx->timer.stop(s, &ms);
+        KOMB_HIP(ctx, ctx->timer.resolve());
         KOMB_HIP(ctx, hipGetLastError());
         KOMB_HIP(ctx, d2h(ctx, &h, d_ctl, sizeof(ChCtl)));
         n_nodes = (int64_t)n; n_roots = (int64_t)h.f.n_roots; depth = h.f.depth; n_members = (int64_t)nm;
diff --git a/komb_amd/csrc/components.hip b/komb_amd/csrc/components.hip
--- a/komb_amd/csrc/components.hip
+++ b/komb_amd/csrc/components.hip
@@ -267,7 +267,9 @@
     const int tail_grid = grid < kCompTailGrid ? grid : kCompTailGrid;
     k_comp_count<<<tail_grid, kBlock, 0, s>>>((uint32_t)nv, parent, d_cnt);
     k_comp_finish<<<tail_grid, kBlock, 0, s>>>((uint32_t)nv, parent, d_cnt, ctx->d_comp_size, d_ctl);
-    const double ms = ctx->timer.stop(s);
+    double ms = 0.0;
+    ctx->timer.stop(s, &ms);
+    KOMB_HIP(ctx, ctx->timer.resolve());
     KOMB_HIP(ctx, hipGetLastError());
     CompCtl h;
     KOMB_HIP(ctx, d2h(ctx, &h, d_ctl, sizeof(CompCtl)));
diff --git a/komb_amd/csrc/corea.hip b/komb_amd/csrc/corea.hip
--- a/komb_amd/csrc/corea.hip
+++ b/komb_amd/csrc/corea.hip
@@ -81,7 +81,8 @@
         st = prim_sort_pairs_desc_i64(ctx, d_k[2], d_k[3], d_i[2], d_i[3], n, bits_for((int64_t)maxc * n + maxd), &sk, &si);
     }
     if (st == KOMB_OK) k_run_ranks<<<grid, kBlock, 0, s>>>(sk, si, n, d_r[1]);
-    ctx->stats.ms_corea = ctx->timer.stop(s);
+    ctx->timer.stop(s, &ctx->stats.ms_corea);
+    KOMB_HIP(ctx, ctx->timer.resolve());
     KOMB_TRY(st);
     KOMB_HIP(ctx, staged_copy(ctx, rank_deg, d_r[0], (size_t)n * 8, false));
     KOMB_HIP(ctx, staged_copy(ctx, rank_key, d_r[1], (size_t)n * 8, false));
diff --git a/komb_amd/csrc/densest.hip b/komb_amd/csrc/densest.hip
--- a/komb_amd/csrc/densest.hip
+++ b/komb_amd/csrc/densest.hip
@@ -493,7 +493,9 @@
     den_row_pass(ctx, DenCount{ctx->d_core, d_cnt, d_hdeg, 0u, 0u, 0u}, 0, d_ctl, d_heavy, heavy_cap);
     KOMB_TRY(prim_exclusive_sum_u32(ctx, d_cnt, d_off, nv));
     k_den_total<<<1, kBlock, 0, s>>>((uint32_t)nv, d_flag, d_pid, d_cnt, d_off, d_hdeg, heavy_cap, d_ctl);
-    double ms = ctx->timer.stop(s);
+    double ms = 0.0;
+    ctx->timer.stop(s, &ms);
+    KOMB_HIP(ctx, ctx->timer.resolve());
     KOMB_HIP(ctx, hipGetLastError());
     DenCtl h;
     KOMB_HIP(ctx, d2h(ctx, &h, d_ctl, sizeof(DenCtl)));
@@ -556,7 +558,8 @@
     k_den_decide<<<1, kWave, 0, s>>>(rounds ? (uint32_t)part_grid : 0u, d_part, d_ctl);
     KOMB_HIP(ctx, hipGetLastError());
     k_den_out<<<grid, kBlock, 0, s>>>((uint32_t)nv, ctx->d_core, d_pid, d_load, d_rank, d_ctl, ctx->d_dens_member, ctx->d_dens_load);
-    ms += ctx->timer.stop(s);
+    ctx->timer.stop(s, &ms, true);
+    KOMB_HIP(ctx, ctx->timer.resolve());
     hipError_t e = hipGetLastError();
     if (e == hipSuccess) e = d2h(ctx, &h, d_ctl, sizeof(DenCtl));
     if (e != hipSuccess) { ctx->dens_done = false; KOMB_HIP(ctx, e); }
diff --git a/komb_amd/csrc/hierarchy.hip b/komb_amd/csrc/hierarchy.hip
--- a/komb_amd/csrc/hierarchy.hip
+++ b/komb_amd/csrc/hierarchy.hip
@@ -269,7 +269,9 @@
     int32_t *rank = cur;
     if (n > 0) KOMB_TRY(forest_tail(ctx, bufs, f, n, bits, out, rank, nullptr, vvals, vvals2));
     k_hier_vertices_out<<<grid, kBlock, 0, s>>>((uint32_t)nv, vnode, rank, ctx->d_hier_vnode);
-    const double ms = ctx->timer.stop(s);
+    double ms = 0.0;
+    ctx->timer.stop(s, &ms);
+    KOMB_HIP(ctx, ctx->timer.resolve());
     KOMB_HIP(ctx, hipGetLastError());
     KOMB_HIP(ctx, d2h(ctx, &h, d_ctl, sizeof(HierCtl)));
     ctx->hier_nodes = (int64_t)n; ctx->hier_roots = (int64_t)h.f.n_roots; ctx->hier_depth = h.f.depth;
diff --git a/komb_amd/csrc/kcore.hip b/komb_amd/csrc/kcore.hip
--- a/komb_amd/csrc/kcore.hip
+++ b/komb_amd/csrc/kcore.hip
@@ -227,6 +227,9 @@
 
     Range r_all("komb_core_run");
     DevBufs bufs(ctx);
+    Stopwatch &sw = ctx->timer;
+    sw.discard();
+    struct SwGuard { Stopwatch &w; ~SwGuard() { w.discard(); } } sw_guard{sw};
     const size_t heavy_cap = (size_t)(2 * ctx->ne) / 32 + 64;
     int32_t *d_degw = nullptr; PeelCtrl *d_ctrl = nullptr; uint32_t *d_grp = nullptr;
     CoreTailBufs T{};
@@ -264,7 +267,7 @@
     const int grid_init = (int)(g > 1024 ? 1024 : g);
     const int grid = peel_grid(nv);
     CoreProblem P{(uint32_t)nv, ctx->d_o_rowptr, ctx->d_o_col, d_degw, ctx->d_core};
-    ctx->timer.start(s);
+    const int mk_core = sw.mark(s);
     peel_ctrl_pre(s, d_grp);
     k_core_init<<<grid_init, kBlock, 0, s>>>(ctx->d_o_rowptr, nv, ctx->d_deg, d_degw, ctx->d_core, d_grp + kInitOff);
     peel_ctrl_init(s, d_ctrl, d_grp, (uint32_t)nv, tail_limit);
@@ -282,10 +285,7 @@
     auto run_local = [&]() -> int {
         const PeelCtrl hc = ctx->h_ctrl[0];
         Range r_local("core: local finish");
-        EventSet evs;
-        hipEvent_t ev[2] = {nullptr, nullptr};
-        for (auto &e : ev) KOMB_HIP(ctx, evs.make(&e));
-        (void)hipEventRecord(ev[0], s);
+        const int mk0 = sw.mark(s);
         KOMB_HIP(ctx, hipMemsetAsync(d_livebits, 0, live_words * sizeof(unsigned long long), s));
         LocalStats ls;
         const int rc = local_finish(ctx, bufs, hc, d_ctrl, (uint32_t)nv, ctx->d_core, d_degw, Q.live[hc.live_sel],
@@ -299,14 +299,11 @@
             },
             &ls,
             [&](const LocalGraph &lg) { k_live_bits<<<(int)((lg.n + 255) / 256 > 1024 ? 1024 : (lg.n + 255) / 256), 256, 0, s>>>(lg.gid, lg.n, d_livebits); });
-        (void)hipEventRecord(ev[1], s);
-        (void)hipEventSynchronize(ev[1]);
-        float ms = 0.f;
-        (void)hipEventElapsedTime(&ms, ev[0], ev[1]);
+        const int mk1 = sw.mark(s);
         KOMB_TRY(rc);
         if (ls.refused) { ctx->h_ctrl[0].done = 0; ctx->h_ctrl[0].tail_limit = ls.new_limit; return KOMB_OK; }
         stt.core_local_units = (int32_t)ls.units; stt.core_local_sweeps = ls.sweeps; stt.core_local_items = (int64_t)ls.items;
-        stt.ms_core_local = (double)ms;
+        sw.span(mk0, mk1, &stt.ms_core_local);
         PeelCtrl done = hc;
         done.done = 1; done.remaining = 0;
         done.n_levels += (int32_t)ls.levels;
@@ -334,6 +331,7 @@
         if (st == KOMB_OK && !ctx->h_ctrl[0].done) st = (fin == FIN_LOCAL) ? run_local() : run_tail(nullptr, (uint32_t)nv);
     } else {
         ctx->h_ctrl[0].done = 0;
+        ctx->h_ctrl[0].seq = 1;
     }
     for (int guard = 0; st == KOMB_OK && ctx->h_ctrl[0].done != 1 && ctx->h_ctrl[0].done != 2 && guard < 64; ++guard) {
         if (ctx->h_ctrl[0].done == 3) {
@@ -345,10 +343,11 @@
         int batch = 0;
         st = drive_peel(ctx, d_ctrl, nv, [&](int32_t launch) {
             k_peel_step<CoreProblem><<<grid, kPeelBlock, 0, s>>>(d_ctrl, d_grp, Q, P, launch);
-        }, &batch);
+        }, &batch, ctx->h_ctrl[0].seq);
         launches += batch;
     }
-    stt.ms_core = ctx->timer.stop(s);
+    sw.span(mk_core, sw.mark(s), &stt.ms_core);
+    if (st == KOMB_OK) KOMB_HIP(ctx, sw.resolve());
 #ifdef KOMB_STEP_TIMERS
     {
         const PeelCtrl &c = ctx->h_ctrl[0];
diff --git a/komb_amd/csrc/ktruss.hip b/komb_amd/csrc/ktruss.hip
--- a/komb_amd/csrc/ktruss.hip
+++ b/komb_amd/csrc/ktruss.hip
@@ -282,6 +282,9 @@
     if (ctx->nv == 0 || ctx->ne == 0) return empty_result();
     Range r_all("komb_truss_run");
     DevBufs bufs(ctx);
+    Stopwatch &sw = ctx->timer;
+    sw.discard();
+    struct SwGuard { Stopwatch &w; ~SwGuard() { w.discard(); } } sw_guard{sw};
 
     Range phase("truss: preparation");
     InducedCsr sub;
@@ -289,9 +292,9 @@
     struct SubGuard { komb_ctx *c; InducedCsr *g; TrussPrep *p; ~SubGuard() { prep_free(c, p); induced_free(c, g); } } sub_guard{ctx, &sub, &sub_prep};
     TrussPrep *tp = &ctx->prep;
     if (vmask_host) {
-        ctx->timer.start(s);
+        sw.start(s);
         KOMB_TRY(induce_csr(ctx, vmask_host, &sub));
-        st.ms_orient = ctx->timer.stop(s);
+        sw.stop(s, &st.ms_orient);
         if (sub.ns == 0) return empty_result();
         KOMB_TRY(prep_build(ctx, sub.rowptr, sub.col, sub.nv, sub.ns, &sub_prep));
         st.ms_prepare = sub_prep.ms; st.truss_prepared = 1;
@@ -366,17 +369,18 @@
     auto zero_counts = [&]() -> hipError_t { return hipMemsetAsync(d_own, 0, 2 * ((size_t)m + 1) * sizeof(uint32_t), s); };
     if (!(world == 1 && layout == IDX_STREAM)) KOMB_HIP(ctx, zero_counts());
     bool have_counts = false;
+    unsigned long long own_claimed = 0, rec_claimed = 0;
     if (world > 1) {
         const int64_t task_lo = n_wtasks * rank / world, task_hi = n_wtasks * (rank + 1) / world;
-        ctx->timer.start(s);
+        sw.start(s);
         k_wedges<TRI_COUNT><<<gw, kBlock, 0, s>>>(d_orow, d_ocol, d_line, d_wtasks, task_lo, task_hi, d_own, d_other, nullptr, nullptr, 0ull, nullptr, no_stream, nullptr, ablate);
-        st.ms_tri_count = ctx->timer.stop(s);
+        sw.stop(s, &st.ms_tri_count);
         k_sum_counts<<<ge, kBlock, 0, s>>>(d_own, d_other, nullptr, m + 1, d_cnt, d_mom + 5);
-        ctx->timer.start(s);
+        sw.start(s);
         KOMB_HIP(ctx, hipStreamSynchronize(s));
         if (fn(user, d_cnt, (int64_t)m + 1) != 0)
             KOMB_FAIL(ctx, KOMB_ERR_DEVICE, "komb_truss_run_sharded: all-reduce callback failed");
-        st.ms_allreduce = ctx->timer.stop(s);
+        sw.stop(s, &st.ms_allreduce);
         KOMB_HIP(ctx, hipMemsetAsync(d_mom + 5, 0, sizeof(unsigned long long), s));
         k_total_u32<<<ge, kBlock, 0, s>>>(d_cnt, m + 1, d_mom + 5);
         have_counts = true;
@@ -425,12 +429,13 @@
             if (!ok) { (void)hipGetLastError(); break; }
             KOMB_HIP(ctx, hipMemsetAsync(d_dcur, 0, 4 * sizeof(unsigned long long), s));
             const TriStream ts{d_key, d_val, d_dcur + 2, rec_cap, sentinel, geom.nb - 1u, kChunkBits};
-            ctx->timer.start(s);
+            sw.start(s);
             k_wedges<TRI_SINGLE><<<gws, kBlock, 0, s>>>(d_orow, d_ocol, d_line, d_wtasks, 0, n_wtasks, d_own, d_other, d_owndense, d_dcur, own_cap, d_ownoff, ts, d_scratch, ablate);
-            st.ms_tri_fill += ctx->timer.stop(s);
+            sw.stop(s, &st.ms_tri_fill, true);
             unsigned long long dc[4] = {0, 0, 0, 0};
             KOMB_HIP(ctx, d2h(ctx, dc, d_dcur, sizeof(dc)));
             n_claimed = dc[2];
+            own_claimed = dc[0];
             bufs.release(d_scratch);
             if (ctx_flag(ctx, "TRI_DEBUG"))
                 fprintf(stderr, "komb triangles: stream build (attempt %d): %llu record positions claimed of %llu, dense own-role region %llu entries claimed of %llu, %llu task ranges overflowed their record buffer\n",
@@ -452,11 +457,11 @@
             uint32_t *d_key2 = nullptr; unsigned long long *d_val2 = nullptr;
             ok = bufs.alloc(&d_key2, (size_t)n_claimed + 1) == hipSuccess && bufs.alloc(&d_val2, (size_t)n_claimed + 1) == hipSuccess;
             if (ok) {
-                ctx->timer.start(s);
+                sw.start(s);
                 unsigned long long *sv = nullptr;
                 if (geom.nb_bits > 0) KOMB_TRY(prim_sort_pairs_u32_u64(ctx, d_key, d_key2, (unsigned long long *)d_val, d_val2, (int64_t)n_claimed, kChunkBits, kChunkBits + geom.nb_bits, &d_skey, &sv));
                 else { d_skey = d_key; sv = (unsigned long long *)d_val; }
-                st.ms_sort = ctx->timer.stop(s);
+                sw.stop(s, &st.ms_sort);
                 d_recval = (int2 *)sv;
                 if (d_skey == d_key) { bufs.release(d_key2); bufs.release(d_val2); } else { bufs.release(d_key); bufs.release(d_val); }
                 d_reckey = d_skey;
@@ -464,13 +469,14 @@
                 KOMB_HIP(ctx, bufs.alloc(&d_bintot, (size_t)n_bins + 2));
                 KOMB_HIP(ctx, bufs.alloc(&d_grp, (size_t)kInitOff + 4));
                 if (!whole_peel_finish && !shard_peel_on && !ctx_flag(ctx, "NO_FIRST_QUEUE")) KOMB_HIP(ctx, bufs.alloc(&d_light0, (size_t)m));
-                ctx->timer.start(s);
+                sw.start(s);
                 peel_ctrl_pre(s, d_grp);
                 KOMB_HIP(ctx, hipMemsetAsync(d_mom + 5, 0, sizeof(unsigned long long), s));
                 k_bin_offsets<<<grid_for(n_bins + 1), kBlock, 0, s>>>(d_skey, (int64_t)n_claimed, geom, d_toff);
                 k_bin_count<<<grid_for(n_bins, 1, 256 * 8), kBlock, 0, s>>>(d_skey, d_toff, geom, d_own, m, d_cnt, d_bintot, d_mom + 5, (int32_t *)(d_grp + kInitOff + 1));
-                st.ms_compact = ctx->timer.stop(s);
+                sw.stop(s, &st.ms_compact, true);
                 st.tri_records = (int64_t)n_claimed;
+                rec_claimed = n_claimed;
             } else (void)hipGetLastError();
         }
         if (!ok) {
@@ -479,7 +485,7 @@
             d_owndense = nullptr; d_ownoff = nullptr; d_dcur = nullptr;
             KOMB_HIP(ctx, zero_counts());
             KOMB_HIP(ctx, hipMemsetAsync(d_mom + 5, 0, sizeof(unsigned long long), s));
-            st.ms_tri_fill = 0.0;
+            st.ms_tri_fill = 0.0; sw.forget(&st.ms_tri_fill);
             layout = IDX_TWO_PASS;
         }
     }
@@ -492,43 +498,53 @@
             KOMB_HIP(ctx, hipMemsetAsync(d_mom + 5, 0, sizeof(unsigned long long), s));
             k_total_u32<<<ge, kBlock, 0, s>>>(d_cnt, m + 1, d_mom + 5);
         } else if (!have_counts) {
-            ctx->timer.start(s);
+            sw.start(s);
             k_triangles<TRI_COUNT><<<gt, kBlock, 0, s>>>(d_orow, d_ocol, nv, 0, ntasks, d_own, d_other, nullptr, nullptr, ablate, tri_tv);
-            st.ms_tri_count = ctx->timer.stop(s);
+            sw.stop(s, &st.ms_tri_count);
             k_sum_counts<<<ge, kBlock, 0, s>>>(d_own, d_other, nullptr, m + 1, d_cnt, d_mom + 5);
         }
     }
     st.index_layout = layout;
-    {
-        unsigned long long mom[9];
-        KOMB_HIP(ctx, d2h(ctx, mom, d_mom, sizeof(mom)));
+    unsigned long long mom[9] = {0, 0, 0, 0, 0, 0, 0, 0, 0};
+    unsigned long long *h_mom = nullptr;
+    auto check_moments = [&]() -> int {
         st.triangles = (int64_t)(mom[5] / 3);
-        bufs.release(d_mom);
         if (mom[8] != 0)
             KOMB_FAIL(ctx, KOMB_ERR_DEVICE, "komb_truss_run_sharded: %llu edges whose all-reduced support differs from the support of the index build", mom[8]);
         if (mom[5] > 0xFFFFFFF0ull)
             KOMB_FAIL(ctx, KOMB_ERR_LIMIT, "graph has %llu triangles; the incidence index is limited to 2^32-16 entries (3 per triangle)",
                       mom[5] / 3);
-    }
+        return KOMB_OK;
+    };
+    unsigned long long index_cap = own_claimed + rec_claimed;
+    static_assert(sizeof(mom) <= 128 && 128 + sizeof(LocalCtrl) <= kStageKeep, "the deferred words fit their landing area: the moments, then the local finish's control block");
+    if (layout == IDX_STREAM && index_cap <= 0xFFFFFFF0ull && stage_keep(ctx)) {
+        h_mom = (unsigned long long *)stage_keep(ctx);
+        KOMB_HIP(ctx, hipMemcpyAsync(h_mom, d_mom, sizeof(mom), hipMemcpyDeviceToHost, s));
+    } else {
+        KOMB_HIP(ctx, d2h(ctx, mom, d_mom, sizeof(mom)));
+        KOMB_TRY(check_moments());
+        index_cap = mom[5];
+    }
+    bufs.release(d_mom);
     bufs.release(d_cnt_ref);
     uint32_t total = 0;
-    const uint32_t sum_supports = (uint32_t)st.triangles * 3u;
     int2 *d_inc = nullptr;
     int32_t *d_sup = nullptr, *d_stamp = nullptr, *d_truss = nullptr;
     uint8_t *d_st8 = nullptr;
     bool peel_inited = false;
     if (layout == IDX_STREAM) {
         KOMB_TRY(prim_exclusive_sum_u32(ctx, d_bintot, d_bintot, n_bins + 1));
-        total = sum_supports;
+        total = (uint32_t)index_cap;
         KOMB_HIP(ctx, bufs.alloc(&d_inc, (size_t)total));
         KOMB_HIP(ctx, bufs.alloc(&d_sup, (size_t)m));
         KOMB_HIP(ctx, bufs.alloc(&d_stamp, (size_t)m));
         KOMB_HIP(ctx, bufs.alloc(&d_st8, (size_t)m + 16));
         KOMB_HIP(ctx, bufs.alloc(&d_truss, (size_t)m));
-        ctx->timer.start(s);
+        sw.start(s);
         k_bin_finish<<<grid_for(n_bins, 1, 256 * kFinPerCu), kFinBlock, 0, s>>>(d_reckey, d_recval, d_toff, geom, d_own, d_cnt, d_bintot, d_owndense, d_ownoff, d_inc, m,
                                                                       d_off2, d_sup, d_stamp, d_st8, d_grp + kInitOff, d_light0);
-        st.ms_compact += ctx->timer.stop(s);
+        sw.stop(s, &st.ms_compact, true);
         peel_inited = true;
         bufs.release(d_toff); bufs.release(d_bintot); bufs.release((void *)d_recval); bufs.release(d_reckey);
         bufs.release(d_owndense); bufs.release(d_ownoff); bufs.release(d_dcur);
@@ -537,13 +553,12 @@
         KOMB_TRY(prim_exclusive_sum_u32(ctx, d_cnt, d_off, m + 1));
         KOMB_HIP(ctx, d2h(ctx, &total, d_off + m, sizeof(uint32_t)));
         KOMB_HIP(ctx, bufs.alloc(&d_inc, (size_t)total));
-        ctx->timer.start(s);
+        sw.start(s);
         KOMB_HIP(ctx, zero_counts());
         k_back_cursors<<<ge, kBlock, 0, s>>>(d_off, m, d_other);
         k_triangles<TRI_SINGLE><<<gt, kBlock, 0, s>>>(d_orow, d_ocol, nv, 0, ntasks, d_own, d_other, d_off, d_inc, ablate, tri_tv);
-        st.ms_tri_fill = ctx->timer.stop(s);
-    }
-    st.ms_support = st.ms_tri_count + st.ms_tri_fill + st.ms_sort + st.ms_compact;
+        sw.stop(s, &st.ms_tri_fill);
+    }
     bufs.release(d_cnt); bufs.release(d_own);
 
     phase.next("truss: peel");
@@ -590,30 +605,33 @@
         KOMB_HIP(ctx, bufs.alloc(&T.spill[1], (size_t)tail_limit));
         T.max_edges = tail_limit;
     }
+    int mk_peel = -1;
+    LocalCtrl *h_late = (!shard_peel_on && stage_keep(ctx)) ? (LocalCtrl *)((char *)stage_keep(ctx) + 128) : nullptr;
+    LocalStats late_ls;
     auto run_tail = [&](const int32_t *list, uint32_t n_in) -> int {
         KOMB_HIP(ctx, hipMemsetAsync(T.vmap, 0, (size_t)nv * sizeof(int32_t), s));
         KOMB_HIP(ctx, hipMemsetAsync(T.cnt, 0, 64 * sizeof(uint32_t), s));
         KOMB_HIP(ctx, hipMemsetAsync(T.rows, 0, (size_t)kTailMaxV * kTailRowWords * sizeof(unsigned long long), s));
         const int g = grid_for(n_in, kBlock, 256);
         const bool dbg = ctx_flag(ctx, "TAIL_DEBUG");
-        hipEvent_t ev[3] = {nullptr, nullptr, nullptr};
-        for (auto &e : ev) (void)hipEventCreate(&e);
-        (void)hipEventRecord(ev[0], s);
+        const int t0 = sw.mark(s);
         k_tail_mark<<<g, kBlock, 0, s>>>(list, n_in, d_sup, d_stamp, d_osrc, d_ocol, T);
         k_tail_number<<<1, kTailMaxV, 0, s>>>(T);
         k_tail_rows<<<g, kBlock, 0, s>>>(list, n_in, d_sup, d_stamp, d_osrc, d_ocol, T);
-        (void)hipEventRecord(ev[1], s);
+        const int t1 = sw.mark(s);
         k_truss_tail<<<1, 1024, 0, s>>>(d_ctrl, T, d_truss);
-        (void)hipEventRecord(ev[2], s);
+        const int t2 = sw.mark(s);
         KOMB_HIP(ctx, d2h(ctx, &ctx->h_ctrl[0], d_ctrl, sizeof(PeelCtrl)));
         ++st.truss_tail_runs;
-        float m0 = 0, m1 = 0, m2 = 0;
-        (void)hipEventElapsedTime(&m0, ctx->timer.a, ev[0]); (void)hipEventElapsedTime(&m1, ev[0], ev[1]); (void)hipEventElapsedTime(&m2, ev[1], ev[2]);
-        for (auto &e : ev) (void)hipEventDestroy(e);
-        st.ms_tail += (double)m1 + (double)m2;
+        sw.span(t0, t2, &st.ms_tail, true);
         if (dbg) {
             uint32_t h[16];
             KOMB_HIP(ctx, d2h(ctx, h, T.cnt, sizeof(h)));
+            float m0 = 0, m1 = 0, m2 = 0;
+            if (mk_peel >= 0 && t0 >= 0 && t1 >= 0 && t2 >= 0) {
+                (void)hipEventElapsedTime(&m0, sw.ev[(size_t)mk_peel], sw.ev[(size_t)t0]); (void)hipEventElapsedTime(&m1, sw.ev[(size_t)t0], sw.ev[(size_t)t1]);
+                (void)hipEventElapsedTime(&m2, sw.ev[(size_t)t1], sw.ev[(size_t)t2]);
+            }
             fprintf(stderr, "komb tail: %u vertices, %u edges, %s; general engine before it %.1f us, setup %.1f us, tail kernel %.1f us\n",
                     h[0], h[1], ctx->h_ctrl[0].done == 1 ? "done" : "refused", m0 * 1000.f, m1 * 1000.f, m2 * 1000.f);
 #ifdef KOMB_TAIL_TIMERS
@@ -626,10 +644,7 @@
     const int gp = peel_grid(m);
     auto run_local = [&]() -> int {
         const PeelCtrl hc = ctx->h_ctrl[0];
-        EventSet evs;
-        hipEvent_t ev[2] = {nullptr, nullptr};
-        for (auto &e : ev) KOMB_HIP(ctx, evs.make(&e));
-        (void)hipEventRecord(ev[0], s);
+        const int mk0 = sw.mark(s);
         LocalStats ls;
         const int lrc = local_finish(ctx, bufs, hc, d_ctrl, (uint32_t)m, d_stamp, d_sup, Q.live[hc.live_sel],
             (uint32_t)kWave * TrussLocal::kU, sizeof(uint2), local_item_limit(ctx, kTrussLocalItems), local_density_limit(ctx, kTrussLocalDensity), true, 2, d_truss,
@@ -642,15 +657,13 @@
             [&](const LocalGraph &lg, void *items, uint64_t total_items, LocalCtrl *d_lctrl, uint32_t *d_cnt, int *nl) -> int {
                 return local_fixpoint(ctx, d_lctrl, d_cnt, lg, TrussLocal{(const uint2 *)items}, total_items, nl);
             },
-            &ls, [](const LocalGraph &) {});
-        (void)hipEventRecord(ev[1], s);
-        (void)hipEventSynchronize(ev[1]);
-        float ms = 0.f;
-        (void)hipEventElapsedTime(&ms, ev[0], ev[1]);
+            &ls, [](const LocalGraph &) {}, h_late);
+        const int mk1 = sw.mark(s);
         KOMB_TRY(lrc);
         if (ls.refused) { ctx->h_ctrl[0].done = 0; ctx->h_ctrl[0].tail_limit = ls.new_limit; return KOMB_OK; }
         st.truss_local_units = (int32_t)ls.units; st.truss_local_sweeps = ls.sweeps; st.truss_local_items = (int64_t)ls.items;
-        st.ms_truss_local = (double)ms;
+        sw.span(mk0, mk1, &st.ms_truss_local);
+        if (ls.pending) late_ls = ls;
         PeelCtrl fin_c = hc;
         fin_c.done = 1; fin_c.remaining = 0;
         fin_c.n_levels += (int32_t)ls.levels;
@@ -658,7 +671,7 @@
         ctx->h_ctrl[0] = fin_c;
         return KOMB_OK;
     };
-    ctx->timer.start(s);
+    mk_peel = sw.mark(s);
     if (!peel_inited) {
         peel_ctrl_pre(s, d_grp);
         k_peel_init<<<grid_for(m, kBlock, 1024), kBlock, 0, s>>>(m, d_off, d_off2, d_sup, d_stamp, d_st8, d_grp + kInitOff);
@@ -687,6 +700,7 @@
         if (rc == KOMB_OK && !ctx->h_ctrl[0].done) rc = (fin == FIN_LOCAL) ? run_local() : run_tail(nullptr, (uint32_t)m);
     } else {
         ctx->h_ctrl[0].done = 0;
+        ctx->h_ctrl[0].seq = 1;
     }
     for (int guard = 0; rc == KOMB_OK && ctx->h_ctrl[0].done != 1 && ctx->h_ctrl[0].done != 2 && guard < 64; ++guard) {
         if (ctx->h_ctrl[0].done == 3) {
@@ -698,10 +712,10 @@
         int batch = 0;
         rc = drive_peel(ctx, d_ctrl, m, [&](int32_t launch) {
             k_peel_step<TrussProblem><<<gp, kPeelBlock, 0, s>>>(d_ctrl, d_grp, Q, P, launch);
-        }, &batch);
+        }, &batch, ctx->h_ctrl[0].seq);
         launches += batch;
     }
-    st.ms_peel = ctx->timer.stop(s);
+    sw.span(mk_peel, sw.mark(s), &st.ms_peel);
     KOMB_TRY(rc);
 #ifdef KOMB_STEP_TIMERS
     {
@@ -727,7 +741,7 @@
     bufs.release(d_sup); bufs.release(d_inc);
 
     phase.next("truss: canonical gather");
-    ctx->timer.start(s);
+    sw.start(s);
     KOMB_HIP(ctx, ctx->pool.get((void **)&ctx->d_t_truss, (size_t)m * sizeof(int32_t)));
     uint32_t k_lo = 0, k_hi = (uint32_t)m;
     if (!vmask_host) {
@@ -757,7 +771,25 @@
         k_scatter_len<<<grid_for(m), kBlock, 0, s>>>(ctx->d_t_slice, tp->e2k, m, 0u, (uint32_t)m, ctx->d_t_sup);
         ctx->t_sup_ready = true;
     }
-    st.ms_gather = ctx->timer.stop(s);
+    sw.stop(s, &st.ms_gather);
+    KOMB_HIP(ctx, sw.resolve());
+    st.ms_support = st.ms_tri_count + st.ms_tri_fill + st.ms_sort + st.ms_compact;
+    if (late_ls.pending) {
+        LocalCtrl hl;
+        memcpy(&hl, h_late, sizeof(hl));
+        KOMB_TRY(local_finish_end(ctx, hl, &late_ls));
+        st.truss_local_sweeps = late_ls.sweeps;
+        st.truss_levels += (int32_t)late_ls.levels;
+        st.max_trussness = std::max(st.max_trussness, late_ls.max_val + 2);
+    }
+    if (h_mom) {
+        memcpy(mom, h_mom, sizeof(mom));
+        KOMB_TRY(check_moments());
+        if (mom[5] > index_cap)
+            KOMB_FAIL(ctx, KOMB_ERR_DEVICE, "k-truss index: %llu entries, but the enumeration claimed room for %llu only", mom[5], index_cap);
+    }
+    if (ctx_flag(ctx, "TRI_DEBUG"))
+        fprintf(stderr, "komb triangles: index of %llu entries in room for %llu\n", mom[5], index_cap);
     if (ctx_flag(ctx, "POOL_DEBUG")) {
         size_t held = 0;
         for (const auto &b : ctx->pool.blocks) held += b.bytes;
diff --git a/komb_amd/csrc/local_dev.h b/komb_amd/csrc/local_dev.h
--- a/komb_amd/csrc/local_dev.h
+++ b/komb_amd/csrc/local_dev.h
@@ -693,7 +693,7 @@
     LocalCtrl *h = ctx->h_local;
     const uint64_t max_launches = total_items + (uint64_t)g.n + 64u;
     int launches = 0, slot = 0, status = KOMB_OK;
-    bool have_prev = false, finished = false, stuck = false;
+    bool have_prev = false, finished = false, stuck = false, reached = false;
     int32_t k = 0, seen_iters = -1;
     uint32_t full_thr = g.n / 8u + 1u;
 #ifdef KOMB_DEBUG_SWITCHES
@@ -715,14 +715,14 @@
             hipEventRecord(ev[slot], s) != hipSuccess) { status = KOMB_ERR_DEVICE; break; }
         if (have_prev) {
             if (hipEventSynchronize(ev[slot ^ 1]) != hipSuccess) { status = KOMB_ERR_DEVICE; break; }
-            if (h[slot ^ 1].done) finished = true;
+            if (h[slot ^ 1].done) { finished = true; reached = true; }
             else if ((int32_t)h[slot ^ 1].spare[0] == seen_iters) { stuck = true; finished = true; }
             seen_iters = (int32_t)h[slot ^ 1].spare[0];
         }
         have_prev = true;
         slot ^= 1;
     }
-    hipError_t e = hipStreamSynchronize(s);
+    hipError_t e = (reached && status == KOMB_OK && !per_sweep) ? hipSuccess : hipStreamSynchronize(s);
     if (per_sweep) {
         fprintf(stderr, "komb local sweeps (us):");
         for (size_t i = 1; i < sw.size(); ++i) { float ms = 0.f; (void)hipEventElapsedTime(&ms, sw[i - 1], sw[i]); fprintf(stderr, " %.0f", ms * 1e3f); }
@@ -753,12 +753,21 @@
     uint64_t items = 0, evals = 0;
     bool refused = false;
     uint32_t new_limit = 0;
+    bool pending = false;
 };
+
+inline int local_finish_end(komb_ctx *ctx, const LocalCtrl &hl, LocalStats *ls)
+{
+    if (hl.bad) KOMB_FAIL(ctx, KOMB_ERR_DEVICE, "local finish: %u consistency failures in the compact index", hl.bad);
+    if (!hl.done) KOMB_FAIL(ctx, KOMB_ERR_DEVICE, "local finish: launch budget exhausted before the fixed point");
+    if (ls) { ls->levels = hl.levels; ls->max_val = hl.max_val; ls->sweeps = hl.iters; ls->evals = hl.evals; ls->pending = false; }
+    return KOMB_OK;
+}
 
 template <class LaunchCollect, class RunFix, class AfterNumber>
 int local_finish(komb_ctx *ctx, DevBufs &bufs, const PeelCtrl &hc, PeelCtrl *d_ctrl, uint32_t units, const int32_t *marker,
                  const int32_t *key, const int32_t *live_list, uint32_t light_max, size_t item_bytes, uint64_t item_limit, uint32_t max_density, bool use_list, int32_t add, int32_t *out,
-                 LaunchCollect &&launch_collect, RunFix &&run_fix, LocalStats *ls, AfterNumber &&after_number)
+                 LaunchCollect &&launch_collect, RunFix &&run_fix, LocalStats *ls, AfterNumber &&after_number, LocalCtrl *h_late = nullptr)
 {
     hipStream_t s = ctx->stream;
     const uint32_t n = hc.remaining;
@@ -886,6 +895,14 @@
     k_local_finish<<<grid_n, kBlock, 0, s>>>(g, add, out, d_present, d_lctrl);
     k_local_levels<<<(int)(present_words / kBlock + 1 > 256 ? 256 : present_words / kBlock + 1), kBlock, 0, s>>>(d_present, (uint32_t)present_words, d_cnt, d_lctrl);
     stamp(4);
+#ifndef KOMB_LOCAL_TIMERS
+    if (h_late && ls && !dbg) {
+        KOMB_HIP(ctx, hipMemcpyAsync(h_late, d_lctrl, sizeof(LocalCtrl), hipMemcpyDeviceToHost, s));
+        ls->units = n; ls->heavy = g.nh; ls->launches = launches; ls->items = total; ls->pending = true;
+        release_all();
+        return KOMB_OK;
+    }
+#endif
     KOMB_HIP(ctx, d2h(ctx, &hl, d_lctrl, sizeof(LocalCtrl)));
     if (dbg) {
         float t[4] = {0, 0, 0, 0};
@@ -907,12 +924,8 @@
         }
     }
 #endif
-    if (hl.bad) KOMB_FAIL(ctx, KOMB_ERR_DEVICE, "local finish: %u consistency failures in the compact index", hl.bad);
-    if (!hl.done) KOMB_FAIL(ctx, KOMB_ERR_DEVICE, "local finish: launch budget exhausted before the fixed point");
-    if (ls) {
-        ls->units = n; ls->heavy = g.nh; ls->levels = hl.levels; ls->max_val = hl.max_val;
-        ls->sweeps = hl.iters; ls->launches = launches; ls->items = total; ls->evals = hl.evals;
-    }
+    KOMB_TRY(local_finish_end(ctx, hl, ls));
+    if (ls) { ls->units = n; ls->heavy = g.nh; ls->launches = launches; ls->items = total; }
     release_all();
     return KOMB_OK;
 }
diff --git a/komb_amd/csrc/max_clique.hip b/komb_amd/csrc/max_clique.hip
--- a/komb_amd/csrc/max_clique.hip
+++ b/komb_amd/csrc/max_clique.hip
@@ -429,7 +429,8 @@
         res.n_roots = (int64_t)run.h.n_roots;
         res.nodes = (int64_t)run.h.nodes;
     }
-    res.ms = ctx->timer.stop(s);
+    ctx->timer.stop(s, &res.ms);
+    KOMB_HIP(ctx, ctx->timer.resolve());
     KOMB_HIP(ctx, hipGetLastError());
     if (ctx_flag(ctx, "MAXCLQ_DEBUG")) {
         float f[3] = {0.f, 0.f, 0.f};
diff --git a/komb_amd/csrc/maximal_cliques.hip b/komb_amd/csrc/maximal_cliques.hip
--- a/komb_amd/csrc/maximal_cliques.hip
+++ b/komb_amd/csrc/maximal_cliques.hip
@@ -452,7 +452,8 @@
         res.n_roots = (int64_t)h.n_roots;
         res.nodes = (int64_t)h.nodes;
     }
-    res.ms = ctx->timer.stop(s);
+    ctx->timer.stop(s, &res.ms);
+    KOMB_HIP(ctx, ctx->timer.resolve());
     KOMB_HIP(ctx, hipGetLastError());
     for (uint32_t i = 0; i < n_k; ++i)
         if (res.hist[i]) res.omega = k_min + (int32_t)i;
diff --git a/komb_amd/csrc/nucleus.hip b/komb_amd/csrc/nucleus.hip
--- a/komb_amd/csrc/nucleus.hip
+++ b/komb_amd/csrc/nucleus.hip
@@ -521,7 +521,8 @@
             KOMB_HIP(ctx, hipGetLastError());
         }
     }
-    res.ms = ctx->timer.stop(s);
+    ctx->timer.stop(s, &res.ms);
+    KOMB_HIP(ctx, ctx->timer.resolve());
     KOMB_HIP(ctx, hipGetLastError());
     res.n_tri = T; res.n_clq = Q;
     if (T == 0) res.theta_max = -1;
diff --git a/komb_amd/csrc/nucleus_hierarchy.hip b/komb_amd/csrc/nucleus_hierarchy.hip
--- a/komb_amd/csrc/nucleus_hierarchy.hip
+++ b/komb_amd/csrc/nucleus_hierarchy.hip
@@ -421,13 +421,15 @@
                         (uint32_t *)fresh.nodes + 3 * cap_nodes, (uint32_t *)fresh.nodes + 4 * cap_nodes};
         KOMB_TRY(forest_tail(ctx, bufs, f, n, bits, out, rank, nullptr, mvals, mvals2));
         k_nh_tri_out<<<forest_grid(T), kBlock, 0, s>>>(uT, theta, mnode, rank, n, fresh.tnode);
-        res.ms = ctx->timer.stop(s);
+        ctx->timer.stop(s, &res.ms);
+        KOMB_HIP(ctx, ctx->timer.resolve());
         KOMB_HIP(ctx, hipGetLastError());
         KOMB_HIP(ctx, d2h(ctx, &h, d_ctl, sizeof(NhCtl)));
         res.n_nodes = (int64_t)n; res.n_roots = (int64_t)h.f.n_roots; res.depth = h.f.depth; res.n_members = (int64_t)nm;
     } else {
         if (T > 0) KOMB_HIP(ctx, hipMemsetAsync(fresh.tnode, 0xFF, (size_t)T * sizeof(int32_t), s));
-        res.ms = ctx->timer.stop(s);
+        ctx->timer.stop(s, &res.ms);
+        KOMB_HIP(ctx, ctx->timer.resolve());
         KOMB_HIP(ctx, hipGetLastError());
     }
     if (!fresh.nodes) KOMB_HIP(ctx, ctx->pool.get((void **)&fresh.nodes, 5 * cap_nodes * sizeof(int32_t)));
diff --git a/komb_amd/csrc/onion.hip b/komb_amd/csrc/onion.hip
--- a/komb_amd/csrc/onion.hip
+++ b/komb_amd/csrc/onion.hip
@@ -146,7 +146,9 @@
             k_peel_step<OnionProblem><<<grid, kPeelBlock, 0, s>>>(d_ctrl, d_grp, Q, P, launch);
         }, &batch);
     }
-    const double ms = ctx->timer.stop(s);
+    double ms = 0.0;
+    ctx->timer.stop(s, &ms);
+    KOMB_HIP(ctx, ctx->timer.resolve());
     KOMB_TRY(st);
     if (ctx->h_ctrl[0].done != 1) KOMB_FAIL(ctx, KOMB_ERR_DEVICE, "onion peel ended in an inconsistent state");
     ctx->onion_layers = (int64_t)ctx->h_ctrl[0].round - 1;
diff --git a/komb_amd/csrc/structural.hip b/komb_amd/csrc/structural.hip
--- a/komb_amd/csrc/structural.hip
+++ b/komb_amd/csrc/structural.hip
@@ -298,7 +298,8 @@
         const int tail_grid = gv < kScTailGrid ? gv : kScTailGrid;
         k_sc_count<<<tail_grid, kBlock, 0, s>>>(un, fresh.b.label, d_cnt);
         k_sc_finish<<<tail_grid, kBlock, 0, s>>>(un, simdeg, umu, d_lo, d_hi, d_cnt, fresh.b.label, fresh.b.size, fresh.b.role, d_ctl);
-        res.ms = ctx->timer.stop(s);
+        ctx->timer.stop(s, &res.ms);
+        KOMB_HIP(ctx, ctx->timer.resolve());
         KOMB_HIP(ctx, hipGetLastError());
         ScCtl h;
         KOMB_HIP(ctx, d2h(ctx, &h, d_ctl, sizeof(ScCtl)));
```
